# jerinphilip/whisper.tflite

Hardware: AMD Instinct MI355X
Metric: audio-sec/s (RTF) whisper-tiny 30s clips batch=32 at 1/2/4/8 MI355X (higher is better)
Workload: dtype f32 (operands as two fp16 planes, f16 MFMA, f32 accumulate); 1 GPU; whisper-tiny batch=32x30s synthetic mel U(-1,1.5), fp32, random-init weights (BASELINE.json configs[1]); mel resident in HBM -> token ids on host; clips_per_gpu=32, global_batch=32, decoder_positions=30, argmax_steps=27, parallelism=clip-parallel dp1, one RCCL all_gather of id records per 8 batches, pipelined=True, batches_in_flight=10, decoder=2 consecutive steps' batches share one decoder chain (dec_pair, dec_group), last_batches_announced=2, priming_batches=1

## Files before the change

### include/wt_debug.h

```cpp
#ifndef WT_DEBUG_H_
#define WT_DEBUG_H_
#include "wt_capi.h"
#ifdef __cplusplus
extern "C" {
#endif
int wt_dbg_gemm(wt_engine* h, int M, int N, int K, const float* A, const float* W, const float* bias,
                const float* R, const float* pos, int pos_period, int epi, float* C);
int wt_dbg_gemm_planes(wt_engine* h, int M, int N, int K, const float* A, const float* W, const float* bias,
                       const float* R, const float* pos, int pos_period, int epi, int planes_out, int iters, float* C,
                       float* avg_ms, int n_cu );
int wt_dbg_set_forced_ids(wt_engine* h, const int64_t* ids, int clips);
int wt_dbg_set_plane_gemm_mode(int mode);
int wt_dbg_gemm_planes_ln(wt_engine* h, int M, int K, const float* A, const float* W, const float* bias, const float* R,
                          const float* pos, int pos_period, int epi, const float* ln_g, const float* ln_b, int n_cu,
                          float* C, float* ln_out, float* ln_y32, int* fused);
int wt_dbg_encoder_attention_planes(wt_engine* h, int batch, int T, int heads, const float* qkv, int iters, float* out,
                                    float* avg_ms);
int wt_dbg_gemm_bench(wt_engine* h, int M, int N, int K, int epi, int variant, int iters, float* avg_ms);
int wt_dbg_interference(wt_engine* h, const float* d_mel, int batch, int n_enc, int chain_len, int blocks,
                        float* enc_ms, float* chain_ms);
int wt_dbg_concurrency(wt_engine* h, const float* d_mel, int batch, int n_dec, int n_enc, float* dec_ms,
                       float* enc_ms);
int wt_dbg_dec_gemm_bench(wt_engine* h, int kind, int B, int N, int K, int rows, int iters, float* avg_us);
int wt_dbg_dec_gemm(wt_engine* h, int mode, int B, int N, int K, const float* X, const float* W,
                    const float* bias, const float* R, float* Y, int64_t* argmax_out);
int wt_dbg_dec_ln_gemm(wt_engine* h, int B, int N, int K, const float* xin, const int64_t* ids, int pos,
                       const float* tok_emb, const float* pos_emb, int n_vocab, int n_pos,
                       const float* ln_g, const float* ln_b, const float* W, const float* bias,
                       int gelu, float* Y, float* xout);
int wt_dbg_layernorm(wt_engine* h, int M, int d, const float* x, const float* g, const float* b, float* y);
int wt_dbg_encoder_attention(wt_engine* h, int batch, int T, int heads, const float* qkv, float* out);
int wt_dbg_cross_attention(wt_engine* h, int batch, int heads, int T, int chunks, int nq, const float* x,
                           const float* ln_g, const float* ln_b, const float* wq, const float* bq, const float* kc,
                           const float* vc, float* out);
int wt_dbg_cross_absorbed(wt_engine* h, int batch, int heads, int T, int chunks, int nq, const float* qp, const float* E,
                          const float* wv, const float* bv, float* out, int iters, float* avg_us);
int wt_dbg_cross_absorbed_bf16(wt_engine* h, int batch, int heads, int T, int chunks, int nq, const float* qp, const float* E,
                               const float* wv, const float* bv, float* out, int iters, float* avg_us);
int wt_dbg_cross_absorbed_chain(wt_engine* h, int bf16, int batch, int heads, int T, int chunks, int nq, int split, int n_src,
                                const float* const* E_src, const float* qp, const float* wv, const float* bv, int mode,
                                int p0_only, int nq_only, float* out, float* ws);
int wt_dbg_absorbed_query_matrix(int heads, int d, const float* wq, const float* bq, const float* wk, float* A, float* av);
int wt_dbg_self_attention(wt_engine* h, int batch, int heads, int cap, int pos, int npos, const float* qkv,
                          float* kcache, float* vcache, float* out);
int wt_dbg_self_attention_long(wt_engine* h, int batch, int heads, int cap, int pos, const float* qkv, float* kcache,
                               float* vcache, float* out);
int wt_dbg_timestamp_select(wt_engine* h, int B, int V, const float* logits, const int64_t* ids, int ids_stride,
                            const int32_t* n_ids, int sample_begin, int eot, int beg, int max_initial_timestamp,
                            int64_t* token, double* L, float* M);
int wt_dbg_gemm_bf16(wt_engine* h, int M, int N, int K, const float* A, const float* W, const float* bias,
                     const float* R, const float* pos, int pos_period, int epi, int bf16_out, int iters, float* C,
                     float* avg_ms);
int wt_dbg_gemm_bf16_ln(wt_engine* h, int M, int N, int K, const float* A, const float* W, const float* bias, const float* R,
                        const float* ln_g, const float* ln_b, float* C, float* ln_out, float* ln_y32, int* fused);
int wt_dbg_encoder_attention_bf16(wt_engine* h, int batch, int T, int heads, const float* qkv, int iters, float* out,
                                  float* avg_ms);
int wt_dbg_dec_gemm_bf16(wt_engine* h, int mode, int B, int N, int K, const float* X, const float* W, const float* bias,
                         const float* R, float* Y, int64_t* argmax_out);
int wt_dbg_dec_ln_gemm_bf16(wt_engine* h, int B, int N, int K, const float* xin, const int64_t* ids, int pos,
                            const float* tok_emb, const float* pos_emb, int n_vocab, int n_pos, const float* ln_g,
                            const float* ln_b, const float* W, const float* bias, int gelu, float* Y, float* xout);
int wt_dbg_self_attention_bf16(wt_engine* h, int batch, int heads, int cap, int pos, int npos, const float* qkv,
                               float* kcache, float* vcache, float* out);
int wt_dbg_cross_attention_bf16(wt_engine* h, int batch, int heads, int T, int chunks, int nq, const float* x,
                                const float* ln_g, const float* ln_b, const float* wq, const float* bq, const float* kc,
                                const float* vc, float* out);
int wt_dbg_beam_topk(wt_engine* h, int rows, int V, int ldl, int kk, const float* logits, float* m, float* s,
                     uint64_t* keys);
int wt_dbg_beam_step(wt_engine* h, int K, int clips, int c0, int n_live, int pos, int n_prompt, int V, int64_t eot,
                     const float* logits, const int64_t* ids, float* live_sum, int32_t* fin_tok, float* fin_sum,
                     int32_t* fin_len, int32_t* n_fin, int32_t* done, int32_t* parent, int64_t* token, int64_t* ids_next);
int wt_dbg_beam_reorder(wt_engine* h, int src_rows, int dst_rows, int cap, int d, int slabs, int pos, int V,
                        const float* kv_src, float* kv_dst, const int64_t* ids_src, int64_t* ids_dst,
                        const int32_t* parent, const int64_t* token);
int wt_dbg_beam_finalize(wt_engine* h, int K, int clips, int c0, int pos, int n_prompt, const int64_t* ids,
                         const float* live_sum, int32_t* fin_tok, float* fin_sum, int32_t* fin_len, int32_t* n_fin,
                         const int32_t* done, int64_t* out_ids, int32_t* out_n, float* out_sum, int32_t* out_len);
int wt_dbg_dec_gemm_ksplit(wt_engine* h, int bf16, int M, int B, int N, int K, const float* X, const float* W,
                           const float* bias, float* R, float* Y, float* part);
int wt_dbg_dec_ln_gemm_rows(wt_engine* h, int bf16, int M, int B, int N, int K, const float* xin, const float* xpart,
                            const int64_t* ids, int ids_stride, int pos, const float* tok_emb, const float* pos_emb,
                            int n_vocab, int n_pos, const float* ln_g, const float* ln_b, const float* W, const float* bias,
                            int gelu, float* Y, float* xout);
int wt_dbg_dec_logits(wt_engine* h, int bf16, int M, int V, int K, const float* xin, const float* xpart, const float* ln_g,
                      const float* ln_b, const float* E, int blocks, float* logits, uint64_t* records);
int wt_dbg_select_token(wt_engine* h, int B, int n_tiles, const uint64_t* records, int64_t* ids, int stride, int pos,
                        int32_t* n_ids, int32_t* finished, int64_t eot, int stop_at_eot, int keep_ids);
int wt_dbg_language_head(wt_engine* h, int rows, int d, int n_vocab, int lang_lo, int n_lang, int forced_lang, const float* x,
                         const float* xpart, const float* ln_g, const float* ln_b, const float* tok_emb, float* probs,
                         int32_t* lang, float* lang_prob, int64_t* ids, int ids_stride);
#ifdef __cplusplus
}
#endif
#endif
```

### whisper.tflite_amd/__init__.py

```python
from __future__ import annotations

import ctypes
import enum
import os
from ctypes import (POINTER, byref, c_char_p, c_float, c_int, c_int32, c_int64, c_long, c_size_t,
                    c_uint64, c_void_p)

import numpy as np

_HERE = os.path.dirname(os.path.abspath(__file__))
LIB_PATH = os.environ.get("WT_LIB_PATH") or os.path.join(_HERE, "lib", "libwhisper-tflite.so")

WT_OK = 0
WT_MAX_IDS = 32
WT_PIPELINE_DEPTH = 24
WT_LANGUAGE_AUTO = -1
CHUNK_SAMPLES = 480000
STATUS_NAMES = {0: "WT_OK", 1: "WT_ERR_INVALID_ARG", 2: "WT_ERR_IO", 3: "WT_ERR_FORMAT",
                4: "WT_ERR_UNSUPPORTED", 5: "WT_ERR_DEVICE", 6: "WT_ERR_BUFFER"}

CAPI_SYMBOLS = [
    "wt_device_alloc", "wt_device_free", "wt_device_upload", "wt_device_download", "wt_device_synchronize",
    "wt_engine_create", "wt_engine_destroy", "wt_last_error", "wt_engine_dims",
    "wt_engine_set_option", "wt_engine_get_option", "wt_engine_set_prompt", "wt_transcribe_pcm", "wt_transcribe_long_pcm", "wt_transcribe_file",
    "wt_logmel_batch", "wt_logmel_batch_dev", "wt_encdec_tokens_batch",
    "wt_encdec_tokens_batch_dev", "wt_transcribe_tokens_batch_dev", "wt_pipeline_submit_dev", "wt_pipeline_submit_pcm_dev", "wt_pipeline_collect",
    "wt_encdec_debug_batch",
    "wt_encdec_tokens_full_batch", "wt_encdec_tokens_full_batch_dev", "wt_transcribe_tokens_full_batch_dev",
    "wt_last_segments", "wt_last_segment_text", "wt_vocab_segments",
    "wt_language_count", "wt_detect_language_batch", "wt_detect_language_batch_dev", "wt_detect_language_pcm", "wt_last_languages",
    "wt_last_timings", "wt_last_beam_scores", "wt_last_kernel_stats", "wt_decode_text", "wt_language_id", "wt_lang_code", "wt_wav_read_legacy",
    "wt_vocab_info", "wt_filters", "wt_write_synthetic_weights", "wt_write_synthetic_vocab",
    "wt_vocab_open", "wt_vocab_close", "wt_vocab_get_info", "wt_vocab_get_filters", "wt_vocab_size", "wt_vocab_token",
    "wt_vocab_decode", "wt_log_mel_spectrogram", "wt_convert_tflite", "wt_shutdown",
]
DEBUG_SYMBOLS = [
    "wt_dbg_cross_absorbed", "wt_dbg_cross_absorbed_bf16", "wt_dbg_gemm_planes_ln", "wt_dbg_gemm", "wt_dbg_gemm_bench", "wt_dbg_dec_gemm_bench", "wt_dbg_dec_gemm", "wt_dbg_dec_ln_gemm", "wt_dbg_layernorm", "wt_dbg_encoder_attention",
    "wt_dbg_cross_attention", "wt_dbg_self_attention", "wt_dbg_interference", "wt_dbg_concurrency",
    "wt_dbg_gemm_planes", "wt_dbg_set_plane_gemm_mode", "wt_dbg_set_forced_ids", "wt_dbg_dec_gemm_bf16", "wt_dbg_dec_ln_gemm_bf16",
    "wt_dbg_self_attention_bf16", "wt_dbg_cross_attention_bf16", "wt_dbg_encoder_attention_planes", "wt_dbg_gemm_bf16", "wt_dbg_gemm_bf16_ln", "wt_dbg_encoder_attention_bf16",
    "wt_dbg_beam_topk", "wt_dbg_beam_step", "wt_dbg_beam_reorder", "wt_dbg_beam_finalize",
    "wt_dbg_dec_gemm_ksplit", "wt_dbg_dec_ln_gemm_rows", "wt_dbg_dec_logits", "wt_dbg_select_token",
    "wt_dbg_cross_absorbed_chain", "wt_dbg_absorbed_query_matrix", "wt_dbg_language_head", "wt_dbg_self_attention_long",
    "wt_dbg_timestamp_select",
]


class WtError(RuntimeError):
    def __init__(self, code: int, message: str):
        super().__init__(f"{STATUS_NAMES.get(code, code)}: {message}")
        self.code = code


class EngineType(enum.IntEnum):
    Monolith = 0
    EncDec = 1


class Dims(ctypes.Structure):
    _fields_ = [(n, c_int32) for n in (
        "n_mels", "n_audio_ctx", "n_audio_state", "n_audio_head", "n_audio_layer",
        "n_vocab", "n_text_ctx", "n_text_state", "n_text_head", "n_text_layer")]


class Timings(ctypes.Structure):
    _fields_ = [("logmel_ms", c_float), ("encoder_ms", c_float), ("cross_kv_ms", c_float),
                ("decoder_ms", c_float), ("total_ms", c_float), ("batch", c_int32),
                ("decoder_steps", c_int32)]


class KernelStat(ctypes.Structure):
    _fields_ = [("name", ctypes.c_char * 48), ("launches", c_int32), ("reserved", c_int32),
                ("ms", ctypes.c_double), ("flops", ctypes.c_double), ("bytes", ctypes.c_double)]


_lib = None


def lib() -> ctypes.CDLL:
    global _lib
    if _lib is None:
        if not os.path.exists(LIB_PATH):
            raise ImportError(
                f"{LIB_PATH} is missing: build it with `make lib` (or __graft_entry__.build()); "
                "there is no Python/CPU fallback for the engine")
        L = ctypes.CDLL(LIB_PATH)
        fp, ip64, ip32 = POINTER(c_float), POINTER(c_int64), POINTER(c_int32)
        L.wt_engine_create.argtypes = [c_int, c_char_p, c_char_p, c_int, c_int, POINTER(c_void_p)]
        L.wt_engine_destroy.argtypes = [c_void_p]
        L.wt_engine_destroy.restype = None
        L.wt_last_error.argtypes = [c_void_p]
        L.wt_last_error.restype = c_char_p
        L.wt_engine_dims.argtypes = [c_void_p, POINTER(Dims)]
        L.wt_engine_set_option.argtypes = [c_void_p, c_char_p, c_long]
        L.wt_engine_get_option.argtypes = [c_void_p, c_char_p, POINTER(c_long)]
        L.wt_engine_set_prompt.argtypes = [c_void_p, ip64, c_int]
        L.wt_transcribe_pcm.argtypes = [c_void_p, fp, c_size_t, c_char_p, c_size_t, POINTER(c_size_t)]
        L.wt_transcribe_long_pcm.argtypes = [c_void_p, fp, c_size_t, c_char_p, c_size_t, POINTER(c_size_t)]
        L.wt_transcribe_file.argtypes = [c_void_p, c_char_p, c_char_p, c_size_t, POINTER(c_size_t)]
        L.wt_logmel_batch.argtypes = [c_void_p, fp, c_int, fp]
        L.wt_logmel_batch_dev.argtypes = [c_void_p, c_void_p, c_int, c_void_p]
        L.wt_encdec_tokens_batch.argtypes = [c_void_p, fp, c_int, ip64, ip32]
        L.wt_encdec_tokens_batch_dev.argtypes = [c_void_p, c_void_p, c_int, ip64, ip32]
        L.wt_transcribe_tokens_batch_dev.argtypes = [c_void_p, c_void_p, c_int, ip64, ip32]
        L.wt_pipeline_submit_dev.argtypes = [c_void_p, c_void_p, c_int]
        L.wt_pipeline_submit_pcm_dev.argtypes = [c_void_p, c_void_p, c_int]
        L.wt_pipeline_collect.argtypes = [c_void_p, ip64, ip32]
        L.wt_encdec_debug_batch.argtypes = [c_void_p, fp, c_int, ip64, ip32, fp, fp, c_int]
        L.wt_last_timings.argtypes = [c_void_p, POINTER(Timings)]
        L.wt_last_beam_scores.argtypes = [c_void_p, fp, ip32, c_int]
        L.wt_last_kernel_stats.argtypes = [c_void_p, POINTER(KernelStat), c_int]
        L.wt_decode_text.argtypes = [c_void_p, ip64, c_int, c_int, c_char_p, c_size_t, POINTER(c_size_t)]
        L.wt_language_id.argtypes = [c_char_p]
        L.wt_lang_code.argtypes = [c_int]
        L.wt_lang_code.restype = c_char_p
        L.wt_wav_read_legacy.argtypes = [c_char_p, fp, c_size_t, POINTER(c_size_t)]
        L.wt_vocab_info.argtypes = [c_void_p, ip32]
        L.wt_filters.argtypes = [c_void_p, fp, c_size_t, ip32, ip32]
        L.wt_write_synthetic_weights.argtypes = [c_char_p, c_char_p, c_uint64]
        L.wt_write_synthetic_vocab.argtypes = [c_char_p, c_int]
        L.wt_vocab_open.argtypes = [c_char_p, c_int, POINTER(c_void_p)]
        L.wt_vocab_close.argtypes = [c_void_p]
        L.wt_vocab_close.restype = None
        L.wt_vocab_get_info.argtypes = [c_void_p, ip32]
        L.wt_vocab_get_filters.argtypes = [c_void_p, fp, c_size_t, ip32, ip32]
        L.wt_vocab_size.argtypes = [c_void_p]
        L.wt_vocab_token.argtypes = [c_void_p, c_int, c_char_p, c_size_t, POINTER(c_size_t)]
        L.wt_vocab_decode.argtypes = [c_void_p, ip64, c_int, c_int, c_char_p, c_size_t, POINTER(c_size_t)]
        L.wt_log_mel_spectrogram.argtypes = [fp, c_int, fp, c_int, c_int, c_int, fp, c_size_t, POINTER(c_int)]
        L.wt_convert_tflite.argtypes = [c_char_p, c_char_p]
        L.wt_dbg_gemm.argtypes = [c_void_p, c_int, c_int, c_int, fp, fp, fp, fp, fp, c_int, c_int, fp]
        L.wt_dbg_gemm_planes.argtypes = [c_void_p, c_int, c_int, c_int, fp, fp, fp, fp, fp, c_int, c_int, c_int, c_int, fp,
                                         POINTER(c_float), c_int]
        L.wt_dbg_encoder_attention_planes.argtypes = [c_void_p, c_int, c_int, c_int, fp, c_int, fp, POINTER(c_float)]
        L.wt_dbg_cross_absorbed.argtypes = [c_void_p, c_int, c_int, c_int, c_int, c_int, fp, fp, fp, fp, fp, c_int, POINTER(c_float)]
        L.wt_dbg_cross_absorbed_bf16.argtypes = L.wt_dbg_cross_absorbed.argtypes
        L.wt_dbg_cross_absorbed_chain.argtypes = [c_void_p, c_int, c_int, c_int, c_int, c_int, c_int, c_int, c_int, POINTER(fp),
                                                  fp, fp, fp, c_int, c_int, c_int, fp, fp]
        L.wt_dbg_absorbed_query_matrix.argtypes = [c_int, c_int, fp, fp, fp, fp, fp]
        L.wt_dbg_gemm_planes_ln.argtypes = [c_void_p, c_int, c_int, fp, fp, fp, fp, fp, c_int, c_int, fp, fp, c_int, fp, fp, fp,
                                            POINTER(c_int)]
        L.wt_dbg_gemm_bf16.argtypes = [c_void_p, c_int, c_int, c_int, fp, fp, fp, fp, fp, c_int, c_int, c_int, c_int, fp,
                                       POINTER(c_float)]
        L.wt_dbg_encoder_attention_bf16.argtypes = [c_void_p, c_int, c_int, c_int, fp, c_int, fp, POINTER(c_float)]
        L.wt_dbg_gemm_bf16_ln.argtypes = [c_void_p, c_int, c_int, c_int, fp, fp, fp, fp, fp, fp, fp, fp, fp, POINTER(c_int)]
        L.wt_dbg_gemm_bench.argtypes = [c_void_p, c_int, c_int, c_int, c_int, c_int, c_int, POINTER(c_float)]
        L.wt_dbg_dec_gemm_bench.argtypes = [c_void_p, c_int, c_int, c_int, c_int, c_int, c_int, POINTER(c_float)]
        L.wt_dbg_dec_gemm.argtypes = [c_void_p, c_int, c_int, c_int, c_int, fp, fp, fp, fp, fp, ip64]
        L.wt_dbg_dec_ln_gemm.argtypes = [c_void_p, c_int, c_int, c_int, fp, ip64, c_int, fp, fp,
                                         c_int, c_int, fp, fp, fp, fp, c_int, fp, fp]
        L.wt_dbg_layernorm.argtypes = [c_void_p, c_int, c_int, fp, fp, fp, fp]
        L.wt_device_alloc.argtypes = [c_void_p, ctypes.c_size_t, POINTER(c_void_p)]
        L.wt_device_free.argtypes = [c_void_p, c_void_p]
        L.wt_device_upload.argtypes = [c_void_p, c_void_p, ctypes.c_size_t, c_void_p, ctypes.c_size_t]
        L.wt_device_download.argtypes = [c_void_p, c_void_p, c_void_p, ctypes.c_size_t, ctypes.c_size_t]
        L.wt_device_synchronize.argtypes = [c_void_p]
        L.wt_dbg_set_forced_ids.argtypes = [c_void_p, POINTER(c_int64), c_int]
        L.wt_dbg_dec_gemm_bf16.argtypes = L.wt_dbg_dec_gemm.argtypes
        L.wt_dbg_dec_ln_gemm_bf16.argtypes = L.wt_dbg_dec_ln_gemm.argtypes
        L.wt_dbg_encoder_attention.argtypes = [c_void_p, c_int, c_int, c_int, fp, fp]
        L.wt_dbg_cross_attention.argtypes = [c_void_p, c_int, c_int, c_int, c_int, c_int, fp, fp, fp, fp, fp, fp, fp, fp]
        L.wt_dbg_self_attention.argtypes = [c_void_p, c_int, c_int, c_int, c_int, c_int, fp, fp, fp, fp]
        L.wt_dbg_self_attention_bf16.argtypes = L.wt_dbg_self_attention.argtypes
        L.wt_dbg_cross_attention_bf16.argtypes = L.wt_dbg_cross_attention.argtypes
        u64p = POINTER(c_uint64)
        L.wt_dbg_beam_topk.argtypes = [c_void_p, c_int, c_int, c_int, c_int, fp, fp, fp, u64p]
        L.wt_dbg_beam_step.argtypes = [c_void_p, c_int, c_int, c_int, c_int, c_int, c_int, c_int, c_int64, fp, ip64, fp, ip32,
                                       fp, ip32, ip32, ip32, ip32, ip64, ip64]
        L.wt_dbg_beam_reorder.argtypes = [c_void_p, c_int, c_int, c_int, c_int, c_int, c_int, c_int, fp, fp, ip64, ip64, ip32,
                                          ip64]
        L.wt_dbg_beam_finalize.argtypes = [c_void_p, c_int, c_int, c_int, c_int, c_int, ip64, fp, ip32, fp, ip32, ip32, ip32,
                                           ip64, ip32, fp, ip32]
        L.wt_dbg_dec_gemm_ksplit.argtypes = [c_void_p, c_int, c_int, c_int, c_int, c_int, fp, fp, fp, fp, fp, fp]
        L.wt_dbg_dec_ln_gemm_rows.argtypes = [c_void_p, c_int, c_int, c_int, c_int, c_int, fp, fp, ip64, c_int, c_int, fp, fp,
                                              c_int, c_int, fp, fp, fp, fp, c_int, fp, fp]
        L.wt_dbg_dec_logits.argtypes = [c_void_p, c_int, c_int, c_int, c_int, fp, fp, fp, fp, fp, c_int, fp, u64p]
        L.wt_dbg_select_token.argtypes = [c_void_p, c_int, c_int, u64p, ip64, c_int, c_int, ip32, ip32, c_int64, c_int,
                                          c_int]
        L.wt_language_count.argtypes = [c_void_p]
        L.wt_detect_language_batch.argtypes = [c_void_p, fp, c_int, ip32, fp]
        L.wt_detect_language_batch_dev.argtypes = [c_void_p, c_void_p, c_int, ip32, fp]
        L.wt_detect_language_pcm.argtypes = [c_void_p, fp, c_size_t, ip32, fp]
        L.wt_last_languages.argtypes = [c_void_p, ip32, fp, c_int]
        L.wt_dbg_language_head.argtypes = [c_void_p, c_int, c_int, c_int, c_int, c_int, c_int, fp, fp, fp, fp, fp, fp, ip32, fp,
                                           ip64, c_int]
        L.wt_encdec_tokens_full_batch.argtypes = [c_void_p, fp, c_int, ip64, c_int, ip32]
        L.wt_encdec_tokens_full_batch_dev.argtypes = [c_void_p, c_void_p, c_int, ip64, c_int, ip32]
        L.wt_transcribe_tokens_full_batch_dev.argtypes = [c_void_p, c_void_p, c_int, ip64, c_int, ip32]
        L.wt_dbg_self_attention_long.argtypes = [c_void_p, c_int, c_int, c_int, c_int, fp, fp, fp, fp]
        L.wt_last_segments.argtypes = [c_void_p, c_void_p, c_int]
        L.wt_last_segment_text.argtypes = [c_void_p, c_int, c_char_p, c_size_t, POINTER(c_size_t)]
        L.wt_vocab_segments.argtypes = [c_void_p, ip64, c_int, c_int, c_void_p, c_int]
        L.wt_dbg_timestamp_select.argtypes = [c_void_p, c_int, c_int, fp, ip64, c_int, ip32, c_int, c_int, c_int, c_int,
                                              ip64, POINTER(ctypes.c_double), fp]
        _lib = L
    return _lib


def _f32(a) -> np.ndarray:
    return np.ascontiguousarray(a, dtype=np.float32)


def _fp(a: np.ndarray):
    return a.ctypes.data_as(POINTER(c_float)) if a is not None else None


def _ip32(a: np.ndarray):
    if a.dtype != np.int32 or not a.flags.c_contiguous:
        raise ValueError("expected a contiguous int32 array")
    return a.ctypes.data_as(POINTER(c_int32))


def _ip64(a: np.ndarray):
    if a.dtype != np.int64 or not a.flags.c_contiguous:
        raise ValueError("expected a contiguous int64 array")
    return a.ctypes.data_as(POINTER(c_int64))


def write_synthetic_weights(path: str, arch: str = "tiny", seed: int = 0) -> None:
    rc = lib().wt_write_synthetic_weights(path.encode(), arch.encode(), seed)
    if rc != WT_OK:
# ... 363 lines not shown
    def decode_text(self, ids, omit_special_tokens: bool = False) -> str:
        return self.decode_bytes(ids, omit_special_tokens).decode("utf-8", errors="replace")

    def vocab_info(self) -> dict:
        out = (c_int32 * 9)()
        self._check(lib().wt_vocab_info(self._h, out))
        keys = ("n_vocab", "eot", "sot", "translate", "transcribe", "prev", "solm", "not", "beg")
        return dict(zip(keys, list(out)))

    def filters(self) -> np.ndarray:
        nm, nf = c_int32(0), c_int32(0)
        total = lib().wt_filters(self._h, None, 0, byref(nm), byref(nf))
        out = np.zeros(total, np.float32)
        lib().wt_filters(self._h, _fp(out), out.size, byref(nm), byref(nf))
        return out.reshape(nm.value, nf.value)

    def dbg_gemm(self, A, W, bias=None, R=None, pos=None, epi=0):
        A, W = _f32(A), _f32(W)
        M, K = A.shape
        N = W.shape[0]
        C = np.zeros((M, N), np.float32)
        bias = _f32(bias) if bias is not None else None
        R = _f32(R) if R is not None else None
        pos = _f32(pos) if pos is not None else None
        self._check(lib().wt_dbg_gemm(self._h, M, N, K, _fp(A), _fp(W), _fp(bias), _fp(R), _fp(pos),
                                      pos.shape[0] if pos is not None else 0, epi, _fp(C)))
        return C

    def dbg_gemm_planes(self, A, W, bias=None, R=None, pos=None, epi=1, planes_out=False, iters=0, n_cu=0):
        A, W = _f32(A), _f32(W)
        M, K = A.shape
        N = W.shape[0]
        C = np.zeros((M, N), np.float32)
        bias = _f32(bias) if bias is not None else np.zeros(N, np.float32)
        R = _f32(R) if R is not None else None
        pos = _f32(pos) if pos is not None else None
        ms = c_float(0)
        self._check(lib().wt_dbg_gemm_planes(self._h, M, N, K, _fp(A), _fp(W), _fp(bias), _fp(R), _fp(pos),
                                             pos.shape[0] if pos is not None else 0, epi, int(planes_out), iters, _fp(C),
                                             byref(ms), int(n_cu)))
        return (C, ms.value) if iters > 0 else C

    def dbg_gemm_planes_ln(self, A, W, bias, ln_g, ln_b, R=None, pos=None, epi=5, n_cu=0, want_y32=True):
        A, W = _f32(A), _f32(W)
        M, K = A.shape
        assert W.shape[0] == 384
        C = np.zeros((M, 384), np.float32)
        ln = np.zeros((M, 384), np.float32)
        y32 = np.zeros((M, 384), np.float32) if want_y32 else None
        R = _f32(R) if R is not None else None
        pos = _f32(pos) if pos is not None else None
        fused = ctypes.c_int(0)
        self._check(lib().wt_dbg_gemm_planes_ln(self._h, M, K, _fp(A), _fp(W), _fp(_f32(bias)), _fp(R), _fp(pos),
                                                pos.shape[0] if pos is not None else 0, epi, _fp(_f32(ln_g)), _fp(_f32(ln_b)),
                                                int(n_cu), _fp(C), _fp(ln), _fp(y32) if y32 is not None else None, byref(fused)))
        return C, ln, y32, bool(fused.value)

    def dbg_cross_absorbed(self, qp, E, wv, bv, batch, heads, T, chunks, nq, iters=0, bf16=False):
        qp, E, wv, bv = _f32(qp), _f32(E), _f32(wv), _f32(bv)
        d = heads * 64
        out = np.zeros((nq * batch, d), np.float32)
        us = c_float(0)
        fn = lib().wt_dbg_cross_absorbed_bf16 if bf16 else lib().wt_dbg_cross_absorbed
        self._check(fn(self._h, batch, heads, T, chunks, nq, _fp(qp), _fp(E), _fp(wv), _fp(bv), _fp(out), iters, byref(us)))
        return (out, us.value) if iters > 0 else out

    def dbg_cross_absorbed_chain(self, qp, E_src, wv, bv, batch, heads, T, chunks, nq, split=None, bf16=False, only=None,
                                 combine_only=False, ws=None, out=None, ws_fill=-7.0, out_fill=-9.0):
        d, rows = heads * 64, nq * batch
        wv, bv = _f32(wv), _f32(bv)
        srcs = [_f32(e) for e in (E_src or [])]
        qp = _f32(qp) if qp is not None else None
        ws = np.array(ws, np.float32, order="C") if ws is not None else np.full((rows + 1, heads, chunks, d + 4), ws_fill, np.float32)
        out = np.array(out, np.float32, order="C") if out is not None else np.full((rows + 1, d), out_fill, np.float32)
        assert ws.shape == (rows + 1, heads, chunks, d + 4) and out.shape == (rows + 1, d)
        ptrs = (POINTER(c_float) * max(1, len(srcs)))(*[_fp(e) for e in srcs])
        mode = 2 if combine_only else (1 if only is not None else 0)
        p0, n1 = only if only is not None else (0, 0)
        self._check(lib().wt_dbg_cross_absorbed_chain(
            self._h, int(bf16), batch, heads, T, chunks, nq, batch if split is None else split, len(srcs), ptrs, _fp(qp),
            _fp(wv), _fp(bv), mode, p0, n1, _fp(out), _fp(ws)))
        return out, ws

    def dbg_encoder_attention_planes(self, qkv, batch, T, heads, iters=0):
        qkv = _f32(qkv)
        out = np.zeros((batch * T, heads * 64), np.float32)
        ms = c_float(0)
        self._check(lib().wt_dbg_encoder_attention_planes(self._h, batch, T, heads, _fp(qkv), iters, _fp(out), byref(ms)))
        return (out, ms.value) if iters > 0 else out

    def dbg_gemm_bf16(self, A, W, bias=None, R=None, pos=None, epi=1, bf16_out=False, iters=0):
        A, W = _f32(A), _f32(W)
        M, K = A.shape
        N = W.shape[0]
        C = np.zeros((M, N), np.float32)
        bias = _f32(bias) if bias is not None else np.zeros(N, np.float32)
        R = _f32(R) if R is not None else None
        pos = _f32(pos) if pos is not None else None
        ms = c_float(0)
        self._check(lib().wt_dbg_gemm_bf16(self._h, M, N, K, _fp(A), _fp(W), _fp(bias), _fp(R), _fp(pos),
                                           pos.shape[0] if pos is not None else 0, epi, int(bf16_out), iters, _fp(C),
                                           byref(ms)))
        return (C, ms.value) if iters > 0 else C

    def dbg_encoder_attention_bf16(self, qkv, batch, T, heads, iters=0):
        qkv = _f32(qkv)
        out = np.zeros((batch * T, heads * 64), np.float32)
        ms = c_float(0)
        self._check(lib().wt_dbg_encoder_attention_bf16(self._h, batch, T, heads, _fp(qkv), iters, _fp(out), byref(ms)))
        return (out, ms.value) if iters > 0 else out

    def dbg_gemm_bench(self, M, N, K, epi=1, variant=0, iters=10) -> float:
        ms = c_float(0)
        self._check(lib().wt_dbg_gemm_bench(self._h, M, N, K, epi, variant, iters, byref(ms)))
        return ms.value

    def device_array(self, a):
        return DeviceArray(self, a)

    def device_synchronize(self):
        self._check(lib().wt_device_synchronize(self._h))

    def set_forced_ids(self, ids=None):
        if ids is None:
            self._check(lib().wt_dbg_set_forced_ids(self._h, None, 0))
            return
        a = np.ascontiguousarray(ids, dtype=np.int64)
        assert a.ndim == 2 and a.shape[1] == 32
        self._check(lib().wt_dbg_set_forced_ids(self._h, a.ctypes.data_as(POINTER(c_int64)), a.shape[0]))

    def dbg_gemm_bf16_ln(self, A, W, bias, R, ln_g, ln_b):
        A, W, bias, R, ln_g, ln_b = (_f32(v) for v in (A, W, bias, R, ln_g, ln_b))
        M, K = A.shape
        N = W.shape[0]
        C = np.zeros((M, N), np.float32)
        ln = np.zeros((M, N), np.float32)
        y32 = np.zeros((M, N), np.float32)
        fused = c_int(0)
        self._check(lib().wt_dbg_gemm_bf16_ln(self._h, M, N, K, _fp(A), _fp(W), _fp(bias), _fp(R), _fp(ln_g), _fp(ln_b), _fp(C), _fp(ln),
                                              _fp(y32), byref(fused)))
        return C, ln, y32, bool(fused.value)

    def dbg_dec_gemm_bench(self, kind, B, N, K, rows=None, iters=200) -> float:
        us = c_float(0)
        self._check(lib().wt_dbg_dec_gemm_bench(self._h, kind, B, N, K, rows or B, iters, byref(us)))
        return us.value

    def dbg_dec_gemm(self, X, W, bias=None, mode=0, R=None, bf16=False):
        X, W = _f32(X), _f32(W)
        B, K = X.shape
        N = W.shape[0]
        bias = _f32(bias) if bias is not None else np.zeros(N, np.float32)
        R = _f32(R) if R is not None else None
        Y = np.zeros((B, N), np.float32)
        am = np.zeros(B, np.int64)
        fn = lib().wt_dbg_dec_gemm_bf16 if bf16 else lib().wt_dbg_dec_gemm
        self._check(fn(self._h, mode, B, N, K, _fp(X), _fp(W), _fp(bias), _fp(R), _fp(Y), am.ctypes.data_as(POINTER(c_int64))))
        return (Y, am) if mode == 3 else Y

    def dbg_dec_ln_gemm(self, W, bias, ln_g, ln_b, xin=None, ids=None, pos=0, tok_emb=None, pos_emb=None,
                        gelu=False, bf16=False):
        W, bias, ln_g, ln_b = _f32(W), _f32(bias), _f32(ln_g), _f32(ln_b)
        N, K = W.shape
        xin = _f32(xin) if xin is not None else None
        ids_a = np.ascontiguousarray(ids, dtype=np.int64) if ids is not None else None
        tok_emb = _f32(tok_emb) if tok_emb is not None else None
# ... 224 lines not shown
```

### whisper.tflite_amd/csrc/capi.cpp

```cpp
#include "wt_capi.h"

#include <hip/hip_runtime.h>

#include <functional>

#include <cstdio>
#include <cstdlib>
#include <sys/stat.h>
#include <unistd.h>
#include <cmath>
#include <cstring>
#include <memory>
#include <string>
#include <vector>

#include <mutex>

#include "engine.h"
#include "tflite_extract.h"
#include "weights_gen.h"
#include "wt_debug.h"
#include "kernels.h"

struct wt_engine {
// ... 127 lines not shown
    auto make = [&] {
      h->impl.reset(new wt::Engine(prefix, vocab_path, multilingual != 0, device_id, engine_type == WT_ENGINE_MONOLITH, wpath));
    };
    try {
      make();
    } catch (const wt::Error& e) {
      if (e.code != wt::kErrFormat || !have_pair || converted) throw;
      convert();
      make();
    }
  });
  if (rc != WT_OK) return rc;
  *out = h.release();
  return WT_OK;
}

void wt_engine_destroy(wt_engine* h) { delete h; }

const char* wt_last_error(const wt_engine* h) {
  return h ? h->last_error.c_str() : g_create_error.c_str();
}

int wt_engine_dims(const wt_engine* h, wt_dims* out) {
  if (!h || !out) return WT_ERR_INVALID_ARG;
  static_assert(sizeof(wt_dims) == sizeof(wtw::Dims), "wt_dims mirrors wtw::Dims");
  std::memcpy(out, &h->impl->dims(), sizeof(wt_dims));
  return WT_OK;
}

int wt_engine_set_option(wt_engine* h, const char* key, long value) {
  if (!h || !key) return WT_ERR_INVALID_ARG;
  wt::Engine& e = *h->impl;
  const std::string k(key);
  if (k == "language") {
    try {
      e.set_language(value);
    } catch (const wt::Error& err) {
      return fail(h, err.code, err.what());
    }
  } else if (k == "max_tokens") {
    if (value < 4 || value > 31) return fail(h, WT_ERR_INVALID_ARG, "max_tokens must be in [4, 31]");
    e.max_tokens = value;
  } else if (k == "max_positions") {
    if (value != 0 && (value < 32 || value > e.full_cap())) {
      return fail(h, WT_ERR_INVALID_ARG, "max_positions must be 0 (off) or in [32, n_text_ctx] (at most 448)");
    }
    e.max_positions = value;
  } else if (k == "timestamps") {
    if (value != 0 && value != 1) return fail(h, WT_ERR_INVALID_ARG, "timestamps must be 0 or 1");
    if (value == 1 && !e.has_timestamp_tokens()) {
      return fail(h, WT_ERR_UNSUPPORTED, "timestamps: the model's vocabulary has no timestamp ids (n_vocab <= token_beg + 1)");
    }
    e.timestamps = value;
  } else if (k == "max_initial_timestamp") {
    if (value < -1 || value > 1500) return fail(h, WT_ERR_INVALID_ARG, "max_initial_timestamp must be in [-1, 1500] (ticks of 20 ms, -1 = no limit)");
    e.max_initial_timestamp = value;
  } else if (k == "stop_at_eot") {
    e.stop_at_eot = value != 0;
  } else if (k == "verbose") {
    e.verbose = value;
  } else if (k == "cross_chunks") {
    if (value != 0 && value != 1 && value != 2 && value != 4 && value != 8) return fail(h, WT_ERR_INVALID_ARG, "cross_chunks must be 0 (by batch size), 1, 2, 4 or 8");
    e.cross_chunks = value;
  } else if (k == "attn_variant") {
    if (value != 0 && value != 1 && value != 4) return fail(h, WT_ERR_INVALID_ARG, "attn_variant must be 4 (default: two fp16 planes), 1 (three bf16 planes, full range) or 0 (fp32 MFMA)");
    e.attn_variant = value;
  } else if (k == "fc2_ksplit") {
    if (value != 1 && value != 2) return fail(h, WT_ERR_INVALID_ARG, "fc2_ksplit must be 1 or 2");
    e.fc2_ksplit = value;
  } else if (k == "use_graphs") {
    e.use_graphs = value != 0;
  } else if (k == "cross_absorb") {
    e.cross_absorb = value != 0;
  } else if (k == "last_batches") {
    if (value < 0 || value > WT_PIPELINE_DEPTH) return fail(h, WT_ERR_INVALID_ARG, "last_batches: 0..24");
    e.last_batches = value;
  } else if (k == "dec_pair") {
    if (h->impl->in_flight() > 0) return fail(h, WT_ERR_INVALID_ARG, "collect the submitted batches before changing dec_pair");
    e.dec_pair = value != 0;
  } else if (k == "dec_group") {
    if (h->impl->in_flight() > 0) return fail(h, WT_ERR_INVALID_ARG, "collect the submitted batches before changing dec_group");
    if (value < 2 || value > 4) return fail(h, WT_ERR_INVALID_ARG, "dec_group: 2, 3 or 4 batches per decoder chain (dec_pair = 0 turns grouping off)");
    e.dec_group = value;
  } else if (k == "abs_chunks") {
    if (value < 0 || value > 16) return fail(h, WT_ERR_INVALID_ARG, "abs_chunks must be 0 (automatic) or 1..16");
    e.abs_chunks = value;
  } else if (k == "gemm_variant") {
    if (value != -1 && !wt::gemm_variant_supported(int(value))) {
      return fail(h, WT_ERR_INVALID_ARG, "gemm_variant must be -1 (default: plane GEMM), 0 (fp32 MFMA), 13 or 16 (three bf16 planes)");
    }
    e.gemm_variant = value;
  } else if (k == "force_fallback") {
    try {
      e.set_force_fallback(value);
    } catch (const wt::Error& err) {
      return fail(h, err.code, err.what());
    }
  } else if (k == "kernel_timers") {
    if (value < 0 || value > 1024) return fail(h, WT_ERR_INVALID_ARG, "kernel_timers must be in [0, 1024]");
    e.kernel_timers = value;
  } else if (k == "beam_size") {
    if (value < 1 || value > wt::kBeamMax) return fail(h, WT_ERR_INVALID_ARG, "beam_size must be in [1, 8] (1 = greedy)");
    e.beam_size = value;
  } else if (k == "bf16") {
    try {
      e.bind_device();
      e.set_bf16(value != 0);
    } catch (const wt::Error& err) {
      return fail(h, err.code, err.what());
    } catch (const std::exception& err) {
      return fail(h, WT_ERR_DEVICE, err.what());
    }
  } else {
    return fail(h, WT_ERR_INVALID_ARG, "unknown option: " + k);
  }
  return WT_OK;
}

int wt_engine_set_prompt(wt_engine* h, const int64_t* ids, int n) {
  if (!h || n < 0 || n > 8 || (n && !ids)) return WT_ERR_INVALID_ARG;
  h->impl->prompt_override.assign(ids, ids + n);
  return WT_OK;
}

int wt_engine_get_option(const wt_engine* h, const char* key, long* value) {
  if (!h || !key || !value) return WT_ERR_INVALID_ARG;
  const wt::Engine& e = *h->impl;
  const std::string k(key);
  if (k == "language") *value = e.language;
  else if (k == "max_tokens") *value = e.max_tokens;
  else if (k == "max_positions") *value = e.max_positions;
  else if (k == "timestamps") *value = e.timestamps;
  else if (k == "max_initial_timestamp") *value = e.max_initial_timestamp;
  else if (k == "stop_at_eot") *value = e.stop_at_eot;
  else if (k == "verbose") *value = e.verbose;
  else if (k == "cross_chunks") *value = e.cross_chunks;
  else if (k == "gemm_variant") *value = e.gemm_variant;
  else if (k == "use_graphs") *value = e.use_graphs;
  else if (k == "cross_absorb") *value = e.cross_absorb;
  else if (k == "abs_chunks") *value = e.abs_chunks;
  else if (k == "dec_pair") *value = e.dec_pair;
  else if (k == "dec_group") *value = e.dec_group;
  else if (k == "last_batches") *value = e.last_batches;
  else if (k == "cross_absorb_active") *value = e.absorb_active() ? 1 : 0;
  else if (k == "bf16") *value = e.bf16;
  else if (k == "beam_size") *value = e.beam_size;
  else if (k == "kernel_timers") *value = e.kernel_timers;
  else if (k == "fc2_ksplit") *value = e.fc2_ksplit;
  else if (k == "attn_variant") *value = e.attn_variant;
  else if (k == "force_fallback") *value = e.force_fallback();
  else if (k == "f16_fallbacks") *value = e.f16_fallbacks();
  else if (k == "f16_contractions") *value = e.f16_contractions();
  else if (k == "f16_min_slack_millibits") *value = long(std::lround(1000.0 * e.f16_min_slack_bits()));
  else if (k == "in_flight") *value = e.in_flight();
  else if (k == "pipelined_encoder_cus") *value = e.pipelined_encoder_cus();
  else return WT_ERR_INVALID_ARG;
  return WT_OK;
}


int wt_device_alloc(wt_engine* h, size_t bytes, void** d_ptr) {
  if (!h || !d_ptr) return WT_ERR_INVALID_ARG;
  *d_ptr = nullptr;
  return guarded(h, [&] {
    h->impl->bind_device();
    hipchk(hipMalloc(d_ptr, bytes > 0 ? bytes : 4), "hipMalloc");
  });
}

int wt_device_free(wt_engine* h, void* d_ptr) {
  if (!h) return WT_ERR_INVALID_ARG;
  return guarded(h, [&] {
    h->impl->bind_device();
    if (d_ptr) hipchk(hipFree(d_ptr), "hipFree");
  });
}

int wt_device_upload(wt_engine* h, void* d_dst, size_t offset, const void* src, size_t bytes) {
  if (!h || !d_dst || (!src && bytes)) return WT_ERR_INVALID_ARG;
  return guarded(h, [&] {
    h->impl->bind_device();
    if (bytes) hipchk(hipMemcpy(static_cast<char*>(d_dst) + offset, src, bytes, hipMemcpyHostToDevice), "H2D");
  });
}

int wt_device_download(wt_engine* h, void* dst, const void* d_src, size_t offset, size_t bytes) {
  if (!h || !d_src || (!dst && bytes)) return WT_ERR_INVALID_ARG;
  return guarded(h, [&] {
    h->impl->bind_device();
    if (bytes) hipchk(hipMemcpy(dst, static_cast<const char*>(d_src) + offset, bytes, hipMemcpyDeviceToHost), "D2H");
  });
}

int wt_device_synchronize(wt_engine* h) {
  if (!h) return WT_ERR_INVALID_ARG;
  return guarded(h, [&] {
    h->impl->bind_device();
    hipchk(hipDeviceSynchronize(), "hipDeviceSynchronize");
  });
}

int wt_logmel_batch_dev(wt_engine* h, const float* d_pcm, int batch, float* d_mel) {
  if (!h || !d_pcm || !d_mel) return WT_ERR_INVALID_ARG;
  return guarded(h, [&] {
    h->impl->require_idle();
    h->impl->logmel(d_pcm, batch, d_mel);
    h->impl->sync();
  });
}

int wt_logmel_batch(wt_engine* h, const float* pcm, int batch, float* mel) {
  if (!h || !pcm || !mel) return WT_ERR_INVALID_ARG;
  return guarded(h, [&] {
    wt::Engine& e = *h->impl;
    e.require_idle();
    float* d_pcm = e.staging_pcm(batch);
    float* d_mel = e.staging_mel(batch);
    hipchk(hipMemcpyAsync(d_pcm, pcm, size_t(batch) * e.pcm_elems() * sizeof(float), hipMemcpyHostToDevice, e.stream()), "H2D pcm");
    e.logmel(d_pcm, batch, d_mel);
    hipchk(hipMemcpyAsync(mel, d_mel, size_t(batch) * e.mel_elems() * sizeof(float), hipMemcpyDeviceToHost, e.stream()), "D2H mel");
    e.sync();
  });
}
// ... 1537 lines not shown
    wt::launch_select_token(dRec.p, n_tiles, dids.p, stride, pos, dn.p, dfin.p, eot, stop_at_eot, B, h->impl->stream(),
                            keep_ids != 0);
    h->impl->sync();
    dids.to_host(reinterpret_cast<long long*>(ids));
    dn.to_host(n_ids);
    dfin.to_host(finished);
  });
}

int wt_dbg_timestamp_select(wt_engine* h, int B, int V, const float* logits, const int64_t* ids, int ids_stride,
                            const int32_t* n_ids, int sample_begin, int eot, int beg, int max_initial_timestamp,
                            int64_t* token, double* L, float* M) {
  if (!h || !logits || !ids || !n_ids || !token || B < 1 || B > 64 || V < 2 || ids_stride < 1 || sample_begin < 0) {
    return WT_ERR_INVALID_ARG;
  }
  return guarded(h, [&] {
    const int ldl = (V + 3) & ~3;
    for (int b = 0; b < B; ++b) {
      if (n_ids[b] < sample_begin || n_ids[b] > ids_stride) throw wt::Error(WT_ERR_INVALID_ARG, "wt_dbg_timestamp_select: n_ids outside [sample_begin, ids_stride]");
    }
    std::vector<float> padded(size_t(B) * ldl, 0.0f);
    for (int b = 0; b < B; ++b) std::memcpy(&padded[size_t(b) * ldl], logits + size_t(b) * V, size_t(V) * sizeof(float));
    const int stride = ids_stride + 1;
    std::vector<long long> rows(size_t(B) * stride, 0);
    for (int b = 0; b < B; ++b)
      for (int i = 0; i < n_ids[b]; ++i) rows[size_t(b) * stride + i] = ids[size_t(b) * ids_stride + i];
    DevArr<float> dlog(padded.size(), padded.data());
    DevArr<long long> dids(rows.size(), rows.data());
    DevArr<int> dn(B, n_ids), dfin(B);
    DevArr<wt::TsPart> dpart(size_t(B) * wt::ts_chunks(V));
    DevArr<wt::TsState> dstate(B);
    DevArr<double> dL(B);
    DevArr<float> dM(B);
    hipchk(hipMemsetAsync(dfin.p, 0, size_t(B) * sizeof(int), h->impl->stream()), "memset");
    wt::launch_ts_state_init(dids.p, stride, dn.p, 0, sample_begin, V, beg, dstate.p, B, h->impl->stream());
    for (int b0 = 0, b1 = 0; b0 < B; b0 = b1 + 1) {
      b1 = b0;
      while (b1 + 1 < B && n_ids[b1 + 1] == n_ids[b0]) ++b1;
      wt::TsSelectArgs t;
      t.logits = dlog.p + size_t(b0) * ldl; t.ldl = ldl; t.V = V; t.batch = b1 - b0 + 1;
      t.eot = eot; t.beg = beg; t.max_initial = max_initial_timestamp;
      t.n_gen = n_ids[b0] - sample_begin; t.part = dpart.p + size_t(b0) * wt::ts_chunks(V); t.state = dstate.p + b0;
      t.ids = dids.p + size_t(b0) * stride; t.ids_stride = stride; t.pos = n_ids[b0] - 1; t.stop_at_eot = 1;
      t.n_ids = dn.p + b0; t.finished = dfin.p + b0;
      t.dbg_L = dL.p + b0; t.dbg_M = dM.p + b0;
      wt::launch_ts_select(t, h->impl->stream());
    }
    h->impl->sync();
    dids.to_host(rows.data());
    for (int b = 0; b < B; ++b) token[b] = rows[size_t(b) * stride + n_ids[b]];
    if (L) dL.to_host(L);
    if (M) dM.to_host(M);
  });
}

int wt_dbg_language_head(wt_engine* h, int rows, int d, int n_vocab, int lang_lo, int n_lang, int forced_lang, const float* x,
                         const float* xpart, const float* ln_g, const float* ln_b, const float* tok_emb, float* probs,
                         int32_t* lang, float* lang_prob, int64_t* ids, int ids_stride) {
  if (!h || !x || !ln_g || !ln_b || !tok_emb || !probs || !lang || !lang_prob || rows < 1 || rows > 128 || d < 1 ||
      d > wt::kLangMaxD || n_vocab < 1 || n_vocab > 4096 || lang_lo < 0 || n_lang < 1 || n_lang > wt::kLangMax ||
      lang_lo + n_lang > n_vocab || forced_lang >= n_lang || (ids && ids_stride < 2)) {
    return WT_ERR_INVALID_ARG;
  }
  return guarded(h, [&] {
    const size_t rd = size_t(rows) * d;
    DevArr<float> dx(rd, x), dxp(xpart ? rd : 0, xpart), dg(d, ln_g), db(d, ln_b), demb(size_t(n_vocab) * d, tok_emb);
    DevArr<float> dprobs(size_t(rows) * n_lang), dprob(rows);
    DevArr<int> dlang(rows);
    DevArr<long long> dids(ids ? size_t(rows) * ids_stride : 0, reinterpret_cast<const long long*>(ids));
    wt::LanguageHeadArgs a;
    a.x = dx.p; a.xpart = xpart ? dxp.p : nullptr; a.ln_g = dg.p; a.ln_b = db.p; a.tok_emb = demb.p;
    a.rows = rows; a.d = d; a.n_vocab = n_vocab; a.lang_lo = lang_lo; a.n_lang = n_lang;
    a.probs = dprobs.p; a.lang = dlang.p; a.lang_prob = dprob.p; a.forced_lang = forced_lang;
    if (ids) a.ids = dids.p, a.ids_stride = ids_stride, a.id_pos = 1;
    wt::launch_language_head(a, h->impl->stream());
    h->impl->sync();
    dprobs.to_host(probs);
    dprob.to_host(lang_prob);
    dlang.to_host(lang);
    if (ids) dids.to_host(reinterpret_cast<long long*>(ids));
  });
}

int wt_dbg_cross_absorbed_chain(wt_engine* h, int bf16, int batch, int heads, int T, int chunks, int nq, int split, int n_src,
                                const float* const* E_src, const float* qp, const float* wv, const float* bv, int mode,
                                int p0_only, int nq_only, float* out, float* ws) {
  if (!h || !wv || !bv || !out || !ws || batch < 1 || heads < 1 || heads > 8 || T < 1 || nq < 1 || chunks < 1 || chunks > 16 ||
      size_t(nq) * batch > 128 || mode < 0 || mode > 2) {
    return WT_ERR_INVALID_ARG;
  }
  if (mode != 2) {
    if (!qp || !E_src || n_src < 1 || n_src > 4 || split < 1 || split > batch || (n_src == 1 && split != batch)) return WT_ERR_INVALID_ARG;
    for (int i = 0; i < n_src; ++i)
      if (!E_src[i]) return WT_ERR_INVALID_ARG;
    if (mode == 1 && (p0_only < 0 || nq_only < 1 || p0_only + nq_only > nq)) return WT_ERR_INVALID_ARG;
  }
  return guarded(h, [&] {
    const bool bf = bf16 != 0;
    const size_t d = size_t(heads) * 64, rows = size_t(nq) * batch, clip = size_t(T) * d;
    const std::vector<float> wvt = wt::cross_q_layout(wv, int(d));
    DevArr<float> dwv(wvt.size(), wvt.data()), dbv(d, bv), dq(mode != 2 ? rows * heads * d : 0, qp);
    DevArr<float> dws((rows + 1) * heads * chunks * (d + 4), ws), dout((rows + 1) * d, out);
    hipStream_t st = h->impl->stream();
    const size_t plane = size_t(batch) * clip + 64;
    std::vector<std::unique_ptr<DevArr<unsigned short>>> src;
    float se = 1.0f;
    if (mode != 2) {
      const auto clips_of = [&](int i) { return std::max(0, std::min(split, batch - i * split)); };
      float mx = 0.0f;
      for (int i = 0; i < n_src; ++i) mx = std::max(mx, max_abs(E_src[i], size_t(clips_of(i)) * clip));
      se = bf ? 1.0f : wt::f16_scale_for(mx);
      for (int i = 0; i < n_src; ++i) {
        const size_t n = size_t(clips_of(i)) * clip;
        std::vector<unsigned short> host((bf ? 1 : 2) * plane, bf ? 0x7FC0 : 0x7E00);
        for (size_t k = 0; k < n; ++k) {
          if (bf) {
            host[k] = DevBf16::rne(E_src[i][k]);
          } else {
            const float v = E_src[i][k] * se;
            const _Float16 hi = static_cast<_Float16>(v), lo = static_cast<_Float16>(v - static_cast<float>(hi));
            std::memcpy(&host[k], &hi, 2);
            std::memcpy(&host[plane + k], &lo, 2);
          }
        }
        src.push_back(std::make_unique<DevArr<unsigned short>>(host.size(), host.data()));
      }
      const int nq_max = wt::cross_absorbed_max_nq(heads);
      const auto launch = [&](int p0, int n) {
        wt::CrossAbsorbedArgs a;
        a.qp = dq.p; a.e = src[0]->p; a.e_plane = long(plane); a.e_scale = se; a.ws = dws.p; a.bf16 = bf;
        if (n_src > 1) {
          a.split = split;
          a.e2 = src[1]->p;
          if (n_src > 2) a.e3 = src[2]->p;
          if (n_src > 3) a.e4 = src[3]->p;
        }
        a.batch = batch; a.heads = heads; a.d_model = int(d); a.T = T; a.chunks = chunks; a.nq = n; a.p0 = p0;
        wt::launch_cross_absorbed(a, st);
      };
      if (mode == 1) {
        launch(p0_only, nq_only);
      } else {
        for (int p0 = 0; p0 < nq; p0 += nq_max) launch(p0, std::min(nq_max, nq - p0));
      }
    }
    wt::launch_cross_absorbed_combine(dws.p, dwv.p, dbv.p, dout.p, int(rows), heads, chunks, int(d), st);
    h->impl->sync();
    dout.to_host(out);
    dws.to_host(ws);
  });
}

int wt_dbg_absorbed_query_matrix(int heads, int d, const float* wq, const float* bq, const float* wk, float* A, float* av) {
  if (heads < 1 || d != heads * 64 || !wq || !bq || !wk || !A || !av) return WT_ERR_INVALID_ARG;
  return guarded(nullptr, [&] {
    std::vector<float> Am, am;
    wt::absorbed_query_matrix(wq, bq, wk, heads, d, &Am, &am);
    std::memcpy(A, Am.data(), Am.size() * sizeof(float));
    std::memcpy(av, am.data(), am.size() * sizeof(float));
  });
}

}
```

### whisper.tflite_amd/csrc/engine.cpp

```cpp
#include "engine.h"

#include <fcntl.h>
#include <sys/mman.h>
#include <sys/stat.h>
#include <unistd.h>

#include <chrono>
#include <cmath>
#include <complex>
#include <cstdio>
#include <cstdlib>
#include <cstring>
#include <stdexcept>

#include "kernels.h"

namespace wt {

namespace {
void hip_check(hipError_t e, const char* what) {
  if (e != hipSuccess) {
    throw Error(5, std::string("HIP failure in ") + what + ": " + hipGetErrorString(e));
  }
}
// ... 828 lines not shown
  if (target == stream_) return;
  HIPCHK(hipEventRecord(ev_switch_, stream_));
  HIPCHK(hipStreamWaitEvent(target, ev_switch_, 0));
  stream_ = target;
}

void Engine::bind_device() { HIPCHK(hipSetDevice(device_)); }

void Engine::sync() {
  HIPCHK(hipStreamSynchronize(stream_full_));
  if (stream_masked_) HIPCHK(hipStreamSynchronize(stream_masked_));
  for (auto& ds : dstream_) HIPCHK(hipStreamSynchronize(ds));
}

void Engine::need_cross_kv(Slot& slot) {
  if (slot.cross_kv) return;
  const wtw::Dims& c = dims_;
  void* p = nullptr;
  HIPCHK(hipMalloc(&p, size_t(c.n_text_layer) * 2 * size_t(ws_.batch) * c.n_audio_ctx * c.n_audio_state * sizeof(float)));
  ws_.owned.push_back(p);
  slot.cross_kv = static_cast<float*>(p);
}

void Engine::ensure_batch(int batch) {
  if (batch <= 0 || batch > 4096) throw Error(1, "batch must be in [1, 4096]");
  HIPCHK(hipSetDevice(device_));
  if (batch <= ws_.batch) return;
  if (!inflight_.empty()) throw Error(1, "cannot grow the workspace while batches are in flight");
  HIPCHK(hipStreamSynchronize(stream_));
  for (auto& ds : dstream_) HIPCHK(hipStreamSynchronize(ds));
  for (auto& g : graphs_) (void)hipGraphExecDestroy(g.second.exec);
  graphs_.clear();
  for (void* p : ws_.owned) (void)hipFree(p);
  ws_ = Workspace();
  const wtw::Dims& c = dims_;
  const size_t B = batch, T0 = mel_frames(), T = c.n_audio_ctx, d = c.n_audio_state;
  auto alloc = [&](size_t n_floats, bool zero) -> float* {
    void* p = nullptr;
    HIPCHK(hipMalloc(&p, n_floats * sizeof(float)));
    ws_.owned.push_back(p);
    if (zero) HIPCHK(hipMemsetAsync(p, 0, n_floats * sizeof(float), stream_));
    return static_cast<float*>(p);
  };
  if (d == 0) {
    ws_.mel_stage = alloc(B * mel_elems(), false);
    ws_.batch = batch;
    HIPCHK(hipStreamSynchronize(stream_));
    return;
  }
  ws_.melT = alloc(B * (T0 + 2) * c.n_mels + 256, true);
  ws_.h1p = alloc(B * (T0 + 2) * d + 256, true);
  ws_.melTp = reinterpret_cast<unsigned short*>(alloc(B * (T0 + 2) * c.n_mels + 256, true));
  ws_.h1pp = reinterpret_cast<unsigned short*>(alloc(B * (T0 + 2) * d + 256, true));
  ws_.x = alloc(B * T * d, false);
  ws_.ln = alloc(B * T * d, false);
  ws_.qkv = alloc(B * T * 3 * d, false);
  ws_.att = alloc(B * T * d, false);
  ws_.hid = alloc(B * T * 4 * d, false);
  ws_.enc_out = alloc(B * T * d, false);
  ws_.cvt = reinterpret_cast<unsigned short*>(alloc(B * T * 4 * d, false));
  for (Slot& sl : slots_) {
    sl.cross_kv = nullptr;
    sl.e_planes = reinterpret_cast<unsigned short*>(alloc(B * T * d, false));
    sl.used = false;
  }
  const size_t R = std::max<size_t>(B, kDecRowsMax);
  for (DecWorkspace& dw : dws_) {
    dw.xd = alloc(R * d, false);
    dw.xb = alloc(R * d, false);
    dw.xpart = alloc(R * d, false);
    dw.qkvd = alloc(R * 3 * d, false);
    dw.attd = alloc(R * d, false);
    dw.hd = alloc(R * 4 * d, false);
    dw.cross_ws = alloc(R * c.n_text_head * 8 * 68, false);
    dw.qp = alloc(R * c.n_text_head * d, false);
    dw.abs_ws = alloc(R * c.n_text_head * 16 * (d + 4), false);
    dw.cabs = alloc(R * c.n_text_head * d, false);
    dw.self_kv = alloc(size_t(c.n_text_layer) * 2 * B * self_cap_ * d, true);
    dw.logits = alloc(B * c.n_vocab, false);
    dw.best = reinterpret_cast<unsigned long long*>(alloc(B * 2 * size_t((c.n_vocab + 31) / 32), true));
    dw.ids = reinterpret_cast<long long*>(alloc(B * 32 * 2, true));
    dw.n_ids = reinterpret_cast<int*>(alloc(B, true));
    dw.finished = reinterpret_cast<int*>(alloc(B, true));
  }
  ws_.mel_stage = alloc(B * mel_elems(), false);
  ws_.batch = batch;
  HIPCHK(hipStreamSynchronize(stream_));
}

float* Engine::staging_mel(int batch) {
  ensure_batch(batch);
  return ws_.mel_stage;
}

float* Engine::staging_pcm(int batch) {
  ensure_batch(batch);
  if (!ws_.pcm_stage) {
    void* p = nullptr;
    HIPCHK(hipMalloc(&p, size_t(ws_.batch) * pcm_elems() * sizeof(float)));
    ws_.owned.push_back(p);
    ws_.pcm_stage = static_cast<float*>(p);
  }
  return ws_.pcm_stage;
}


void Engine::logmel(const float* d_pcm, int batch, float* d_mel, int valid_frames) {
  if (!have_logmel_) throw Error(3, "vocab file carries no 80x201 mel filter bank");
  ensure_batch(batch);
  const size_t T0 = mel_frames(), n_samples = pcm_elems(), pad = n_samples + 512;
  if (!ws_.pcm_planes) {
    const size_t Bc = ws_.batch;
    auto alloc = [&](size_t n_floats) -> float* {
      void* p = nullptr;
      HIPCHK(hipMalloc(&p, n_floats * sizeof(float)));
      ws_.owned.push_back(p);
      HIPCHK(hipMemsetAsync(p, 0, n_floats * sizeof(float), stream_));
      return static_cast<float*>(p);
    };
    pcm_plane_ = long(Bc * pad + 1024);
    ws_.pcm_planes = reinterpret_cast<unsigned short*>(alloc((size_t(pcm_plane_) * 2 * sizeof(unsigned short) + 3) / 4 + 64));
    ws_.pw = alloc(Bc * T0 * size_t(pw_ld_));
    ws_.melacc = alloc(Bc * T0 * mel_n);
    ws_.clip_max = reinterpret_cast<unsigned*>(alloc(Bc * kClipMaxStride * kClipMaxWays));
  }
  HIPCHK(hipEventRecord(ev_[0], stream_));
  const long M = long(batch) * long(T0);
  launch_pcm_to_planes(d_pcm, ws_.pcm_planes, pcm_plane_, f16_scale_for(kPcmBound), kPcmBound, batch, long(n_samples), long(pad),
                       stream_);
  PlaneGemmArgs g;
  g.A = ws_.pcm_planes;
  g.a_plane = pcm_plane_;
  g.a_rpb = int(T0);
  g.a_bs = long(pad);
  g.lda = 160;
  g.W = dft_basis_p_.w;
  g.bias = dft_zero_bias_;
  g.C = ws_.pw;
  g.M = int(M);
  g.N = dft_n;
  g.K = dft_k;
  g.ldc = pw_ld_;
  g.a_scale = f16_scale_for(kPcmBound);
  g.w_scale = dft_w_scale_;
  g.n_cu = stream_ == stream_masked_ && enc_cus_masked_ > 0 ? enc_cus_masked_ : n_cu_;
  launch_gemm_planes(g, kEpiBias | kEpiPower, stream_);
  GemmArgs m;
  m.A = ws_.pw;
  m.lda = pw_ld_;
  m.W = mel_w;
  m.C = ws_.melacc;
  m.M = int(M);
  m.N = mel_n;
  m.K = mel_k;
  m.ldc = mel_n;
  m.variant = gemm_variant >= 0 ? int(gemm_variant) : 13;
  launch_gemm(m, 0, stream_);
  HIPCHK(hipMemsetAsync(ws_.clip_max, 0, sizeof(unsigned) * batch * kClipMaxStride * kClipMaxWays, stream_));
  launch_log_clipmax(ws_.melacc, mel_n, d_mel, ws_.clip_max, batch, dims_.n_mels, int(T0), stream_, valid_frames);
  launch_mel_normalize(d_mel, ws_.clip_max, batch, dims_.n_mels, int(T0), stream_);
  HIPCHK(hipEventRecord(ev_[1], stream_));
  timings_.logmel_ms = -1.0f;
}


thread_local LaunchTimer g_launch_timer;
// ... 616 lines not shown
  float* d_mel = staging_mel(batch);
  logmel(d_pcm, batch, d_mel);
  encode_enqueue(d_mel, batch);
  submit_decoder(batch, last_enc_slot_);
}

void Engine::collect(int64_t* ids, int32_t* n_ids) {
  if (inflight_.empty()) throw Error(1, "collect() without a submitted batch");
  const int slot = inflight_.front();
  if (std::find(pending_.begin(), pending_.end(), slot) != pending_.end()) flush_pending();
  inflight_.erase(inflight_.begin());
  decode_collect(slot, ids, n_ids);
}

std::vector<long long> Engine::prompt() const {
  if (!prompt_override.empty()) return prompt_override;
  if (monolith_ && !multilingual_) {
    if (timestamps) return {vocab_.token_sot};
    return {vocab_.token_sot, vocab_.token_not};
  }
  if (timestamps) return {vocab_.token_sot, kLangLo + std::max<long>(language, 0), vocab_.token_transcribe};
  return {vocab_.token_sot, kLangLo + std::max<long>(language, 0), vocab_.token_transcribe, vocab_.token_not};
}

void Engine::decode_enqueue(int batch, int slot_idx, float* logits_host, int logits_steps_cap, int group, bool pipelined,
                            int stream_override) {
  const bool paired = group > 1;
  const int per = batch;
  if (group < 1 || group > 4) throw Error(kErrInvalidArg, "decoder chains take one to four batches");
  batch = group * per;
  if (batch > (paired ? kDecRowsMax : 64)) throw Error(1, "decoder batches are limited to 64 clips per call");
  for (int j = 0; paired && j < group; ++j) {
    if (!slots_[(slot_idx + j) % kSlots].absorbed || logits_host) throw Error(kErrInvalidArg, "decoder groups: the absorbed form only");
  }
  ensure_batch(batch);
  Slot& slot = slots_[slot_idx];
  auto dec_of = [&](int si) { return stream_override >= 0 ? stream_override : (si / group) % n_dec_streams_; };
  slot.dec = dec_of(slot_idx);
  slot.pair_leader = -1;
  DecWorkspace& dw = dws_[slot.dec];
  hipStream_t const stream_ = dec_stream_at(slot.dec);
  HIPCHK(hipStreamWaitEvent(stream_, slot.enc_done, 0));
  for (int j = 1; j < group; ++j) HIPCHK(hipStreamWaitEvent(stream_, slots_[(slot_idx + j) % kSlots].enc_done, 0));
  HIPCHK(hipEventRecord(slot.dec_begin, stream_));
  long long* const h_ids_ = slot.h_ids;
  int* const h_n_ = slot.h_n;
  const wtw::Dims& c = dims_;
  const int d = c.n_text_state, T = c.n_audio_ctx, H = c.n_text_head, V = c.n_vocab;
  const int lang_mode = detect_only_ ? 2 : (language < 0 ? 1 : 0);
  const int n_lang = lang_mode ? lang_tokens() : 0;
  if (lang_mode) {
    if (n_lang < 1) throw Error(kErrUnsupported, "language detection: this engine's vocabulary has no language tokens");
    ensure_lang_workspace();
  }
  const std::vector<long long> prompt = lang_mode == 2 ? std::vector<long long>{vocab_.token_sot} : this->prompt();
  const int n_prompt = int(prompt.size()), stride = 32;
  for (long long id : prompt) {
    if (id < 0 || id >= V) throw Error(1, "prompt token id outside the model's vocabulary");
  }
  const int max_pos = lang_mode == 2 ? 1 : int(std::min<long>(std::max<long>(max_tokens, n_prompt), 31));
  const bool forced = !forced_ids.empty() && lang_mode != 2;
  if (forced && forced_ids.size() != size_t(batch) * stride) {
    throw Error(kErrInvalidArg, "forced ids are set for another number of clips than this decode has");
  }
  for (long long id : forced_ids) {
    if (!forced) break;
    if (id < 0 || id >= V) throw Error(kErrInvalidArg, "forced token id outside the model's vocabulary");
  }
  for (int b = 0; b < batch; ++b) {
    for (int i = 0; i < stride; ++i) {
      h_ids_[size_t(b) * stride + i] = forced ? forced_ids[size_t(b) * stride + i] : (i < n_prompt ? prompt[i] : 0);
    }
    h_n_[b] = n_prompt;
  }
  int chunks = int(cross_chunks);
  if (chunks == 0) {
    chunks = 1;
    while (chunks < 8 && batch * H * chunks < 192) chunks *= 2;
  }
  const bool absorbed = slot.absorbed;
  const int abs_blocks = pipelined ? (bf16 ? 64 : 128) : 256;
  int n_abs = abs_chunks > 0 ? int(abs_chunks) : std::min(16, std::max(1, (abs_blocks + batch - 1) / batch));
  n_abs = std::min(n_abs, (T + 31) / 32);
  int steps = 0;
  static const bool dec_timers = getenv("WT_DEC_KERNEL_TIMERS") != nullptr;
  std::vector<hipEvent_t>& dt_ev = slot.dt_events;
  std::vector<int>& dt_cls = slot.dt_cls;
  size_t dt_used = 0;
  bool dt_on = false;
#define DT(CLS, CALL)                                                         \
  do {                                                                        \
    if (dt_on) {                                                              \
      while (dt_ev.size() < dt_used + 2) {                                    \
        hipEvent_t e_;                                                        \
        HIPCHK(hipEventCreate(&e_));                                          \
        dt_ev.push_back(e_);                                                  \
      }                                                                       \
      HIPCHK(hipEventRecord(dt_ev[dt_used], stream_));                        \
      CALL;                                                                   \
      HIPCHK(hipEventRecord(dt_ev[dt_used + 1], stream_));                    \
      dt_cls.push_back(CLS);                                                  \
      dt_used += 2;                                                           \
    } else {                                                                  \
      CALL;                                                                   \
    }                                                                         \
  } while (0)
  (void)dw;
  auto enqueue_all = [&](int si) {
    Slot& slot = slots_[si];
    const Slot* const member[4] = {&slot, &slots_[(si + 1) % kSlots], &slots_[(si + 2) % kSlots], &slots_[(si + 3) % kSlots]};
    DecWorkspace& dw = dws_[dec_of(si)];
    hipStream_t const stream_ = dec_stream_at(dec_of(si));
    long long* const h_ids_ = slot.h_ids;
    int* const h_n_ = slot.h_n;
    steps = 0;
    HIPCHK(hipMemcpyAsync(dw.ids, h_ids_, size_t(batch) * stride * sizeof(long long),
                          hipMemcpyHostToDevice, stream_));
    HIPCHK(hipMemcpyAsync(dw.n_ids, h_n_, size_t(batch) * sizeof(int), hipMemcpyHostToDevice, stream_));
    HIPCHK(hipMemsetAsync(dw.finished, 0, size_t(batch) * sizeof(int), stream_));

    const bool bf = bf16 != 0;
    const size_t kv_slab = size_t(batch) * T * d;
    const size_t self_slab = size_t(batch) * self_cap_ * d;
    auto cache_at = [&](float* base, size_t elems) -> void* {
      return bf ? static_cast<void*>(reinterpret_cast<unsigned short*>(base) + elems) : static_cast<void*>(base + elems);
    };
    float* const x = dw.xd;
    const bool split = fc2_ksplit == 2 && (4 * d) % 256 == 0;
    const int np_max = std::max(1, std::min(4, kDecRowsMax / batch));
    const int prompt_end = std::min(n_prompt, max_pos);
    for (int pos0 = 0, np = 1; pos0 < max_pos; pos0 += np) {
      np = pos0 < prompt_end ? std::min(np_max, prompt_end - pos0) : 1;
      if (lang_mode && pos0 == 0) np = 1;
      const int M = np * batch, last = pos0 + np - 1;
      for (int l = 0; l < c.n_text_layer; ++l) {
        const DecBlockWeights& w = bf ? dec_blocks_bf_[l] : dec_blocks_[l];
        DecGemmArgs q;
        q.bf16 = bf;
        q.Wt = w.wqkv.w; q.w_scale = w.wqkv.scale; q.N = 3 * d; q.K = d; q.B = batch; q.M = M;
        q.xin = x; q.ln_g = w.attn_ln_g; q.ln_b = w.attn_ln_b;
        if (l > 0 && split) {
          q.xin = dw.xb; q.xpart = dw.xpart; q.xout = x;
        }
        if (l == 0) {
          q.ids = dw.ids; q.ids_stride = stride; q.pos = pos0; q.tok_emb = tok_emb; q.pos_emb = dec_pos;
          q.n_vocab = V; q.xout = x;
        }
        q.bias = w.bqkv; q.Y = dw.qkvd; q.ldy = 3 * d;
        DT(0, launch_dec_gemm(q, kProLn, kDecBias, stream_));
        DT(1, launch_self_attention(dw.qkvd, cache_at(dw.self_kv, (size_t(l) * 2 + 0) * self_slab),
                                    cache_at(dw.self_kv, (size_t(l) * 2 + 1) * self_slab), self_cap_, pos0, np, dw.attd,
                                    batch, H, stream_, bf));
        DecGemmArgs o;
        o.bf16 = bf;
        o.Wt = w.wo.w; o.w_scale = w.wo.scale; o.N = d; o.K = d; o.B = batch; o.M = M; o.X = dw.attd; o.ldx = d;
        o.bias = w.bo; o.R = x; o.Y = x; o.ldy = d;
        DT(2, launch_dec_gemm(o, kProNone, kDecResid, stream_));

        if (absorbed) {
          DecGemmArgs qa;
          qa.Wt = w.wq_abs.w; qa.w_scale = w.wq_abs.scale; qa.N = H * d; qa.K = d; qa.B = batch; qa.M = M;
          qa.bf16 = bf;
          qa.xin = x; qa.ln_g = w.cross_ln_g; qa.ln_b = w.cross_ln_b; qa.bias = w.bq_abs; qa.Y = dw.qp; qa.ldy = H * d;
          DT(3, launch_dec_gemm(qa, kProLn, kDecBias, stream_));
          const int nq_max = cross_absorbed_max_nq(H);
          for (int p0 = 0; p0 < np; p0 += nq_max) {
            CrossAbsorbedArgs ca;
            ca.qp = dw.qp; ca.e = slot.e_planes; ca.e_plane = long(ws_.batch) * T * d; ca.e_scale = sc_cross_kv_.a;
            ca.bf16 = bf;
            if (paired) {
              ca.split = per;
              ca.e2 = member[1]->e_planes;
              if (group > 2) ca.e3 = member[2]->e_planes;
              if (group > 3) ca.e4 = member[3]->e_planes;
            }
            ca.ws = dw.abs_ws; ca.batch = batch; ca.heads = H; ca.d_model = d; ca.T = T; ca.chunks = n_abs;
            ca.nq = std::min(nq_max, np - p0); ca.p0 = p0;
            DT(4, launch_cross_absorbed(ca, stream_));
          }
          DT(8, launch_cross_absorbed_combine(dw.abs_ws, w.cross_wv_t, w.cross_bv, dw.cabs, M, H, n_abs, d, stream_));
          DecGemmArgs co;
          co.bf16 = bf;
          co.Wt = w.cross_wo.w; co.w_scale = w.cross_wo.scale; co.N = d; co.K = d; co.B = batch; co.M = M;
          co.X = dw.cabs; co.ldx = d; co.bias = w.cross_bo; co.R = x; co.Y = x; co.ldy = d;
          DT(5, launch_dec_gemm(co, kProNone, kDecResid, stream_));
        } else {
        CrossAttnArgs ca;
        ca.x = x; ca.ln_g = w.cross_ln_g; ca.ln_b = w.cross_ln_b; ca.wq_t = w.cross_wq_t; ca.bq = w.cross_bq;
        ca.kc = cache_at(slot.cross_kv, (size_t(l) * 2 + 0) * kv_slab); ca.vc = cache_at(slot.cross_kv, (size_t(l) * 2 + 1) * kv_slab);
        ca.bf16 = bf;
        ca.ws = dw.cross_ws; ca.batch = batch; ca.heads = H; ca.T = T; ca.chunks = chunks; ca.nq = np;
        DT(4, launch_cross_attention(ca, stream_));
        DecGemmArgs co;
        co.bf16 = bf;
        co.Wt = w.cross_wo.w; co.w_scale = w.cross_wo.scale; co.N = d; co.K = d; co.B = batch; co.M = M;
        co.cross_ws = dw.cross_ws; co.heads = H; co.chunks = chunks;
        co.bias = w.cross_bo; co.R = x; co.Y = x; co.ldy = d;
        DT(5, launch_dec_gemm(co, kProCombine, kDecResid, stream_));
        }

        DecGemmArgs f1;
        f1.bf16 = bf;
        f1.Wt = w.w1.w; f1.w_scale = w.w1.scale; f1.N = 4 * d; f1.K = d; f1.B = batch; f1.M = M;
        f1.xin = x; f1.ln_g = w.mlp_ln_g; f1.ln_b = w.mlp_ln_b;
        f1.bias = w.b1; f1.Y = dw.hd; f1.ldy = 4 * d;
        DT(6, launch_dec_gemm(f1, kProLn, kDecBiasGelu, stream_));
        DecGemmArgs f2;
        f2.bf16 = bf;
        f2.Wt = w.w2.w; f2.w_scale = w.w2.scale; f2.N = d; f2.K = 4 * d; f2.B = batch; f2.M = M; f2.X = dw.hd; f2.ldx = 4 * d;
        f2.bias = w.b2; f2.R = x; f2.Y = x; f2.ldy = d;
        if (split) {
          f2.Y = dw.xb; f2.ksplit = 2; f2.part = dw.xpart;
        }
        DT(7, launch_dec_gemm(f2, kProNone, kDecResid, stream_));
      }
      if (lang_mode && pos0 == 0) {
        LangWorkspace& lw = lw_[dec_of(si)];
        LanguageHeadArgs la;
        la.x = split ? dw.xb : x; la.xpart = split ? dw.xpart : nullptr; la.ln_g = dec_ln_g; la.ln_b = dec_ln_b;
        la.tok_emb = tok_emb; la.rows = batch; la.d = d; la.n_vocab = V; la.lang_lo = int(kLangLo); la.n_lang = n_lang;
        la.probs = lw.probs; la.lang = lw.lang; la.lang_prob = lw.prob;
        if (lang_mode == 1) la.ids = dw.ids, la.ids_stride = stride, la.id_pos = 1;
        DT(10, launch_language_head(la, stream_));
        if (!pipelined) {
          HIPCHK(hipMemcpyAsync(h_lang_, lw.lang, size_t(batch) * sizeof(int), hipMemcpyDeviceToHost, stream_));
          HIPCHK(hipMemcpyAsync(h_lang_prob_, lw.prob, size_t(batch) * sizeof(float), hipMemcpyDeviceToHost, stream_));
          if (lang_mode == 2) {
            HIPCHK(hipMemcpyAsync(h_lang_probs_, lw.probs, size_t(batch) * n_lang * sizeof(float), hipMemcpyDeviceToHost, stream_));
          }
        }
      }
      if (last >= n_prompt - 1 && lang_mode != 2) {
        const size_t off = size_t(np - 1) * batch * d;
        DecGemmArgs lg;
        lg.bf16 = bf;
        lg.logits_blocks = pipelined ? 256 : 0;
        lg.Wt = (bf ? tok_emb_tiled_bf_ : tok_emb_tiled).w; lg.w_scale = (bf ? tok_emb_tiled_bf_ : tok_emb_tiled).scale; lg.N = V; lg.K = d; lg.B = batch;
        lg.xin = (split ? dw.xb : x) + off; lg.xpart = split ? dw.xpart + off : nullptr; lg.ln_g = dec_ln_g; lg.ln_b = dec_ln_b;
        lg.Y = logits_host ? dw.logits : nullptr; lg.ldy = V; lg.best = dw.best;
        DT(9, launch_dec_gemm(lg, kProLn, kDecLogits, stream_));
        if (logits_host && steps < logits_steps_cap) {
          HIPCHK(hipMemcpy2DAsync(logits_host + size_t(steps) * V, size_t(logits_steps_cap) * V * sizeof(float),
                                  dw.logits, size_t(V) * sizeof(float), size_t(V) * sizeof(float), batch,
                                  hipMemcpyDeviceToHost, stream_));
        }
        DT(10, launch_select_token(dw.best, (V + 31) / 32, dw.ids, stride, last, dw.n_ids, dw.finished,
                            vocab_.token_eot, int(stop_at_eot), batch, stream_, forced));
        ++steps;
      }
    }
    for (int j = 0; j < group; ++j) {
      HIPCHK(hipMemcpyAsync(member[j]->h_ids, dw.ids + size_t(j) * per * stride, size_t(per) * stride * sizeof(long long),
                            hipMemcpyDeviceToHost, stream_));
      HIPCHK(hipMemcpyAsync(member[j]->h_n, dw.n_ids + size_t(j) * per, size_t(per) * sizeof(int), hipMemcpyDeviceToHost, stream_));
    }
  };
  auto key_of = [&](int si) {
    return std::vector<long long>{si, batch, max_pos, n_prompt, chunks, long(stop_at_eot), fc2_ksplit, bf16, absorbed ? 1 : 0, n_abs, group, stream_override, forced ? 1 : 0, pipelined ? 1 : 0, lang_mode};
  };
  if (!absorbed && use_graphs && !logits_host) {
    for (Slot& s : slots_) need_cross_kv(s);
  }
  hipGraphExec_t exec = nullptr;
  if (use_graphs && !logits_host) {
    auto it = graphs_.find(key_of(slot_idx));
    if (it != graphs_.end()) {
      exec = it->second.exec;
      steps = it->second.steps;
    }
  }
  if (exec) {
    HIPCHK(hipGraphLaunch(exec, stream_));
  } else {
    dt_on = dec_timers && !logits_host;
    dt_cls.clear();
    enqueue_all(slot_idx);
    dt_on = false;
    const int eager_steps = steps;
    HIPCHK(hipEventRecord(slot.dec_done, stream_));
    slot.steps = eager_steps;
    for (int j = 1; j < group; ++j) {
      Slot& sb = slots_[(slot_idx + j) % kSlots];
      HIPCHK(hipEventRecord(sb.dec_done, stream_));
      sb.pair_leader = slot_idx, sb.steps = eager_steps, sb.dec = slot.dec;
    }
    if (use_graphs && !logits_host) {
      std::map<std::vector<long long>, GraphEntry> fresh;
      try {
        for (int si = 0; si < kSlots; ++si) {
          hipStream_t cs = dec_stream_at(dec_of(si));
          hipGraph_t graph = nullptr;
          hipGraphExec_t ge = nullptr;
          HIPCHK(hipStreamBeginCapture(cs, hipStreamCaptureModeThreadLocal));
          try {
            enqueue_all(si);
          } catch (...) {
            (void)hipStreamEndCapture(cs, &graph);
            if (graph) (void)hipGraphDestroy(graph);
            throw;
          }
          HIPCHK(hipStreamEndCapture(cs, &graph));
          const hipError_t ie = hipGraphInstantiate(&ge, graph, nullptr, nullptr, 0);
          (void)hipGraphDestroy(graph);
          if (ie != hipSuccess) throw Error(kErrDevice, std::string("hipGraphInstantiate: ") + hipGetErrorString(ie));
          fresh[key_of(si)] = GraphEntry{ge, steps};
        }
        for (auto& g : fresh) graphs_[g.first] = g.second;
      } catch (const std::exception& e) {
        for (auto& g : fresh) (void)hipGraphExecDestroy(g.second.exec);
        (void)hipGetLastError();
        use_graphs = 0;
        std::fprintf(stderr, "[wt] decoder hipGraph capture failed (%s): continuing with eager launches\n", e.what());
      }
    }
    steps = eager_steps;
    return;
  }
  HIPCHK(hipEventRecord(slot.dec_done, stream_));
  slot.steps = steps;
  for (int j = 1; j < group; ++j) {
    Slot& sb = slots_[(slot_idx + j) % kSlots];
    HIPCHK(hipEventRecord(sb.dec_done, stream_));
    sb.pair_leader = slot_idx, sb.steps = steps, sb.dec = slot.dec;
  }
}

#undef DT

void Engine::debug_concurrency(const float* d_mel, int batch, int n_dec, int n_enc, float* dec_ms,
                               float* enc_ms) {
  if (!inflight_.empty()) throw Error(1, "collect the submitted batches first");
  if (n_dec < 0 || n_dec > 4 || n_enc < 0 || n_enc > 4) throw Error(1, "debug_concurrency: 0..4 decodes, 0..4 encoder passes");
  ensure_batch(batch);
  sync();
  for (int i = 0; i < n_dec; ++i)
    if (!slots_[i].used) throw Error(1, "debug_concurrency: run a batch per slot first so every slot holds a cross-KV cache");
  select_stream(true);
  hipEvent_t e0, e1;
  HIPCHK(hipEventCreate(&e0));
  HIPCHK(hipEventCreate(&e1));
  for (int i = 0; i < n_dec; ++i) decode_enqueue(batch, i, nullptr, 0);
// ... 620 lines not shown
```

### whisper.tflite_amd/csrc/engine.h

```cpp
#pragma once
#include <hip/hip_runtime.h>

#include <algorithm>
#include <cstdint>
#include <map>
#include <stdexcept>
#include <string>
#include <vector>

#include "error.h"
#include "host_util.h"
#include "wtw_format.h"

namespace wt {

struct TsPart;
struct TsState;

struct BeamPart;

struct Timings {
  float logmel_ms = 0, encoder_ms = 0, cross_kv_ms = 0, decoder_ms = 0, total_ms = 0;
  int batch = 0, decoder_steps = 0;
};

struct KernelStat {
  const char* name;
  int launches;
  double ms;
  double flops;
  double bytes;
};
enum KernelClass { kKcGemm = 0, kKcEncAttn, kKcLayerNorm, kKcTranspose, kKcGemmAlt, kKcEncAttnAlt, kKcConvert, kKcCount };

struct AttnWeights {
  const float *wqkv = nullptr, *bqkv = nullptr;
  const float *wo = nullptr, *bo = nullptr;
};
struct BlockWeights {
  const float *attn_ln_g, *attn_ln_b;
  AttnWeights attn;
  const float *mlp_ln_g, *mlp_ln_b, *w1, *b1, *w2, *b2;
};
struct TiledW {
  const unsigned short* w = nullptr;
  float scale = 1.0f;
};
struct DecBlockWeights {
  const float *attn_ln_g, *attn_ln_b, *bqkv, *bo;
  TiledW wqkv, wo;
  const float *cross_ln_g, *cross_ln_b, *cross_wq_t, *cross_bq, *cross_bo;
  TiledW cross_wo;
  TiledW wq_abs;
  const float *bq_abs = nullptr, *cross_wv_t = nullptr, *cross_bv = nullptr;
  const float *mlp_ln_g, *mlp_ln_b, *b1, *b2;
  TiledW w1, w2;
};

void check_wtw_file(const std::string& path);

class Engine {
 public:
  Engine(const std::string& model_prefix, const std::string& vocab_path, bool multilingual,
         int device_id, bool monolith = false, const std::string& weights_path = "");
  Engine(const FilterBank& filters, int device_id);
  ~Engine();
  Engine(const Engine&) = delete;
  Engine& operator=(const Engine&) = delete;

  const wtw::Dims& dims() const { return dims_; }
  const VocabData& vocab() const { return vocab_; }
  const FilterBank& filters() const { return filters_; }
  const Timings& timings() const { return timings_; }
  hipStream_t stream() const { return stream_; }
  hipStream_t decoder_stream(int i) const { return dstream_[i % n_dec_streams_]; }

  long language = 2;
  long max_tokens = 30;
  long stop_at_eot = 1;
  long verbose = 0;
  long cross_chunks = 0;
  long attn_variant = 4;
  long fc2_ksplit = 2;
  long use_graphs = 1;
  long cross_absorb = 1;
  long abs_chunks = 0;
  long dec_pair = 1;
  long dec_group = 2;
  long last_batches = 0;
  bool absorb_active() const { return cross_absorb != 0 && (bf16 != 0 || (gemm_variant < 0 && sc_cross_kv_.f16_ok)); }
  bool absorb_for(int batch) const { return absorb_active() && (pipelined_call_ || batch >= 32 || beam_size > 1); }
  long beam_size = 1;
  void check_beam_call(bool logits_tap) const;
  std::vector<float> beam_sum;
  std::vector<int> beam_len;
  bool beam_scores_valid = false;
  static constexpr long kLangLo = 50259;
  int lang_tokens() const;
  void set_language(long value);
  void check_language_call() const;
  void detect_language(int batch, int32_t* lang, float* probs, float* prob);
  std::vector<int> last_lang;
  std::vector<float> last_lang_prob;
  bool last_lang_valid = false;
  long max_positions = 0;
  int full_cap() const { return std::min(dims_.n_text_ctx, 448); }
  void check_full_args(int batch, int ids_stride) const;
  void check_full_call() const;
  void decode_full(int batch, int64_t* ids, int ids_stride, int32_t* n_ids);
  void encode_full(const float* d_mel, int batch);
  long timestamps = 0;
  long max_initial_timestamp = 50;
  bool has_timestamp_tokens() const { return dims_.n_vocab > vocab_.token_beg + 1 && vocab_.token_eot >= 0 && vocab_.token_eot < vocab_.token_beg; }
  void check_timestamp_call() const;
  std::vector<Segment> last_segments;
  std::vector<std::string> last_segment_text;
  bool last_segments_valid = false;
  long gemm_variant = -1;
  long bf16 = 0;
  void set_bf16(bool on);
  long kernel_timers = 1;
  std::vector<long long> prompt_override;
  std::vector<long long> forced_ids;
  std::vector<long long> prompt() const;

  int mel_frames() const { return 2 * dims_.n_audio_ctx; }
  size_t mel_elems() const { return size_t(dims_.n_mels) * mel_frames(); }
  size_t pcm_elems() const { return size_t(mel_frames()) * 160; }

  void logmel(const float* d_pcm, int batch, float* d_mel, int valid_frames = -1);
  void encode(const float* d_mel, int batch);
  void decode(int batch, int64_t* ids, int32_t* n_ids, float* logits_host, int logits_steps_cap);
  void submit(const float* d_mel, int batch);
  void submit_pcm(const float* d_pcm, int batch);
  void collect(int64_t* ids, int32_t* n_ids);
  int in_flight() const { return int(inflight_.size()); }
  int f16_fallbacks() const { return n_f16_fallbacks_; }
  float f16_min_slack_bits() const { return f16_min_slack_bits_; }
  int f16_contractions() const { return int(load_ok_.size()); }
  void set_force_fallback(long mask);
  long force_fallback() const { return force_fallback_; }
  void require_idle() const;
  void sync();
  void bind_device();

  const float* enc_out() const { return ws_.enc_out; }
  void ensure_batch(int batch);
  float* staging_mel(int batch);
  float* staging_pcm(int batch);

  void debug_concurrency(const float* d_mel, int batch, int n_dec, int n_enc, float* dec_ms, float* enc_ms);
  float* dalloc(size_t n_floats);

  const KernelStat* kernel_stats() const { return kstats_; }

 private:
  void open_device();
  void create_streams();
  void release() noexcept;
  void upload_weights(const std::string& path);
  void ensure_bf16_weights();
  std::string weights_path_;
  bool bf16_ready_ = false;
  struct Bf16Encoder {
    const unsigned short *conv1 = nullptr, *conv2 = nullptr, *cross_kv = nullptr;
    int conv1_kpad = 0;
    struct Layer {
      const unsigned short *qkv = nullptr, *out = nullptr, *fc1 = nullptr, *fc2 = nullptr;
    };
// ... 82 lines not shown
    std::vector<int> kt_cls;
    std::vector<double> kt_flops, kt_bytes;
  } slots_[kSlots];
  struct GraphEntry {
    hipGraphExec_t exec;
    int steps;
  };
  void need_cross_kv(Slot& slot);
  std::map<std::vector<long long>, GraphEntry> graphs_;
  hipEvent_t trace_base_ = nullptr;
  int enc_slot_ = 0;
  int last_enc_slot_ = 0;
  std::vector<int> inflight_;
  wtw::Dims dims_{};
  VocabData vocab_;
  FilterBank filters_;
  Timings timings_;
  bool have_logmel_ = false;

  std::vector<void*> allocations_;
  std::map<std::string, const float*> tensors_;

  const float *conv1_w = nullptr, *conv1_b = nullptr, *conv2_w = nullptr, *conv2_b = nullptr;
  int conv1_kpad = 0;
  struct PlaneW {
    const unsigned short* w = nullptr;
  };
  PlaneW conv1_p_, conv2_p_, cross_kv_p_;
  struct EncLayerPlanes {
    PlaneW qkv, out, fc1, fc2;
  };
  std::vector<EncLayerPlanes> enc_planes_;
  PlaneW upload_planes(const float* W, int N, int K, int Kpad, float scale);
  int conv1_kpad_p_ = 0;
  const float* enc_pos = nullptr;
  std::vector<BlockWeights> enc_blocks_;
  std::vector<DecBlockWeights> dec_blocks_;
  std::vector<DecBlockWeights> dec_blocks_bf_;
  TiledW tok_emb_tiled_bf_;
  struct GemmScale {
    float a = 1.0f, w = 64.0f;
    bool f16_ok = true;
  };
  bool gemm_on_planes(const GemmScale& sc) const { return gemm_variant < 0 && sc.f16_ok; }
  struct EncLayerScales {
    GemmScale qkv, out, fc1, fc2;
    float q = 1.0f, k = 1.0f, v = 1.0f;
    bool attn_f16_ok = true;
  };
  static constexpr float kMelBound = 8.0f;
  static constexpr float kF16Slack = 4096.0f;
  int n_f16_fallbacks_ = 0;
  float f16_min_slack_bits_ = 0.0f;
  long force_fallback_ = 0;
  std::vector<bool> load_ok_;
  std::vector<bool*> ok_flags();
  int alt_gemm_variant() const {
    if (gemm_variant >= 0) return int(gemm_variant);
    return (stream_ == stream_masked_ && stream_masked_) ? 16 : 13;
  }
  GemmScale sc_conv1_, sc_conv2_, sc_cross_kv_;
  std::vector<EncLayerScales> sc_layers_;
  const float *enc_ln_post_g = nullptr, *enc_ln_post_b = nullptr;
  const float *cross_kv_w = nullptr, *cross_kv_b = nullptr;
  const float *tok_emb = nullptr, *dec_pos = nullptr, *dec_ln_g = nullptr, *dec_ln_b = nullptr;
  TiledW tok_emb_tiled;
  PlaneW dft_basis_p_;
  const float* dft_zero_bias_ = nullptr;
  float dft_w_scale_ = 1.0f;
  int pw_ld_ = 0;
  long pcm_plane_ = 0;
  static constexpr float kPcmBound = 32.0f;
  const float* mel_w = nullptr;
  int dft_n = 0, dft_k = 0, mel_n = 0, mel_k = 0;

  struct DecWorkspace {
    float *xb = nullptr, *xpart = nullptr;
    float *xd = nullptr, *qkvd = nullptr, *attd = nullptr,
          *hd = nullptr, *cross_ws = nullptr, *self_kv = nullptr, *logits = nullptr;
    float *qp = nullptr, *abs_ws = nullptr, *cabs = nullptr;
    unsigned long long* best = nullptr;
    long long* ids = nullptr;
    int *n_ids = nullptr, *finished = nullptr;
  } dws_[kDecStreams + 1];
  struct LangWorkspace {
    float *probs = nullptr, *prob = nullptr;
    int* lang = nullptr;
  } lw_[kDecStreams + 1];
  float *h_lang_probs_ = nullptr, *h_lang_prob_ = nullptr;
  int* h_lang_ = nullptr;
  void ensure_lang_workspace();
  bool detect_only_ = false;
  struct Workspace {
    int batch = 0;
    float *melT = nullptr, *h1p = nullptr, *x = nullptr, *ln = nullptr, *qkv = nullptr,
          *att = nullptr, *hid = nullptr, *enc_out = nullptr;
    unsigned short *melTp = nullptr, *h1pp = nullptr;
    unsigned short* cvt = nullptr;
    unsigned short* pcm_planes = nullptr;
    float *pw = nullptr, *melacc = nullptr;
    unsigned* clip_max = nullptr;
    float *mel_stage = nullptr, *pcm_stage = nullptr;
    std::vector<void*> owned;
  } ws_;
  bool kt_on_ = true;
  long enc_count_ = 0;
  void kt_begin(int cls, double flops, double bytes);
  void kt_end();
  void resolve_kernel_stats(int slot);
  KernelStat kstats_[kKcCount] = {{"gemm_planes_tile", 0, 0, 0, 0},     {"encoder_attention_planes", 0, 0, 0, 0},
                                  {"layernorm_rows", 0, 0, 0, 0},       {"mel_transpose", 0, 0, 0, 0},
                                  {"gemm_split16_tile", 0, 0, 0, 0},    {"encoder_attention_split", 0, 0, 0, 0},
                                  {"f32_to_planes", 0, 0, 0, 0}};
  int self_cap_ = 32;
  static constexpr int kDecRowsMax = 128;
};

}
```

### whisper.tflite_amd/csrc/k_cross_absorbed.hip

```cpp
#include <hip/hip_runtime.h>

#include <algorithm>

#include "bf16_split.h"
#include "kernels.h"

namespace wt {
namespace {

using f32x4 = __attribute__((ext_vector_type(4))) float;
using half8 = __attribute__((ext_vector_type(8))) _Float16;
using u32x4 = __attribute__((ext_vector_type(4))) unsigned;
using u32x2 = __attribute__((ext_vector_type(2))) unsigned;

struct CrossAbsDev {
  const float* qp;
  const _Float16* e;
  const _Float16* eg[4];
  int split;
  long e_plane;
  float e_scale;
  float* ws;
  int B, H, T, chunks, nq, p0, tiles_per_chunk;
};

constexpr float kDeferA = 3.0f, kPShiftA = 12.0f;

__device__ __forceinline__ unsigned lds_addr(const void* p) {
  return (unsigned)(size_t)(const __attribute__((address_space(3))) unsigned char*)p;
}
struct TrFrag {
  u32x2 h0, h1, g0, g1;
};
__device__ __forceinline__ void ds_read_tr16_x2(unsigned a0, unsigned a1, unsigned b0, unsigned b1, unsigned plane, TrFrag& x,
                                                TrFrag& y) {
  asm volatile(
      "ds_read_b64_tr_b16 %0, %8\n\t"
      "ds_read_b64_tr_b16 %1, %9\n\t"
      "ds_read_b64_tr_b16 %2, %12\n\t"
      "ds_read_b64_tr_b16 %3, %13\n\t"
      "ds_read_b64_tr_b16 %4, %10\n\t"
      "ds_read_b64_tr_b16 %5, %11\n\t"
      "ds_read_b64_tr_b16 %6, %14\n\t"
      "ds_read_b64_tr_b16 %7, %15\n\t"
      "s_waitcnt lgkmcnt(0)"
      : "=&v"(x.h0), "=&v"(x.h1), "=&v"(x.g0), "=&v"(x.g1), "=&v"(y.h0), "=&v"(y.h1), "=&v"(y.g0), "=&v"(y.g1)
      : "v"(a0), "v"(a1), "v"(b0), "v"(b1), "v"(a0 + plane), "v"(a1 + plane), "v"(b0 + plane), "v"(b1 + plane)
      : "memory");
}

__device__ __forceinline__ void ds_read_tr16_x2_one_plane(unsigned a0, unsigned a1, unsigned b0, unsigned b1, TrFrag& x, TrFrag& y) {
  asm volatile(
      "ds_read_b64_tr_b16 %0, %4\n\t"
      "ds_read_b64_tr_b16 %1, %5\n\t"
      "ds_read_b64_tr_b16 %2, %6\n\t"
      "ds_read_b64_tr_b16 %3, %7\n\t"
      "s_waitcnt lgkmcnt(0)"
      : "=&v"(x.h0), "=&v"(x.h1), "=&v"(y.h0), "=&v"(y.h1)
      : "v"(a0), "v"(a1), "v"(b0), "v"(b1)
      : "memory");
}

#ifdef WT_ABS_STAMPS
__device__ long long g_abs_stamps[4096 * 16];
#define ABS_ACC(i)                                    \
  do {                                                \
    const long long t__ = __builtin_readcyclecounter(); \
    ph_[i] += t__ - tl_;                              \
    tl_ = t__;                                        \
  } while (0)
#define ABS_STAMP(i) st_[i] = __builtin_readcyclecounter()
#else
#define ABS_STAMP(i) \
  do {               \
  } while (0)
#define ABS_ACC(i) \
  do {             \
  } while (0)
#endif

template <int DM, int NST, bool BF>
__global__ __launch_bounds__(320) void cross_absorbed_attention(CrossAbsDev a) {
  using bf16x8 = __attribute__((ext_vector_type(8))) __bf16;
  constexpr int P = DM / 128;
  constexpr int kPlane = P * 8192;
  constexpr int NP = BF ? 1 : 2;
  constexpr int kStage = NP * kPlane;
  constexpr int KS = DM / 64;
  constexpr int DT = DM / 64;
  constexpr int IPT = 8 * NP * P;
  extern __shared__ __attribute__((aligned(16))) unsigned char lds[];
  float* const xch = reinterpret_cast<float*>(lds + NST * kStage);
#ifdef WT_ABS_STAMPS
  long long st_[8] = {0, 0, 0, 0, 0, 0, 0, 0};
  long long ph_[6] = {0, 0, 0, 0, 0, 0}, tl_ = 0;
  const long long rt0_ = (long long)__builtin_amdgcn_s_memrealtime();
  ABS_STAMP(0);
#endif

  const int b = blockIdx.x / a.chunks, ck = blockIdx.x % a.chunks;
  const int tid = threadIdx.x, lane = tid & 63, wid = __builtin_amdgcn_readfirstlane(tid >> 6);
  const int qc = lane & 15, lq = lane >> 4;
  const int sub = wid & 1, khalf = wid >> 1;
  const int n_qc = a.nq * a.H;
  const bool q_ok = qc < n_qc;
  const int qpos = q_ok ? qc / a.H : 0, qh_i = q_ok ? qc % a.H : 0;
  const long row = (long)(a.p0 + qpos) * a.B + b;

  const int key_lo = ck * a.tiles_per_chunk * 32;
  int key_hi = key_lo + a.tiles_per_chunk * 32;
  key_hi = key_hi < a.T ? key_hi : a.T;
  const int n_tiles = key_hi > key_lo ? (key_hi - key_lo + 31) / 32 : 0;

  const int eb = b / a.split;
  const _Float16* const ebase = (eb == 0 ? a.e : eb == 1 ? a.eg[1] : eb == 2 ? a.eg[2] : a.eg[3]) + (long)(b - eb * a.split) * a.T * DM;
  const unsigned long long ebytes = reinterpret_cast<unsigned long long>(ebase);
  const unsigned lds_ring = lds_addr(lds);
  const unsigned voff_even = (unsigned)(lq * DM * 2 + (((lane & 15) ^ ((lq & 7) << 1)) << 4));
  const unsigned voff_odd = (unsigned)(lq * DM * 2 + (((lane & 15) ^ (((4 + lq) & 7) << 1)) << 4));
  auto dma_part = [&](int t, int i0, int i1) {
    if (t >= n_tiles) return;
    const int stage = t % NST;
    if (key_lo + t * 32 + 32 <= a.T) {
      const unsigned long long tb = ebytes + (unsigned long long)(key_lo + t * 32) * (DM * 2);
#pragma unroll
      for (int i = i0; i < i1; ++i) {
        const int plane = i / (8 * P), rem = i % (8 * P), panel = rem / 8, kg = rem % 8;
        const unsigned long long sb = tb + (unsigned long long)plane * (unsigned long long)a.e_plane * 2 + (unsigned)((4 * kg * DM + panel * 128) * 2);
        lds_dma16_sgpr((kg & 1) ? voff_odd : voff_even, sb, lds_ring + (unsigned)(stage * kStage + plane * kPlane + panel * 8192 + kg * 1024));
      }
    } else {
      unsigned char* const sbase = lds + stage * kStage;
#pragma unroll
      for (int i = i0; i < i1; ++i) {
        const int plane = i / (8 * P), rem = i % (8 * P), panel = rem / 8, kg = rem % 8;
        const int key = 4 * kg + lq;
        int gk = key_lo + t * 32 + key;
        gk = gk < a.T ? gk : a.T - 1;
        const int chunk = (lane & 15) ^ ((key & 7) << 1);
        __builtin_amdgcn_global_load_lds(
            (const __attribute__((address_space(1))) void*)(ebase + plane * a.e_plane + (long)gk * DM + panel * 128 + chunk * 8),
            (__attribute__((address_space(3))) void*)(sbase + plane * kPlane + panel * 8192 + kg * 1024), 16, 0, 0);
      }
    }
  };

  if (wid == 4) {
    constexpr int kHead = IPT / 3;
    static_assert(NST <= 2 || IPT <= 63, "the counted wait leaves one whole tile in flight: it must fit the 6-bit counter");
#pragma unroll
    for (int st0 = 0; st0 < NST - 1; ++st0) dma_part(st0, 0, IPT);
    for (int t = 0; t < n_tiles; ++t) {
      if (NST > 2 && t + 1 < n_tiles) {
        asm volatile("s_waitcnt vmcnt(%0)" ::"n"(IPT < 63 ? IPT : 63) : "memory");
      } else {
        asm volatile("s_waitcnt vmcnt(0)" ::: "memory");
      }
      __builtin_amdgcn_s_barrier();
      dma_part(t + NST - 1, 0, kHead);
      __builtin_amdgcn_s_barrier();
      dma_part(t + NST - 1, kHead, IPT);
    }
    asm volatile("s_waitcnt vmcnt(0)" ::: "memory");
    return;
// ... 107 lines not shown
    float tmax = fmaxf(fmaxf(fmaxf(s0[0], s0[1]), fmaxf(s0[2], s0[3])), fmaxf(fmaxf(s1[0], s1[1]), fmaxf(s1[2], s1[3])));
    tmax = xor32_max(xor16_max(tmax));
    tmax *= s_inv;
    if (__any(tmax > m_run + kDeferA)) {
      const float m_new = fmaxf(m_run, tmax);
      const float alpha = __builtin_amdgcn_exp2f(m_run - m_new);
      l_run *= alpha;
#pragma unroll
      for (int d = 0; d < DT; ++d) cacc[d] *= alpha;
      m_run = m_new;
    }
    const float shift = kPShiftA - m_run;
    float psum = 0.0f;
#pragma unroll
    for (int r = 0; r < 4; ++r) {
      s0[r] = __builtin_amdgcn_exp2f(fmaf(s0[r], s_inv, shift));
      s1[r] = __builtin_amdgcn_exp2f(fmaf(s1[r], s_inv, shift));
      psum += s0[r] + s1[r];
    }
    psum = xor32_sum(xor16_sum(psum));
    l_run += psum;
    unsigned ph[4], pl[4] = {0, 0, 0, 0};
    if constexpr (BF) {
      ph[0] = pack_bf16x2(s0[0], s0[1]);
      ph[1] = pack_bf16x2(s0[2], s0[3]);
      ph[2] = pack_bf16x2(s1[0], s1[1]);
      ph[3] = pack_bf16x2(s1[2], s1[3]);
    } else {
      split_f16x2(s0[0], s0[1], &ph[0], &pl[0]);
      split_f16x2(s0[2], s0[3], &ph[1], &pl[1]);
      split_f16x2(s1[0], s1[1], &ph[2], &pl[2]);
      split_f16x2(s1[2], s1[3], &ph[3], &pl[3]);
    }
    const half8 pH = __builtin_bit_cast(half8, u32x4{ph[0], ph[1], ph[2], ph[3]});
    const half8 pL = __builtin_bit_cast(half8, u32x4{pl[0], pl[1], pl[2], pl[3]});
    ABS_ACC(4);
    const unsigned sa = lds0 + (unsigned)((t % NST) * kStage);
    const int k0 = 4 * lq + tq, k1 = 16 + 4 * lq + tq;
    static_assert(DT % 2 == 0, "d tiles are read in pairs");
#pragma unroll
    for (int d = 0; d < DT; d += 2) {
      unsigned ad[2][2];
#pragma unroll
      for (int u = 0; u < 2; ++u) {
        const int dtg = wid * DT + d + u;
        const unsigned col = (unsigned)((dtg >> 3) * 8192 + tp * 8);
        ad[u][0] = sa + col + (unsigned)(k0 * 256 + (((dtg & 7) ^ (k0 & 7)) << 5));
        ad[u][1] = sa + col + (unsigned)(k1 * 256 + (((dtg & 7) ^ (k1 & 7)) << 5));
      }
      TrFrag f[2];
      if constexpr (BF) {
        ds_read_tr16_x2_one_plane(ad[0][0], ad[0][1], ad[1][0], ad[1][1], f[0], f[1]);
      } else {
        ds_read_tr16_x2(ad[0][0], ad[0][1], ad[1][0], ad[1][1], (unsigned)kPlane, f[0], f[1]);
      }
#pragma unroll
      for (int u = 0; u < 2; ++u) {
        const half8 eh = __builtin_bit_cast(half8, u32x4{f[u].h0[0], f[u].h0[1], f[u].h1[0], f[u].h1[1]});
        if constexpr (BF) {
          cacc[d + u] = __builtin_amdgcn_mfma_f32_16x16x32_bf16(__builtin_bit_cast(bf16x8, eh), __builtin_bit_cast(bf16x8, pH),
                                                                cacc[d + u], 0, 0, 0);
        } else {
          const half8 el = __builtin_bit_cast(half8, u32x4{f[u].g0[0], f[u].g0[1], f[u].g1[0], f[u].g1[1]});
          cacc[d + u] = __builtin_amdgcn_mfma_f32_16x16x32_f16(eh, pL, cacc[d + u], 0, 0, 0);
          cacc[d + u] = __builtin_amdgcn_mfma_f32_16x16x32_f16(el, pH, cacc[d + u], 0, 0, 0);
          cacc[d + u] = __builtin_amdgcn_mfma_f32_16x16x32_f16(eh, pH, cacc[d + u], 0, 0, 0);
        }
      }
    }
    ABS_ACC(5);
  }

  ABS_STAMP(3);
  if (q_ok) {
    const float cs = 1.0f / (a.e_scale * 4096.0f);
    float* rec = a.ws + ((row * a.H + qh_i) * a.chunks + ck) * (long)(DM + 4);
#pragma unroll
    for (int d = 0; d < DT; ++d) *reinterpret_cast<f32x4*>(rec + 16 * (wid * DT + d) + 4 * lq) = cacc[d] * cs;
    if (wid == 0 && lq == 0) {
      rec[DM] = m_run * 0.69314718055994530942f;
      rec[DM + 1] = l_run * (1.0f / 4096.0f);
    }
  }
#ifdef WT_ABS_STAMPS
  ABS_STAMP(4);
  if (tid == 0 && blockIdx.x < 4096) {
    long long* o = g_abs_stamps + blockIdx.x * 16;
    o[0] = st_[1] - st_[0], o[1] = st_[2] - st_[1], o[2] = st_[3] - st_[2], o[3] = st_[4] - st_[3], o[4] = st_[4] - st_[0];
    o[5] = (long long)__builtin_amdgcn_s_memrealtime() - rt0_;
    o[6] = n_tiles;
    for (int i = 0; i < 6; ++i) o[8 + i] = ph_[i];
  }
#endif
}

__global__ __launch_bounds__(256) void cross_absorbed_combine(const float* __restrict__ ws, const float* __restrict__ wv_t,
                                                              const float* __restrict__ bv, float* __restrict__ out, int H,
                                                              int chunks, int DM) {
  __shared__ __attribute__((aligned(16))) float cs[512];
  __shared__ float part[4][64];
  const long rh = blockIdx.x;
  const int h = (int)(rh % H);
  const float* rec = ws + rh * chunks * (long)(DM + 4);
  const int tid = threadIdx.x;
  float mx = -3.0e38f;
  for (int k = 0; k < chunks; ++k) mx = fmaxf(mx, rec[k * (DM + 4) + DM]);
  if (4 * tid < DM) {
    f32x4 acc = {0, 0, 0, 0};
    float l = 0.0f;
    for (int k = 0; k < chunks; ++k) {
      const float* r = rec + k * (long)(DM + 4);
      const float w = __expf(r[DM] - mx);
      acc += w * *reinterpret_cast<const f32x4*>(r + 4 * tid);
      l += w * r[DM + 1];
    }
    *reinterpret_cast<f32x4*>(&cs[4 * tid]) = acc * (1.0f / l);
  }
  __syncthreads();
  const int j = tid & 63, cq = tid >> 6, c4n = DM / 16;
  const float* w = wv_t + ((long)h * (DM / 4) + cq * c4n) * 256 + j * 4;
  float acc = 0.0f;
  for (int c = 0; c < c4n; ++c) {
    const f32x4 wv = *reinterpret_cast<const f32x4*>(w + (long)c * 256);
    const f32x4 x = *reinterpret_cast<const f32x4*>(&cs[(cq * c4n + c) * 4]);
    acc += (wv[0] * x[0] + wv[1] * x[1]) + (wv[2] * x[2] + wv[3] * x[3]);
  }
  part[cq][j] = acc;
  __syncthreads();
  if (tid < 64) out[(rh / H) * (long)(H * 64) + h * 64 + tid] = ((part[0][tid] + part[1][tid]) + (part[2][tid] + part[3][tid])) + bv[h * 64 + tid];
}

template <int DM, int NST, bool BF = false>
void launch_abs(const CrossAbsDev& g, hipStream_t s) {
  constexpr size_t smem = (size_t)NST * (BF ? 1 : 2) * (DM / 128) * 8192 + 8192;
  static_assert(smem <= 160 * 1024, "ring + exchange buffer fit the CU's LDS");
  static const bool raised = [] {
    (void)hipFuncSetAttribute(reinterpret_cast<const void*>(&cross_absorbed_attention<DM, NST, BF>),
                              hipFuncAttributeMaxDynamicSharedMemorySize, 160 * 1024);
    return true;
  }();
  (void)raised;
  hipLaunchKernelGGL((cross_absorbed_attention<DM, NST, BF>), dim3(g.B * g.chunks), dim3(320), smem, s, g);
}

}

int cross_absorbed_max_nq(int heads) { return heads > 0 ? 16 / heads : 0; }

void launch_cross_absorbed(const CrossAbsorbedArgs& a, hipStream_t s) {
  const int dm = a.d_model;
  if (!a.qp || !a.e || !a.ws || a.batch < 1 || a.heads < 1 || a.heads * 64 != dm || a.T < 1 || a.chunks < 1 || a.chunks > 16 ||
      a.nq < 1 || a.nq * a.heads > 16 || a.p0 < 0 || !(a.e_scale > 0.0f) ||
      (!a.bf16 && a.e_plane < (long)(a.e2 ? std::min(a.split, a.batch) : a.batch) * a.T * dm)) {
    throw Error(kErrInvalidArg, "absorbed cross-attention: shape outside the kernel contract");
  }
  const int tiles = (a.T + 31) / 32;
  const int split = a.e2 ? a.split : a.batch;
  if (split < 1 || split > a.batch) throw Error(kErrInvalidArg, "absorbed cross-attention: bad batch split");
  const int groups = (a.batch + split - 1) / split;
  const unsigned short* src[4] = {a.e, a.e2, a.e3, a.e4};
  if (groups > 4) throw Error(kErrInvalidArg, "absorbed cross-attention: at most four encoder batches per chain");
  for (int i = 0; i < groups; ++i)
    if (!src[i]) throw Error(kErrInvalidArg, "absorbed cross-attention: an encoder batch of the chain has no planes");
  CrossAbsDev g{a.qp, reinterpret_cast<const _Float16*>(a.e),
                {reinterpret_cast<const _Float16*>(a.e), reinterpret_cast<const _Float16*>(src[1] ? src[1] : a.e),
                 reinterpret_cast<const _Float16*>(src[2] ? src[2] : a.e), reinterpret_cast<const _Float16*>(src[3] ? src[3] : a.e)},
                split, a.e_plane, a.bf16 ? 1.0f : a.e_scale, a.ws, a.batch, a.heads, a.T, a.chunks, a.nq, a.p0,
                (tiles + a.chunks - 1) / a.chunks};
  switch (dm) {
    case 128: a.bf16 ? launch_abs<128, 3, true>(g, s) : launch_abs<128, 3>(g, s); break;
    case 384: a.bf16 ? launch_abs<384, 3, true>(g, s) : launch_abs<384, 3>(g, s); break;
    case 512: a.bf16 ? launch_abs<512, 3, true>(g, s) : launch_abs<512, 2>(g, s); break;
    default: throw Error(kErrFormat, "absorbed cross-attention supports d_model 128, 384 or 512");
  }
}

void launch_cross_absorbed_combine(const float* ws, const float* wv_t, const float* bv, float* out, int rows, int heads,
                                   int chunks, int d_model, hipStream_t s) {
  if (!ws || !wv_t || !bv || !out || rows < 1 || heads < 1 || chunks < 1 || d_model != heads * 64 || d_model > 512) {
    throw Error(kErrInvalidArg, "absorbed cross-attention combine: bad shape");
  }
  hipLaunchKernelGGL(cross_absorbed_combine, dim3(rows * heads), dim3(256), 0, s, ws, wv_t, bv, out, heads, chunks, d_model);
}

}
```

### whisper.tflite_amd/csrc/k_decoder.hip

```cpp
#include <hip/hip_runtime.h>

#include <cstdlib>

#include "bf16_split.h"
#include "kernels.h"

namespace wt {
namespace {

using f32x16 = __attribute__((ext_vector_type(16))) float;
using f32x4 = __attribute__((ext_vector_type(4))) float;
using half8 = __attribute__((ext_vector_type(8))) _Float16;

__device__ __forceinline__ float gelu_erf(float x) {
  return 0.5f * x * (1.0f + erff(x * 0.70710678118654752440f));
}
__device__ __forceinline__ unsigned ordered_bits(float v) {
  v = v + 0.0f;
  const unsigned u = __float_as_uint(v);
  return (u & 0x80000000u) ? ~u : (u | 0x80000000u);
}
__device__ __forceinline__ int crow(int r, int h) { return (r & 3) + 8 * (r >> 2) + 4 * h; }

struct DecGemmDev {
  const unsigned short* Wt;
  float w_descale;
  int N, K, M, B;
  const float* X;
  int ldx;
  const float* xin;
  float* xout;
  const float* ln_g;
  const float* ln_b;
  const long long* ids;
  int ids_stride, pos;
  const float* tok_emb;
  const float* pos_emb;
  int n_vocab;
  const float* cross_ws;
  int heads, chunks;
  const float* bias;
  int gelu;
  const float* R;
  float* Y;
  int ldy;
  unsigned long long* best;
  int best_stride;
  int ksplit;
  float* part;
  const float* xpart;
  int lnp_off;
};

struct RowSrc {
  const float* xin;
  const float* xpart;
  const long long* ids;
  int ids_stride, pos, B;
  const float* tok_emb;
  const float* pos_emb;
  int n_vocab;
};

template <int NF4, int LNMODE>
__device__ __forceinline__ void load_row(f32x4 (&v)[NF4], const RowSrc& r, int row, int sub, int K) {
  const float* src = r.xin + (long)row * K;
  int p = 0;
  if (LNMODE == 2) {
    p = row / r.B;
    const int b = row - p * r.B;
    long long id = r.ids[(long)b * r.ids_stride + r.pos + p];
    id = id < 0 ? 0 : (id >= r.n_vocab ? r.n_vocab - 1 : id);
    src = r.tok_emb + id * K;
  }
#pragma unroll
  for (int j = 0; j < NF4; ++j) v[j] = *reinterpret_cast<const f32x4*>(src + (sub + 8 * j) * 4);
  if (LNMODE == 2) {
    const float* pe = r.pos_emb + (long)(r.pos + p) * K;
#pragma unroll
    for (int j = 0; j < NF4; ++j) v[j] += *reinterpret_cast<const f32x4*>(pe + (sub + 8 * j) * 4);
  }
  if (LNMODE == 3) {
    const float* pp = r.xpart + (long)row * K;
#pragma unroll
    for (int j = 0; j < NF4; ++j) v[j] += *reinterpret_cast<const f32x4*>(pp + (sub + 8 * j) * 4);
  }
}

template <int NF4>
__device__ __forceinline__ void row_stats(const f32x4 (&v)[NF4], int K, float* mean, float* rstd) {
  float s = 0.0f;
#pragma unroll
  for (int j = 0; j < NF4; ++j) s += (v[j][0] + v[j][1]) + (v[j][2] + v[j][3]);
  s += __shfl_xor(s, 1, 64);
  s += __shfl_xor(s, 2, 64);
  s += __shfl_xor(s, 4, 64);
  const float m = s / (float)K;
  float q = 0.0f;
#pragma unroll
  for (int j = 0; j < NF4; ++j)
#pragma unroll
    for (int e = 0; e < 4; ++e) {
      const float t = v[j][e] - m;
      q += t * t;
    }
  q += __shfl_xor(q, 1, 64);
  q += __shfl_xor(q, 2, 64);
  q += __shfl_xor(q, 4, 64);
  *mean = m;
  *rstd = rsqrtf(q / (float)K + 1e-5f);
}

template <int PRO, int EPI, int NF4, int LNMODE, int WAVES, int CH, int GT, int SMAX, bool BF>
__global__ __launch_bounds__(WAVES * 64) void dec_gemm(DecGemmDev g) {
  extern __shared__ __attribute__((aligned(16))) float smem[];
  float* const xs = smem;
  float* const red = smem;
  float* const lnp = smem + g.lnp_off;
  const int tid = threadIdx.x, lane = tid & 63, wid = tid >> 6;
  const int l31 = lane & 31, lh = lane >> 5;
  const int n_tiles = (g.N + 31) / 32;
  const int tile = blockIdx.x % n_tiles, khalf = blockIdx.x / n_tiles;
  const int K = g.K, M = g.M, xld = K + 4;
  const int m_tiles = (M + 31) >> 5;

  const int kwave = (K / g.ksplit) / WAVES;
  const int k0 = khalf * (K / g.ksplit) + wid * kwave;
  const int nsteps = kwave >> 4;
  constexpr int WSTEP = BF ? 512 : 1024;
  const unsigned short* wp = g.Wt + ((long)tile * (K >> 4) + (k0 >> 4)) * WSTEP + lane * 8;
  u32x4_t wh[SMAX], wl[BF ? 1 : SMAX];
#pragma unroll
  for (int s = 0; s < SMAX; ++s) {
    const int ss = s < nsteps ? s : nsteps - 1;
// ... 295 lines not shown
#pragma unroll
        for (int e = 0; e < 8; ++e) mx = fmaxf(mx, fabsf(xa[s][e]));
      mx = fmaxf(mx, __shfl_xor(mx, 32, 64));
      const unsigned ex = (__float_as_uint(mx) >> 23) & 0xFFu;
      const float sc = ex < 32u ? 1.0f : __uint_as_float((268u - ex) << 23);
      inv = ex < 32u ? 1.0f : __uint_as_float((ex - 14u) << 23);
#pragma unroll
      for (int s = 0; s < KS; ++s) {
        u32x4_t pl[3];
        split8_f16x2(xa[s], sc, pl);
        ah[s] = pl[0];
        al[s] = pl[1];
      }
    }
  }
  if (LNMODE >= 0) __syncthreads();
  float rscale[16];
#pragma unroll
  for (int r = 0; r < 16; ++r) rscale[r] = BF ? 1.0f : __shfl(inv, crow(r, lh), 64) * g.w_descale;

  for (int par = 0; tile < n_tiles; tile += gridDim.x, par ^= 1) {
    const int nt = tile + (int)gridDim.x < n_tiles ? tile + (int)gridDim.x : tile;
    const unsigned short* np = wbase + (long)nt * tile_stride;
    u32x4_t nwh[KS], nwl[BF ? 1 : KS];
#pragma unroll
    for (int s = 0; s < KS; ++s) {
      nwh[s] = *reinterpret_cast<const u32x4_t*>(np + (long)s * WSTEP);
      if (!BF) nwl[s] = *reinterpret_cast<const u32x4_t*>(np + (long)s * WSTEP + 512);
    }
    f32x16 part;
#pragma unroll
    for (int r = 0; r < 16; ++r) part[r] = 0.0f;
#pragma unroll
    for (int s = 0; s < KS; ++s) {
      if (BF) {
        using bf16x8 = __attribute__((ext_vector_type(8))) __bf16;
        part = __builtin_amdgcn_mfma_f32_32x32x16_bf16(__builtin_bit_cast(bf16x8, ah[s]), __builtin_bit_cast(bf16x8, wh[s]), part, 0, 0, 0);
      } else {
        const half8 a_h = __builtin_bit_cast(half8, ah[s]), a_l = __builtin_bit_cast(half8, al[BF ? 0 : s]);
        const half8 b_h = __builtin_bit_cast(half8, wh[s]), b_l = __builtin_bit_cast(half8, wl[BF ? 0 : s]);
        part = __builtin_amdgcn_mfma_f32_32x32x16_f16(a_h, b_l, part, 0, 0, 0);
        part = __builtin_amdgcn_mfma_f32_32x32x16_f16(a_l, b_h, part, 0, 0, 0);
        part = __builtin_amdgcn_mfma_f32_32x32x16_f16(a_h, b_h, part, 0, 0, 0);
      }
    }
#pragma unroll
    for (int r = 0; r < 16; ++r) red[par][wid][r][lane] = BF ? part[r] : 0.0f + part[r] * rscale[r];
    __syncthreads();
    {
      const int n_epi = tile * 32 + l31;
      const bool n_ok = n_epi < g.N;
#pragma unroll
      for (int rr = 0; rr < 4; ++rr) {
        const int r = wid * 4 + rr;
        float v = red[par][0][r][lane];
        v += red[par][1][r][lane];
        v += red[par][2][r][lane];
        v += red[par][3][r][lane];
        v += 0.0f;
        const int m = m0 + crow(r, lh);
        const bool ok = n_ok && m < M;
        if (ok && g.Y) g.Y[(long)m * g.ldy + n_epi] = v;
        const unsigned key = ok ? ordered_bits(v) : 0u;
        unsigned kmax = key;
#pragma unroll
        for (int off = 16; off >= 1; off >>= 1) {
          const unsigned o2 = __shfl_xor(kmax, off, 64);
          kmax = o2 > kmax ? o2 : kmax;
        }
        const unsigned long long hit = __ballot(ok && key == kmax);
        const unsigned half_hits = (unsigned)(hit >> (32 * lh));
        if (l31 == 0 && m < M) {
          const unsigned col = half_hits ? (unsigned)(tile * 32 + 31 - __clz(half_hits)) : 0u;
          g.best[(long)m * g.best_stride + tile] = half_hits ? (((unsigned long long)kmax << 32) | col) : 0ull;
        }
      }
    }
#pragma unroll
    for (int s = 0; s < KS; ++s) {
      wh[s] = nwh[s];
      if (!BF) wl[s] = nwl[s];
    }
  }
}

template <bool BF, int LNMODE>
bool launch_logits_persistent(const DecGemmDev& g, hipStream_t s, int blocks = 0) {
  if (g.K % 64 != 0 || g.ksplit != 1) return false;
  const int n_tiles = (g.N + 31) / 32, m_tiles = (g.M + 31) / 32;
  static const int forced = [] {
    const char* v = getenv("WT_LOGITS_BLOCKS");
    const int n = v ? atoi(v) : 0;
    return n >= 32 && n <= 1024 ? n : 0;
  }();
  const int total = forced ? forced : (blocks >= 32 && blocks <= 1024 ? blocks : 512);
  const int per = total / m_tiles;
  const dim3 grid(n_tiles < per ? n_tiles : per, m_tiles);
  switch (g.K / 64) {
    case 2: hipLaunchKernelGGL((dec_logits_persistent<2, BF, LNMODE>), grid, dim3(256), 0, s, g); return true;
    case 6: hipLaunchKernelGGL((dec_logits_persistent<6, BF, LNMODE>), grid, dim3(256), 0, s, g); return true;
    case 8: hipLaunchKernelGGL((dec_logits_persistent<8, BF, LNMODE>), grid, dim3(256), 0, s, g); return true;
    default: return false;
  }
}

template <int NF4, int LNMODE>
__global__ __launch_bounds__(256) void dec_finalize_ln(RowSrc src, const float* __restrict__ g,
                                                       const float* __restrict__ b,
                                                       float* __restrict__ y, int B, int K) {
  const int lane = threadIdx.x & 63, wid = threadIdx.x >> 6;
  const int r8 = lane >> 3, sub = lane & 7;
  const int row = blockIdx.x * 32 + wid * 8 + r8;
  if (row >= B) return;
  f32x4 v[NF4], gg[NF4], bb[NF4];
#pragma unroll
  for (int j = 0; j < NF4; ++j) {
    gg[j] = *reinterpret_cast<const f32x4*>(g + (sub + 8 * j) * 4);
    bb[j] = *reinterpret_cast<const f32x4*>(b + (sub + 8 * j) * 4);
  }
  load_row<NF4, LNMODE>(v, src, row, sub, K);
  float mean, rstd;
  row_stats<NF4>(v, K, &mean, &rstd);
#pragma unroll
  for (int j = 0; j < NF4; ++j) {
    const int c = (sub + 8 * j) * 4;
    f32x4 o;
#pragma unroll
    for (int e = 0; e < 4; ++e) o[e] = (v[j][e] - mean) * rstd * gg[j][e] + bb[j][e];
    *reinterpret_cast<f32x4*>(y + (long)row * K + c) = o;
  }
}

template <int PRO, int EPI, int NF4, int LNMODE, int WAVES, int CH, int GT, int SMAX, bool BF>
void launch_one(const DecGemmDev& g, size_t smem, dim3 grid, hipStream_t s) {
  static const bool raised = [] {
    (void)hipFuncSetAttribute(reinterpret_cast<const void*>(&dec_gemm<PRO, EPI, NF4, LNMODE, WAVES, CH, GT, SMAX, BF>),
                              hipFuncAttributeMaxDynamicSharedMemorySize, 160 * 1024);
    return true;
  }();
  (void)raised;
  hipLaunchKernelGGL((dec_gemm<PRO, EPI, NF4, LNMODE, WAVES, CH, GT, SMAX, BF>), grid, dim3(WAVES * 64), smem, s, g);
}

template <int PRO, int EPI, int NF4, int LNMODE, int WAVES, int CH, int GT, bool BF>
void launch_steps(DecGemmDev g, hipStream_t s) {
  const int n_tiles = (g.N + 31) / 32;
  const dim3 grid(n_tiles * (PRO == kProNone && EPI == kDecResid ? g.ksplit : 1));
  const size_t red_bytes = (size_t)WAVES * GT * 16 * 64 * sizeof(float);
  const size_t xs_bytes = PRO == kProLn ? (size_t)GT * 32 * (g.K + 4) * sizeof(float) : 0;
  const size_t body = red_bytes > xs_bytes ? red_bytes : xs_bytes;
  g.lnp_off = (int)(body / sizeof(float));
  const size_t smem = body + (PRO == kProLn ? (size_t)2 * g.K * sizeof(float) : 0);
  const int nsteps = (g.K / g.ksplit) / WAVES / 16;
  if (nsteps <= 2) launch_one<PRO, EPI, NF4, LNMODE, WAVES, CH, GT, 2, BF>(g, smem, grid, s);
  else if (nsteps == 3) launch_one<PRO, EPI, NF4, LNMODE, WAVES, CH, GT, 3, BF>(g, smem, grid, s);
  else if (nsteps == 4) launch_one<PRO, EPI, NF4, LNMODE, WAVES, CH, GT, 4, BF>(g, smem, grid, s);
  else if (nsteps <= 6) launch_one<PRO, EPI, NF4, LNMODE, WAVES, CH, GT, 6, BF>(g, smem, grid, s);
  else launch_one<PRO, EPI, NF4, LNMODE, WAVES, CH, GT, 8, BF>(g, smem, grid, s);
}

template <int PRO, int EPI, int NF4, int LNMODE, int WAVES, int CH, bool BF>
void launch_gt(const DecGemmDev& g, hipStream_t s) {
  const bool two = g.M > 32 && !(PRO == kProLn && g.K > 512);
  if (two) {
    launch_steps<PRO, EPI, NF4, LNMODE, WAVES, CH, 2, BF>(g, s);
  } else {
    launch_steps<PRO, EPI, NF4, LNMODE, WAVES, CH, 1, BF>(g, s);
  }
}

template <int LNMODE, bool BF>
void launch_ln(const DecGemmDev& g, hipStream_t s) {
  switch (g.K) {
    case 128: launch_gt<kProLn, kDecBias, 4, LNMODE, 4, 1, BF>(g, s); break;
    case 384: launch_gt<kProLn, kDecBias, 12, LNMODE, 4, 1, BF>(g, s); break;
    case 512: launch_gt<kProLn, kDecBias, 16, LNMODE, 4, 1, BF>(g, s); break;
    default: throw Error(kErrFormat, "decoder kernels support d_model 128, 384 or 512");
  }
}

}

template <bool BF>
static void dispatch_dec_gemm(const DecGemmArgs& a, const DecGemmDev& g, int pro, int epi, hipStream_t s) {
  if (pro == kProLn && epi == kDecLogits) {
    if (a.ids || !a.xin || !a.ln_g || !a.ln_b) throw Error(kErrInvalidArg, "logits GEMM: LayerNorm rows come from xin (+ xpart)");
    const bool ok = a.xpart ? launch_logits_persistent<BF, 3>(g, s, a.logits_blocks) : launch_logits_persistent<BF, 0>(g, s, a.logits_blocks);
    if (!ok) throw Error(kErrInvalidArg, "logits GEMM with the LayerNorm prologue: K must be a multiple of 64");
    return;
  }
  if (pro == kProLn) {
    if (epi != kDecBias) throw Error(kErrInvalidArg, "decoder GEMM: the LayerNorm prologue pairs with the bias epilogue");
    if (a.ids) {
      if (a.xpart) throw Error(kErrInvalidArg, "decoder GEMM: embedding rows have no pending partial");
      launch_ln<2, BF>(g, s);
    } else if (a.xpart) {
      launch_ln<3, BF>(g, s);
    } else {
      launch_ln<0, BF>(g, s);
    }
    return;
  }
  const int key = pro * 8 + epi;
  switch (key) {
    case kProNone * 8 + kDecResid: launch_gt<kProNone, kDecResid, 0, 0, 8, 1, BF>(g, s); break;
    case kProNone * 8 + kDecBias: launch_gt<kProNone, kDecBias, 0, 0, 4, 1, BF>(g, s); break;
    case kProNone * 8 + kDecLogits:
      if (!launch_logits_persistent<BF, -1>(g, s, a.logits_blocks)) launch_gt<kProNone, kDecLogits, 0, 0, 4, 1, BF>(g, s);
      break;
    case kProCombine * 8 + kDecResid:
      switch (a.chunks) {
        case 1: launch_gt<kProCombine, kDecResid, 0, 0, 8, 1, BF>(g, s); break;
        case 2: launch_gt<kProCombine, kDecResid, 0, 0, 8, 2, BF>(g, s); break;
        case 4: launch_gt<kProCombine, kDecResid, 0, 0, 8, 4, BF>(g, s); break;
        case 8: launch_gt<kProCombine, kDecResid, 0, 0, 8, 8, BF>(g, s); break;
        default: throw Error(kErrInvalidArg, "cross_chunks must be 1, 2, 4 or 8");
      }
      break;
    default: throw Error(kErrInvalidArg, "unsupported decoder GEMM prologue / epilogue pair");
  }
}

void launch_dec_gemm(const DecGemmArgs& a, int pro, int epi, hipStream_t s) {
  const int gelu = epi == kDecBiasGelu ? 1 : 0;
  if (epi == kDecBiasGelu) epi = kDecBias;
  const int M = a.M > 0 ? a.M : a.B;
  const int ksplit = a.ksplit > 0 ? a.ksplit : 1;
  DecGemmDev g{a.Wt,      1.0f / a.w_scale, a.N,  a.K,       M,         a.B,     a.X,     a.ldx,   a.xin,  a.xout,
               a.ln_g,    a.ln_b,    a.ids,      a.ids_stride, a.pos,   a.tok_emb, a.pos_emb, a.n_vocab,
               a.cross_ws, a.heads,  a.chunks,   a.bias,    gelu,      a.R,     a.Y,     a.ldy,   a.best,
               a.best_stride > 0 ? a.best_stride : (a.N + 31) / 32, ksplit, a.part,  a.xpart, 0};
  const bool resid = epi == kDecResid;
  const int waves = resid ? 8 : 4;
  const int kblock = a.K / ksplit;
  if (!a.Wt || a.B < 1 || M < a.B || M > 128 || M % a.B != 0 || a.K > 4096 || a.K % 16 != 0 || !(a.w_scale > 0.0f) ||
      ksplit > 2 || kblock % (16 * waves) != 0 ||
      (pro == kProCombine && a.K != a.heads * 64) || (resid && (!a.R || !a.Y))) {
    throw Error(kErrInvalidArg, "decoder GEMM shape outside the kernel contract");
  }
  if (ksplit != 1 && !(pro == kProNone && epi == kDecResid && a.part && a.R != a.Y)) {
    throw Error(kErrInvalidArg, "decoder GEMM: K split needs the out-of-place residual form");
  }
  if (a.bf16) {
    dispatch_dec_gemm<true>(a, g, pro, epi, s);
  } else {
    dispatch_dec_gemm<false>(a, g, pro, epi, s);
  }
}

template <int LNMODE>
static void launch_finalize_mode(const RowSrc& src, const float* g, const float* b, float* y, int B, int K,
                                 hipStream_t s) {
  const dim3 grid((B + 31) / 32);
  switch (K) {
    case 128: hipLaunchKernelGGL((dec_finalize_ln<4, LNMODE>), grid, dim3(256), 0, s, src, g, b, y, B, K); break;
    case 384: hipLaunchKernelGGL((dec_finalize_ln<12, LNMODE>), grid, dim3(256), 0, s, src, g, b, y, B, K); break;
    case 512: hipLaunchKernelGGL((dec_finalize_ln<16, LNMODE>), grid, dim3(256), 0, s, src, g, b, y, B, K); break;
    default: throw Error(kErrFormat, "decoder kernels support d_model 128, 384 or 512");
  }
}

void launch_dec_finalize_ln(const float* xin, const float* g, const float* b, float* y, int B, int K,
                            hipStream_t s, const float* xpart) {
  const RowSrc src{xin, xpart, nullptr, 0, 0, B, nullptr, nullptr, 0};
  if (xpart) {
    launch_finalize_mode<3>(src, g, b, y, B, K, s);
  } else {
    launch_finalize_mode<0>(src, g, b, y, B, K, s);
  }
}

}
```

### whisper.tflite_amd/csrc/k_misc.hip

```cpp
#include <hip/hip_runtime.h>

#include <algorithm>

#include "bf16_split.h"
#include "kernels.h"

namespace wt {
namespace {

__device__ __forceinline__ float wave_sum(float v) {
#pragma unroll
  for (int off = 32; off >= 1; off >>= 1) v += __shfl_xor(v, off, 64);
  return v;
}

template <int PER>
__global__ __launch_bounds__(256) void layernorm_rows(const float* __restrict__ x,
                                                      float* __restrict__ y,
                                                      const float* __restrict__ g,
                                                      const float* __restrict__ b, int M, int d,
                                                      int* __restrict__ nonfinite) {
  const int lane = threadIdx.x & 63;
  const long row = (long)blockIdx.x * 4 + (threadIdx.x >> 6);
  if (row >= M) return;
  const float* xr = x + row * d;
  float v[PER];
  float s = 0.0f;
#pragma unroll
  for (int i = 0; i < PER; ++i) {
    const int c = lane + 64 * i;
    v[i] = c < d ? xr[c] : 0.0f;
    s += v[i];
  }
  const float mean = wave_sum(s) / (float)d;
  float q = 0.0f;
#pragma unroll
  for (int i = 0; i < PER; ++i) {
    const int c = lane + 64 * i;
    const float t = c < d ? v[i] - mean : 0.0f;
    q += t * t;
  }
  const float var = wave_sum(q) / (float)d;
  if (nonfinite != nullptr && lane == 0 && !(fabsf(mean) <= 3.0e38f && var <= 3.0e38f)) atomicOr(nonfinite, 1);
  const float rstd = rsqrtf(var + 1e-5f);
  float* yr = y + row * d;
#pragma unroll
  for (int i = 0; i < PER; ++i) {
    const int c = lane + 64 * i;
    if (c < d) yr[c] = (v[i] - mean) * rstd * g[c] + b[c];
  }
}

template <int PER, bool BF>
__global__ __launch_bounds__(256) void layernorm_rows_planes(const float* __restrict__ x, _Float16* __restrict__ yp,
                                                             long plane, float scale, float* __restrict__ y32,
                                                             const float* __restrict__ g, const float* __restrict__ b,
                                                             int M, int d, int* __restrict__ nonfinite) {
  using f32x4 = __attribute__((ext_vector_type(4))) float;
  using half4 = __attribute__((ext_vector_type(4))) _Float16;
  const int l32 = threadIdx.x & 31;
  const long row = (long)blockIdx.x * 8 + (threadIdx.x >> 5);
  if (row >= M) return;
  const float* xr = x + row * d;
  f32x4 v[PER], gg[PER], bb[PER];
  float s = 0.0f;
#pragma unroll
  for (int i = 0; i < PER; ++i) {
    const int c = (l32 + 32 * i) * 4;
    v[i] = *reinterpret_cast<const f32x4*>(xr + c);
    gg[i] = *reinterpret_cast<const f32x4*>(g + c);
    bb[i] = *reinterpret_cast<const f32x4*>(b + c);
    s += (v[i][0] + v[i][1]) + (v[i][2] + v[i][3]);
  }
#pragma unroll
  for (int off = 16; off >= 1; off >>= 1) s += __shfl_xor(s, off, 64);
  const float mean = s / (float)d;
  float q = 0.0f;
#pragma unroll
  for (int i = 0; i < PER; ++i)
#pragma unroll
    for (int e = 0; e < 4; ++e) {
      const float t = v[i][e] - mean;
      q += t * t;
    }
#pragma unroll
  for (int off = 16; off >= 1; off >>= 1) q += __shfl_xor(q, off, 64);
  const float var = q / (float)d;
// ... 130 lines not shown
                                                   int T, int t_valid) {
  __shared__ float tile[32][33];
  __shared__ unsigned smax;
  const int b = blockIdx.z, t0 = blockIdx.x * 32, c0 = blockIdx.y * 32;
  const int tx = threadIdx.x & 31, ty = threadIdx.x >> 5;
  if (threadIdx.x == 0) smax = 0u;
  __syncthreads();
  unsigned lmax = 0u;
  float e4[4];
#pragma unroll
  for (int i = 0; i < 4; ++i) {
    const int t = t0 + ty + 8 * i, c = c0 + tx;
    e4[i] = melacc[((long)b * T + (t < T ? t : T - 1)) * ld + (c < ld ? c : ld - 1)];
  }
#pragma unroll
  for (int i = 0; i < 4; ++i) {
    const int t = t0 + ty + 8 * i, c = c0 + tx;
    float v = 0.0f;
    if (t < T && c < n_mel) {
      float e = e4[i];
      e = e < 1e-10f ? 1e-10f : e;
      const float l2 = __builtin_amdgcn_logf(e);
      v = fmaf(l2, 0.30102999566f, l2 * -1.4320989e-8f);
      if (e <= 1e-10f) v = -10.0f;
      const unsigned o = ordered_bits(v);
      if (t < t_valid) lmax = o > lmax ? o : lmax;
    }
    tile[ty + 8 * i][tx] = v;
  }
#pragma unroll
  for (int off = 32; off >= 1; off >>= 1) {
    const unsigned o = __shfl_xor(lmax, off, 64);
    lmax = o > lmax ? o : lmax;
  }
  if ((threadIdx.x & 63) != 0) lmax = 0u;
  atomicMax(&smax, lmax);
  __syncthreads();
#pragma unroll
  for (int i = 0; i < 4; ++i) {
    const int c = c0 + ty + 8 * i, t = t0 + tx;
    if (c < n_mel && t < T) logmel[((long)b * n_mel + c) * T + t] = tile[tx][ty + 8 * i];
  }
  if (threadIdx.x == 0 && smax != 0u) atomicMax(&clip_max[((long)b * kClipMaxWays + (blockIdx.x % kClipMaxWays)) * kClipMaxStride], smax);
}

__global__ __launch_bounds__(256) void mel_normalize(float* __restrict__ logmel,
                                                     const unsigned* __restrict__ clip_max,
                                                     long per_clip) {
  const int b = blockIdx.y;
  unsigned mx = 0u;
  for (int w = 0; w < kClipMaxWays; ++w) {
    const unsigned o = clip_max[((long)b * kClipMaxWays + w) * kClipMaxStride];
    mx = o > mx ? o : mx;
  }
  const double floor_v = (double)from_ordered(mx) - 8.0;
  float* p = logmel + (long)b * per_clip;
  for (long i = (long)blockIdx.x * 256 + threadIdx.x; i < per_clip; i += (long)gridDim.x * 256) {
    float v = p[i];
    if ((double)v < floor_v) v = (float)floor_v;
    p[i] = (float)(((double)v + 4.0) / 4.0);
  }
}

__global__ __launch_bounds__(256) void select_token(const unsigned long long* __restrict__ best,
                                                    int n_tiles, long long* ids, int ids_stride,
                                                    int pos, int* n_ids, int* finished, long long eot,
                                                    int stop_at_eot, int keep_ids) {
  __shared__ unsigned long long wmax[4];
  const int b = blockIdx.x;
  unsigned long long p = 0ull;
  for (int t = threadIdx.x; t < n_tiles; t += 256) {
    const unsigned long long v = best[(long)b * n_tiles + t];
    p = v > p ? v : p;
  }
#pragma unroll
  for (int off = 32; off >= 1; off >>= 1) {
    const unsigned long long o = __shfl_xor(p, off, 64);
    p = o > p ? o : p;
  }
  if ((threadIdx.x & 63) == 0) wmax[threadIdx.x >> 6] = p;
  __syncthreads();
  if (threadIdx.x != 0) return;
  for (int w = 1; w < 4; ++w) p = wmax[w] > p ? wmax[w] : p;
  const long long tok = (long long)(unsigned)(p & 0xffffffffull);
  if (!keep_ids) ids[(long)b * ids_stride + pos + 1] = tok;
  if (!finished[b]) {
    n_ids[b] = pos + 2;
    if (stop_at_eot && tok == eot) finished[b] = 1;
  }
}

__device__ __forceinline__ float block_sum_256(float v, float* red) {
#pragma unroll
  for (int off = 32; off >= 1; off >>= 1) v += __shfl_xor(v, off, 64);
  __syncthreads();
  if ((threadIdx.x & 63) == 0) red[threadIdx.x >> 6] = v;
  __syncthreads();
  return ((red[0] + red[1]) + red[2]) + red[3];
}

__global__ __launch_bounds__(256) void language_head(const float* __restrict__ x, const float* __restrict__ xpart,
                                                     const float* __restrict__ g, const float* __restrict__ bta,
                                                     const float* __restrict__ tok_emb, int d, int lang_lo, int n_lang,
                                                     float* __restrict__ probs, int* __restrict__ lang,
                                                     float* __restrict__ lang_prob, long long* ids, int ids_stride,
                                                     int id_pos, int forced_lang) {
  __shared__ float ys[kLangMaxD];
  __shared__ float zs[kLangMax];
  __shared__ float red[4];
  const int b = blockIdx.x, tid = threadIdx.x, lane = tid & 63, wave = tid >> 6;
  const float* row = x + (long)b * d;
  const float* prow = xpart ? xpart + (long)b * d : nullptr;
  float s = 0.0f;
  for (int i = tid; i < d; i += 256) {
    const float v = prow ? row[i] + prow[i] : row[i];
    ys[i] = v;
    s += v;
  }
  const float mean = block_sum_256(s, red) / (float)d;
  float q = 0.0f;
  for (int i = tid; i < d; i += 256) {
    const float t = ys[i] - mean;
    q += t * t;
  }
  const float rstd = rsqrtf(block_sum_256(q, red) / (float)d + 1e-5f);
  for (int i = tid; i < d; i += 256) ys[i] = (ys[i] - mean) * rstd * g[i] + bta[i];
  __syncthreads();
  for (int r = wave; r < n_lang; r += 4) {
    const float* e = tok_emb + (long)(lang_lo + r) * d;
    float acc = 0.0f;
    for (int i = lane; i < d; i += 64) acc = fmaf(ys[i], e[i], acc);
#pragma unroll
    for (int off = 32; off >= 1; off >>= 1) acc += __shfl_xor(acc, off, 64);
    if (lane == 0) zs[r] = acc;
  }
  __syncthreads();
  if (wave != 0) return;
  float bz = -INFINITY;
  int bi = -1;
  for (int r = lane; r < n_lang; r += 64) {
    if (zs[r] >= bz) bz = zs[r], bi = r;
  }
#pragma unroll
  for (int off = 32; off >= 1; off >>= 1) {
    const float oz = __shfl_xor(bz, off, 64);
    const int oi = __shfl_xor(bi, off, 64);
    if (oz > bz || (oz == bz && oi > bi)) bz = oz, bi = oi;
  }
  float sum = 0.0f;
  for (int r = lane; r < n_lang; r += 64) sum += expf(zs[r] - bz);
#pragma unroll
  for (int off = 32; off >= 1; off >>= 1) sum += __shfl_xor(sum, off, 64);
  const float inv = 1.0f / sum;
  for (int r = lane; r < n_lang; r += 64) probs[(long)b * n_lang + r] = expf(zs[r] - bz) * inv;
  if (lane != 0) return;
  if (forced_lang >= 0) bi = forced_lang < n_lang ? forced_lang : n_lang - 1;
  bi = bi < 0 ? 0 : bi;
  lang[b] = bi;
  lang_prob[b] = expf(zs[bi] - bz) * inv;
  if (ids) ids[(long)b * ids_stride + id_pos] = (long long)lang_lo + bi;
}

}

void launch_language_head(const LanguageHeadArgs& a, hipStream_t s) {
  if (a.rows < 1 || a.d < 1 || a.d > kLangMaxD || a.n_lang < 1 || a.n_lang > kLangMax || a.lang_lo < 0 ||
      long(a.lang_lo) + a.n_lang > long(a.n_vocab) || !a.x || !a.ln_g || !a.ln_b || !a.tok_emb || !a.probs || !a.lang ||
      !a.lang_prob || a.forced_lang >= a.n_lang || (a.ids && (a.id_pos < 0 || a.id_pos >= a.ids_stride))) {
    throw Error(kErrInvalidArg, "language_head: bad shape or language range");
  }
  hipLaunchKernelGGL(language_head, dim3(a.rows), dim3(256), 0, s, a.x, a.xpart, a.ln_g, a.ln_b, a.tok_emb, a.d, a.lang_lo,
                     a.n_lang, a.probs, a.lang, a.lang_prob, a.ids, a.ids_stride, a.id_pos, a.forced_lang < 0 ? -1 : a.forced_lang);
// ... 122 lines not shown
```

### whisper.tflite_amd/csrc/kernels.h

```cpp
#pragma once
#include <hip/hip_runtime.h>
#include <hip/hip_ext.h>

#include <cstdint>
#include <vector>

#include "error.h"

namespace wt {

struct LaunchTimer {
  hipEvent_t start = nullptr, stop = nullptr;
};
extern thread_local LaunchTimer g_launch_timer;

#define WT_LAUNCH_TIMED(kernel, grid, block, smem, stream, ...)                                                      \
  do {                                                                                                                \
    if (::wt::g_launch_timer.start) {                                                                                 \
      hipExtLaunchKernelGGL(kernel, grid, block, smem, stream, ::wt::g_launch_timer.start, ::wt::g_launch_timer.stop, \
                            0, __VA_ARGS__);                                                                          \
    } else {                                                                                                          \
      hipLaunchKernelGGL(kernel, grid, block, smem, stream, __VA_ARGS__);                                             \
    }                                                                                                                 \
  } while (0)
// ... 28 lines not shown
};
void launch_gemm(const GemmArgs& a, int epi, hipStream_t s);
float f16_scale_for(float bound);
int gemm_occupancy(int variant);
bool gemm_variant_supported(int variant);

struct PlaneGemmArgs {
  const unsigned short* A = nullptr;
  long a_plane = 0;
  const unsigned short* W = nullptr;
  float* C = nullptr;
  unsigned short* P = nullptr;
  long p_plane = 0;
  const float* bias = nullptr;
  const float* R = nullptr;
  const float* pos = nullptr;
  int M = 0, N = 0, K = 0;
  int a_rpb = 1 << 30;
  long a_bs = 0;
  int lda = 0;
  int c_rpb = 1 << 30;
  long c_bs = 0;
  int ldc = 0;
  int pos_period = 1;
  int kv_batch = 0, kv_heads = 0, kv_dmodel = 0;
  float a_scale = 1.0f, w_scale = 1.0f;
  float out_scale[3] = {1.0f, 1.0f, 1.0f};
  int seg = 0;
  int n_cu = 256;
  const float *ln_g = nullptr, *ln_b = nullptr;
  unsigned short* ln_P = nullptr;
  long ln_plane = 0;
  float ln_scale = 1.0f;
  float* ln_y32 = nullptr;
  int* nonfinite = nullptr;
};
bool launch_gemm_planes(const PlaneGemmArgs& a, int epi, hipStream_t s);
int plane_gemm_mode();
void set_plane_gemm_mode(int m);
bool launch_gemm_bf16_planes(const PlaneGemmArgs& a, int epi, hipStream_t s);
std::vector<unsigned short> round_weights_bf16(const float* W, int N, int K, int Kpad);
std::vector<unsigned short> split_weight_planes(const float* W, int N, int K, int Kpad, float scale);

enum DecPro : int {
  kProNone = 0,
  kProLn = 1,
  kProCombine = 2
};
enum DecEpi : int {
  kDecResid = 0,
  kDecBias = 1,
  kDecBiasGelu = 2,
  kDecLogits = 3
};
struct DecGemmArgs {
  int logits_blocks = 0;
  const unsigned short* Wt = nullptr;
  float w_scale = 1.0f;
  int N = 0, K = 0, B = 0;
  int M = 0;
  const float* X = nullptr;
  int ldx = 0;
  const float* xin = nullptr;
  float* xout = nullptr;
  const float* ln_g = nullptr;
  const float* ln_b = nullptr;
  const long long* ids = nullptr;
  int ids_stride = 0, pos = 0;
  const float* tok_emb = nullptr;
  const float* pos_emb = nullptr;
  int n_vocab = 0;
  const float* cross_ws = nullptr;
  int heads = 0, chunks = 0;
  const float* bias = nullptr;
  const float* R = nullptr;
  float* Y = nullptr;
  int ldy = 0;
  unsigned long long* best = nullptr;
  int best_stride = 0;
  int ksplit = 1;
  float* part = nullptr;
  const float* xpart = nullptr;
  bool bf16 = false;
};
void launch_dec_gemm(const DecGemmArgs& a, int pro, int epi, hipStream_t s);
void launch_dec_finalize_ln(const float* xin, const float* g, const float* b, float* y, int B, int K,
                            hipStream_t s, const float* xpart = nullptr);

void launch_layernorm(const float* x, float* y, const float* g, const float* b, int M, int d,
                      hipStream_t s, int* nonfinite = nullptr);
void launch_layernorm_planes(const float* x, unsigned short* yp, long plane, float scale, float* y32, const float* g,
                             const float* b, int M, int d, hipStream_t s, int* nonfinite = nullptr, bool bf16 = false);

void launch_spin(int microseconds, hipStream_t s);

void launch_f32_to_planes(const float* x, unsigned short* yp, long plane, long M, int ld, const float* scales, int seg,
                          hipStream_t s);
void launch_pcm_to_planes(const float* pcm, unsigned short* yp, long plane, float scale, float limit, int batch, long n,
                          long out_stride, hipStream_t s);

void launch_encoder_attention(const float* qkv, float* out, int batch, int T, int heads, int variant,
                              hipStream_t stream, float q_scale = 1.0f, float k_scale = 1.0f, float v_scale = 1.0f);
void launch_encoder_attention_planes(const unsigned short* qkv, long plane, unsigned short* out, long out_plane,
                                     int batch, int T, int heads, float q_scale, float k_scale, float v_scale,
                                     float out_scale, hipStream_t stream);
void launch_encoder_attention_bf16(const unsigned short* qkv, unsigned short* out, int batch, int T, int heads,
                                   hipStream_t stream);

void launch_chain_probe(float* p, int blocks, hipStream_t stream);
void launch_mel_transpose(const float* mel, float* melT, int batch, int n_mels, int T,
                          hipStream_t s);
void launch_mel_transpose_planes(const float* mel, unsigned short* out, long plane, float scale, int batch, int n_mels,
                                 int T, int ld, hipStream_t s, bool bf16 = false);
constexpr int kClipMaxStride = 32, kClipMaxWays = 4;
void launch_log_clipmax(const float* melacc, int ld, float* logmel, unsigned* clip_max, int batch,
                        int n_mel, int T, hipStream_t s, int t_valid = -1);
void launch_mel_normalize(float* logmel, const unsigned* clip_max, int batch, int n_mel, int T,
                          hipStream_t s);

void launch_self_attention(const float* qkv, void* kcache, void* vcache, int cap, int pos0, int npos, float* out,
                           int batch, int heads, hipStream_t s, bool bf16 = false);
constexpr int kSelfLongCap = 448;
void check_self_attention_long(int cap, int pos, int batch, int heads);
void launch_self_attention_long(const float* qkv, float* kcache, float* vcache, int cap, int pos, float* out, int batch,
                                int heads, hipStream_t s);
struct CrossAttnArgs {
  const float* x = nullptr;
  const float *ln_g = nullptr, *ln_b = nullptr, *wq_t = nullptr, *bq = nullptr;
  const void *kc = nullptr, *vc = nullptr;
  float* ws = nullptr;
  int batch = 0, heads = 0, T = 0, chunks = 1, nq = 1;
  bool bf16 = false;
};
void launch_cross_attention(const CrossAttnArgs& a, hipStream_t s);
struct CrossAbsorbedArgs {
  const float* qp = nullptr;
  const unsigned short* e = nullptr;
  const unsigned short* e2 = nullptr;
  const unsigned short* e3 = nullptr;
  const unsigned short* e4 = nullptr;
  int split = 0;
  long e_plane = 0;
  float e_scale = 1.0f;
  float* ws = nullptr;
  int batch = 0, heads = 0, d_model = 0, T = 0, chunks = 1, nq = 1, p0 = 0;
  bool bf16 = false;
};
void launch_cross_absorbed(const CrossAbsorbedArgs& a, hipStream_t s);
int cross_absorbed_max_nq(int heads);
void launch_cross_absorbed_combine(const float* ws, const float* wv_t, const float* bv, float* out, int rows, int heads,
                                   int chunks, int d_model, hipStream_t s);
void launch_select_token(const unsigned long long* best, int n_tiles, long long* ids, int ids_stride,
                         int pos, int* n_ids, int* finished, long long eot, int stop_at_eot, int batch,
                         hipStream_t s, bool keep_ids = false);

constexpr int kLangMax = 128;
constexpr int kLangMaxD = 1280;
struct LanguageHeadArgs {
  const float *x = nullptr, *xpart = nullptr, *ln_g = nullptr, *ln_b = nullptr;
  const float* tok_emb = nullptr;
  int rows = 0, d = 0, n_vocab = 0, lang_lo = 0, n_lang = 0;
  float* probs = nullptr;
  int* lang = nullptr;
  float* lang_prob = nullptr;
  long long* ids = nullptr;
  int ids_stride = 0, id_pos = 1, forced_lang = -1;
};
void launch_language_head(const LanguageHeadArgs& a, hipStream_t s);

constexpr int kBeamMax = 8;
constexpr int kBeamChunk = 4096;
constexpr int kBeamMaxChunks = 16;
constexpr int kBeamClipsMax = 64;
struct BeamPart {
  float m, s;
  unsigned long long key[kBeamMax + 1];
};
int beam_chunks(int n_vocab);
void launch_beam_topk(const float* logits, int ldl, int V, int rows, int kk, BeamPart* part, hipStream_t s);
struct BeamStepArgs {
  const BeamPart* part = nullptr;
  int n_chunks = 0;
  const long long* ids = nullptr;
  int clips = 0, K = 0, n_live = 0, pos = 0, n_prompt = 0, V = 0, c0 = 0;
  long long eot = 0;
  float* live_sum = nullptr;
  int* fin_tok = nullptr;
  float* fin_sum = nullptr;
  int *fin_len = nullptr, *n_fin = nullptr, *done = nullptr;
  int* parent = nullptr;
  long long* token = nullptr;
};
void launch_beam_select(const BeamStepArgs& a, hipStream_t s);
struct BeamReorderArgs {
  const float* kv_src = nullptr;
  float* kv_dst = nullptr;
  int src_rows = 0, dst_rows = 0, cap = 0, d = 0, slabs = 0, pos = 0, V = 0;
  const long long* ids_src = nullptr;
  long long* ids_dst = nullptr;
  const int* parent = nullptr;
  const long long* token = nullptr;
};
void launch_beam_reorder(const BeamReorderArgs& a, hipStream_t s);
struct BeamFinalArgs {
  const long long* ids = nullptr;
  int clips = 0, K = 0, c0 = 0, pos = 0, n_prompt = 0;
  const float* live_sum = nullptr;
  int* fin_tok = nullptr;
  float* fin_sum = nullptr;
  int *fin_len = nullptr, *n_fin = nullptr;
  const int* done = nullptr;
  long long* out_ids = nullptr;
  int* out_n = nullptr;
  float* out_sum = nullptr;
  int* out_len = nullptr;
};
void launch_beam_finalize(const BeamFinalArgs& a, hipStream_t s);

constexpr int kTsChunk = 4096;
constexpr int kTsMaxChunks = 64;
struct TsState {
  int tick;
  int last_is_ts, prev_is_ts;
};
struct TsPart {
  unsigned long long key_text, key_ts;
  float m, s;
};
int ts_chunks(int n_vocab);
// ... 25 lines not shown
```

Before: 150,200 audio-sec/s.

## Fuse absorbed cross-attention combine and token select into producer kernels via tickets

Adds a last-block-done ticket tail to the absorbed cross-attention kernel, so the final chunk block for each clip performs the wv combine itself and the separate combine kernel is skipped. Adds a similar tail to the logits GEMM, where the last block reduces the per-tile argmax records and runs the greedy token step, replacing the separate select_token launch. The aim is to cut two kernel launches and their serialization gaps per decoder step. In exchange it adds atomics and fences, a serial tail in a single block, and a ticket buffer that the kernel must reset itself. The path is gated by a dec_fuse engine option and only applies to the non-bf16 path.

After: 147,500 audio-sec/s. 0.982x the previous value.

```diff
diff --git a/include/wt_debug.h b/include/wt_debug.h
--- a/include/wt_debug.h
+++ b/include/wt_debug.h
@@ -40,6 +40,12 @@
 int wt_dbg_cross_absorbed_chain(wt_engine* h, int bf16, int batch, int heads, int T, int chunks, int nq, int split, int n_src,
                                 const float* const* E_src, const float* qp, const float* wv, const float* bv, int mode,
                                 int p0_only, int nq_only, float* out, float* ws);
+int wt_dbg_cross_absorbed_chain_fused(wt_engine* h, int batch, int heads, int T, int chunks, int nq, int split, int n_src,
+                                      const float* const* E_src, const float* qp, const float* wv, const float* bv, int repeat,
+                                      float* out, float* ws, uint32_t* tickets);
+int wt_dbg_dec_logits_select(wt_engine* h, int fused, int M, int V, int K, const float* xin, const float* ln_g, const float* ln_b,
+                             const float* E, int blocks, int repeat, uint64_t* records, int64_t* ids, int stride, int pos,
+                             int32_t* n_ids, int32_t* finished, int64_t eot, int stop_at_eot, int keep_ids, uint32_t* ticket);
 int wt_dbg_absorbed_query_matrix(int heads, int d, const float* wq, const float* bq, const float* wk, float* A, float* av);
 int wt_dbg_self_attention(wt_engine* h, int batch, int heads, int cap, int pos, int npos, const float* qkv,
                           float* kcache, float* vcache, float* out);
diff --git a/whisper.tflite_amd/__init__.py b/whisper.tflite_amd/__init__.py
--- a/whisper.tflite_amd/__init__.py
+++ b/whisper.tflite_amd/__init__.py
@@ -4,7 +4,7 @@
 import enum
 import os
 from ctypes import (POINTER, byref, c_char_p, c_float, c_int, c_int32, c_int64, c_long, c_size_t,
-                    c_uint64, c_void_p)
+                    c_uint32, c_uint64, c_void_p)
 
 import numpy as np
 
@@ -41,7 +41,7 @@
     "wt_dbg_self_attention_bf16", "wt_dbg_cross_attention_bf16", "wt_dbg_encoder_attention_planes", "wt_dbg_gemm_bf16", "wt_dbg_gemm_bf16_ln", "wt_dbg_encoder_attention_bf16",
     "wt_dbg_beam_topk", "wt_dbg_beam_step", "wt_dbg_beam_reorder", "wt_dbg_beam_finalize",
     "wt_dbg_dec_gemm_ksplit", "wt_dbg_dec_ln_gemm_rows", "wt_dbg_dec_logits", "wt_dbg_select_token",
-    "wt_dbg_cross_absorbed_chain", "wt_dbg_absorbed_query_matrix", "wt_dbg_language_head", "wt_dbg_self_attention_long",
+    "wt_dbg_cross_absorbed_chain", "wt_dbg_cross_absorbed_chain_fused", "wt_dbg_dec_logits_select", "wt_dbg_absorbed_query_matrix", "wt_dbg_language_head", "wt_dbg_self_attention_long",
     "wt_dbg_timestamp_select",
 ]
 
@@ -137,6 +137,10 @@
         L.wt_dbg_cross_absorbed_bf16.argtypes = L.wt_dbg_cross_absorbed.argtypes
         L.wt_dbg_cross_absorbed_chain.argtypes = [c_void_p, c_int, c_int, c_int, c_int, c_int, c_int, c_int, c_int, POINTER(fp),
                                                   fp, fp, fp, c_int, c_int, c_int, fp, fp]
+        L.wt_dbg_cross_absorbed_chain_fused.argtypes = [c_void_p, c_int, c_int, c_int, c_int, c_int, c_int, c_int, POINTER(fp),
+                                                        fp, fp, fp, c_int, fp, fp, POINTER(c_uint32)]
+        L.wt_dbg_dec_logits_select.argtypes = [c_void_p, c_int, c_int, c_int, c_int, fp, fp, fp, fp, c_int, c_int, POINTER(c_uint64), ip64,
+                                               c_int, c_int, ip32, ip32, c_int64, c_int, c_int, POINTER(c_uint32)]
         L.wt_dbg_absorbed_query_matrix.argtypes = [c_int, c_int, fp, fp, fp, fp, fp]
         L.wt_dbg_gemm_planes_ln.argtypes = [c_void_p, c_int, c_int, fp, fp, fp, fp, fp, c_int, c_int, fp, fp, c_int, fp, fp, fp,
                                             POINTER(c_int)]
@@ -666,6 +670,37 @@
             _fp(wv), _fp(bv), mode, p0, n1, _fp(out), _fp(ws)))
         return out, ws
 
+    def dbg_cross_absorbed_chain_fused(self, qp, E_src, wv, bv, batch, heads, T, chunks, nq, split=None, repeat=1,
+                                       ws_fill=-7.0, out_fill=-9.0):
+        d, rows = heads * 64, nq * batch
+        wv, bv, qp = _f32(wv), _f32(bv), _f32(qp)
+        srcs = [_f32(e) for e in E_src]
+        ws = np.full((rows + 1, heads, chunks, d + 4), ws_fill, np.float32)
+        out = np.full((rows + 1, d), out_fill, np.float32)
+        tickets = np.full(batch + 1, 0xFFFFFFFF, np.uint32)
+        ptrs = (POINTER(c_float) * len(srcs))(*[_fp(e) for e in srcs])
+        self._check(lib().wt_dbg_cross_absorbed_chain_fused(
+            self._h, batch, heads, T, chunks, nq, batch if split is None else split, len(srcs), ptrs, _fp(qp), _fp(wv), _fp(bv),
+            repeat, _fp(out), _fp(ws), tickets.ctypes.data_as(POINTER(c_uint32))))
+        return out, ws, tickets
+
+    def dbg_dec_logits_select(self, fused, xin, ln_g, ln_b, E, ids, pos, n_ids, finished, eot, stop_at_eot=True,
+                              keep_ids=False, blocks=0, repeat=1):
+        xin, E, ln_g, ln_b = _f32(xin), _f32(E), _f32(ln_g), _f32(ln_b)
+        M, K = xin.shape
+        V = E.shape[0]
+        ids = np.array(ids, np.int64)
+        g_ids = np.concatenate([ids, np.full((1, ids.shape[1]), -77, np.int64)])
+        g_n = np.concatenate([np.array(n_ids, np.int32), np.array([-77], np.int32)])
+        g_fin = np.concatenate([np.array(finished, np.int32), np.array([-77], np.int32)])
+        records = np.full((M + 1, (V + 31) // 32), 0x7777777777777777, np.uint64)
+        ticket = np.full(2, 0xFFFFFFFF, np.uint32)
+        self._check(lib().wt_dbg_dec_logits_select(
+            self._h, int(fused), M, V, K, _fp(xin), _fp(ln_g), _fp(ln_b), _fp(E), blocks, repeat,
+            records.ctypes.data_as(POINTER(c_uint64)), _ip64(g_ids), ids.shape[1], pos, _ip32(g_n), _ip32(g_fin), int(eot),
+            int(stop_at_eot), int(keep_ids), ticket.ctypes.data_as(POINTER(c_uint32))))
+        return records, g_ids, g_n, g_fin, ticket
+
     def dbg_encoder_attention_planes(self, qkv, batch, T, heads, iters=0):
         qkv = _f32(qkv)
         out = np.zeros((batch * T, heads * 64), np.float32)
diff --git a/whisper.tflite_amd/csrc/capi.cpp b/whisper.tflite_amd/csrc/capi.cpp
--- a/whisper.tflite_amd/csrc/capi.cpp
+++ b/whisper.tflite_amd/csrc/capi.cpp
@@ -233,6 +233,9 @@
     if (h->impl->in_flight() > 0) return fail(h, WT_ERR_INVALID_ARG, "collect the submitted batches before changing dec_group");
     if (value < 2 || value > 4) return fail(h, WT_ERR_INVALID_ARG, "dec_group: 2, 3 or 4 batches per decoder chain (dec_pair = 0 turns grouping off)");
     e.dec_group = value;
+  } else if (k == "dec_fuse") {
+    if (value != 0 && value != 1) return fail(h, WT_ERR_INVALID_ARG, "dec_fuse must be 0 or 1");
+    e.dec_fuse = value;
   } else if (k == "abs_chunks") {
     if (value < 0 || value > 16) return fail(h, WT_ERR_INVALID_ARG, "abs_chunks must be 0 (automatic) or 1..16");
     e.abs_chunks = value;
@@ -290,6 +293,8 @@
   else if (k == "use_graphs") *value = e.use_graphs;
   else if (k == "cross_absorb") *value = e.cross_absorb;
   else if (k == "abs_chunks") *value = e.abs_chunks;
+  else if (k == "dec_fuse") *value = e.dec_fuse;
+  else if (k == "dec_fuse_active") *value = e.dec_fuse_active_;
   else if (k == "dec_pair") *value = e.dec_pair;
   else if (k == "dec_group") *value = e.dec_group;
   else if (k == "last_batches") *value = e.last_batches;
@@ -1993,9 +1998,9 @@
   });
 }
 
-int wt_dbg_cross_absorbed_chain(wt_engine* h, int bf16, int batch, int heads, int T, int chunks, int nq, int split, int n_src,
-                                const float* const* E_src, const float* qp, const float* wv, const float* bv, int mode,
-                                int p0_only, int nq_only, float* out, float* ws) {
+static int abs_chain_impl(wt_engine* h, int bf16, int batch, int heads, int T, int chunks, int nq, int split, int n_src,
+                          const float* const* E_src, const float* qp, const float* wv, const float* bv, int mode,
+                          int p0_only, int nq_only, float* out, float* ws, int fused, int repeat, uint32_t* tickets) {
   if (!h || !wv || !bv || !out || !ws || batch < 1 || heads < 1 || heads > 8 || T < 1 || nq < 1 || chunks < 1 || chunks > 16 ||
       size_t(nq) * batch > 128 || mode < 0 || mode > 2) {
     return WT_ERR_INVALID_ARG;
@@ -2012,6 +2017,9 @@
     const std::vector<float> wvt = wt::cross_q_layout(wv, int(d));
     DevArr<float> dwv(wvt.size(), wvt.data()), dbv(d, bv), dq(mode != 2 ? rows * heads * d : 0, qp);
     DevArr<float> dws((rows + 1) * heads * chunks * (d + 4), ws), dout((rows + 1) * d, out);
+    std::vector<unsigned> zeros(size_t(batch) + 1, 0u);
+    zeros.back() = 0xFFFFFFFFu;
+    DevArr<unsigned> dtick(zeros.size(), zeros.data());
     hipStream_t st = h->impl->stream();
     const size_t plane = size_t(batch) * clip + 64;
     std::vector<std::unique_ptr<DevArr<unsigned short>>> src;
@@ -2047,18 +2055,75 @@
           if (n_src > 3) a.e4 = src[3]->p;
         }
         a.batch = batch; a.heads = heads; a.d_model = int(d); a.T = T; a.chunks = chunks; a.nq = n; a.p0 = p0;
+        if (fused) a.wv_t = dwv.p, a.bv = dbv.p, a.out = dout.p, a.tickets = dtick.p;
         wt::launch_cross_absorbed(a, st);
       };
-      if (mode == 1) {
-        launch(p0_only, nq_only);
-      } else {
-        for (int p0 = 0; p0 < nq; p0 += nq_max) launch(p0, std::min(nq_max, nq - p0));
+      for (int rep = 0; rep < repeat; ++rep) {
+        if (rep > 0) hipchk(hipMemsetAsync(dout.p, 0xFF, rows * d * sizeof(float), st), "memset");
+        if (mode == 1) {
+          launch(p0_only, nq_only);
+        } else {
+          for (int p0 = 0; p0 < nq; p0 += nq_max) launch(p0, std::min(nq_max, nq - p0));
+        }
       }
     }
-    wt::launch_cross_absorbed_combine(dws.p, dwv.p, dbv.p, dout.p, int(rows), heads, chunks, int(d), st);
+    if (!fused) wt::launch_cross_absorbed_combine(dws.p, dwv.p, dbv.p, dout.p, int(rows), heads, chunks, int(d), st);
     h->impl->sync();
     dout.to_host(out);
     dws.to_host(ws);
+    if (tickets) dtick.to_host(tickets);
+  });
+}
+
+int wt_dbg_cross_absorbed_chain(wt_engine* h, int bf16, int batch, int heads, int T, int chunks, int nq, int split, int n_src,
+                                const float* const* E_src, const float* qp, const float* wv, const float* bv, int mode,
+                                int p0_only, int nq_only, float* out, float* ws) {
+  return abs_chain_impl(h, bf16, batch, heads, T, chunks, nq, split, n_src, E_src, qp, wv, bv, mode, p0_only, nq_only, out, ws, 0, 1,
+                        nullptr);
+}
+
+int wt_dbg_cross_absorbed_chain_fused(wt_engine* h, int batch, int heads, int T, int chunks, int nq, int split, int n_src,
+                                      const float* const* E_src, const float* qp, const float* wv, const float* bv, int repeat,
+                                      float* out, float* ws, uint32_t* tickets) {
+  if (repeat < 1 || repeat > 4 || !tickets) return WT_ERR_INVALID_ARG;
+  return abs_chain_impl(h, 0, batch, heads, T, chunks, nq, split, n_src, E_src, qp, wv, bv, 0, 0, 0, out, ws, 1, repeat, tickets);
+}
+
+int wt_dbg_dec_logits_select(wt_engine* h, int fused, int M, int V, int K, const float* xin, const float* ln_g, const float* ln_b,
+                             const float* E, int blocks, int repeat, uint64_t* records, int64_t* ids, int stride, int pos,
+                             int32_t* n_ids, int32_t* finished, int64_t eot, int stop_at_eot, int keep_ids, uint32_t* ticket) {
+  if (!h || !xin || !ln_g || !ln_b || !E || !records || !ids || !n_ids || !finished || !ticket || M < 1 || M > 128 || V < 1 ||
+      blocks < 0 || (K != 128 && K != 384 && K != 512) || pos < 0 || pos + 1 >= stride || repeat < 1 || repeat > 4) {
+    return WT_ERR_INVALID_ARG;
+  }
+  return guarded(h, [&] {
+    const int n_tiles = (V + 31) / 32;
+    const DevTiled dE(E, V, K, false);
+    DevArr<float> dxin(size_t(M) * K, xin), dg(K, ln_g), db(K, ln_b);
+    DevArr<unsigned long long> dBest((size_t(M) + 1) * n_tiles, reinterpret_cast<const unsigned long long*>(records));
+    DevArr<long long> dids((size_t(M) + 1) * stride, reinterpret_cast<const long long*>(ids));
+    DevArr<int> dn(size_t(M) + 1, n_ids), dfin(size_t(M) + 1, finished);
+    const unsigned zero[2] = {0u, 0xFFFFFFFFu};
+    DevArr<unsigned> dtick(2, zero);
+    hipStream_t st = h->impl->stream();
+    wt::DecGemmArgs g;
+    g.logits_blocks = blocks;
+    g.Wt = dE.w(); g.w_scale = dE.scale; g.N = V; g.K = K; g.B = M; g.M = M;
+    g.xin = dxin.p; g.ln_g = dg.p; g.ln_b = db.p; g.ldy = V; g.best = dBest.p;
+    if (fused) {
+      g.sel_ticket = dtick.p; g.sel_ids = dids.p; g.sel_stride = stride; g.sel_pos = pos; g.sel_n_ids = dn.p;
+      g.sel_finished = dfin.p; g.sel_eot = eot; g.sel_stop = stop_at_eot; g.sel_keep = keep_ids != 0;
+    }
+    for (int rep = 0; rep < repeat; ++rep) {
+      wt::launch_dec_gemm(g, wt::kProLn, wt::kDecLogits, st);
+      if (!fused) wt::launch_select_token(dBest.p, n_tiles, dids.p, stride, pos, dn.p, dfin.p, eot, stop_at_eot, M, st, keep_ids != 0);
+    }
+    h->impl->sync();
+    dBest.to_host(reinterpret_cast<unsigned long long*>(records));
+    dids.to_host(reinterpret_cast<long long*>(ids));
+    dn.to_host(n_ids);
+    dfin.to_host(finished);
+    dtick.to_host(ticket);
   });
 }
 
diff --git a/whisper.tflite_amd/csrc/dec_select.h b/whisper.tflite_amd/csrc/dec_select.h
--- /dev/null
+++ b/whisper.tflite_amd/csrc/dec_select.h
@@ -0,0 +1,16 @@
+#pragma once
+#include <hip/hip_runtime.h>
+
+namespace wt {
+
+__device__ __forceinline__ void greedy_step(unsigned long long p, int b, long long* ids, int ids_stride, int pos, int* n_ids,
+                                            int* finished, long long eot, int stop_at_eot, int keep_ids) {
+  const long long tok = (long long)(unsigned)(p & 0xffffffffull);
+  if (!keep_ids) ids[(long)b * ids_stride + pos + 1] = tok;
+  if (!finished[b]) {
+    n_ids[b] = pos + 2;
+    if (stop_at_eot && tok == eot) finished[b] = 1;
+  }
+}
+
+}
diff --git a/whisper.tflite_amd/csrc/engine.cpp b/whisper.tflite_amd/csrc/engine.cpp
--- a/whisper.tflite_amd/csrc/engine.cpp
+++ b/whisper.tflite_amd/csrc/engine.cpp
@@ -934,6 +934,7 @@
     dw.ids = reinterpret_cast<long long*>(alloc(B * 32 * 2, true));
     dw.n_ids = reinterpret_cast<int*>(alloc(B, true));
     dw.finished = reinterpret_cast<int*>(alloc(B, true));
+    dw.tickets = reinterpret_cast<unsigned*>(alloc(R + 32, true));
   }
   ws_.mel_stage = alloc(B * mel_elems(), false);
   ws_.batch = batch;
@@ -1716,6 +1717,8 @@
   const int abs_blocks = pipelined ? (bf16 ? 64 : 128) : 256;
   int n_abs = abs_chunks > 0 ? int(abs_chunks) : std::min(16, std::max(1, (abs_blocks + batch - 1) / batch));
   n_abs = std::min(n_abs, (T + 31) / 32);
+  const bool fuse = dec_fuse != 0 && bf16 == 0;
+  dec_fuse_active_ = fuse ? (absorbed ? 3 : 2) : 0;
   int steps = 0;
   static const bool dec_timers = getenv("WT_DEC_KERNEL_TIMERS") != nullptr;
   std::vector<hipEvent_t>& dt_ev = slot.dt_events;
@@ -1754,6 +1757,9 @@
     HIPCHK(hipMemsetAsync(dw.finished, 0, size_t(batch) * sizeof(int), stream_));
 
     const bool bf = bf16 != 0;
+    const bool fuse_abs = fuse && absorbed, fuse_sel = fuse;
+    unsigned* const clip_tickets = dw.tickets;
+    unsigned* const sel_ticket = dw.tickets + std::max<size_t>(size_t(ws_.batch), kDecRowsMax);
     const size_t kv_slab = size_t(batch) * T * d;
     const size_t self_slab = size_t(batch) * self_cap_ * d;
     auto cache_at = [&](float* base, size_t elems) -> void* {
@@ -1810,9 +1816,10 @@
             }
             ca.ws = dw.abs_ws; ca.batch = batch; ca.heads = H; ca.d_model = d; ca.T = T; ca.chunks = n_abs;
             ca.nq = std::min(nq_max, np - p0); ca.p0 = p0;
+            if (fuse_abs) ca.wv_t = w.cross_wv_t, ca.bv = w.cross_bv, ca.out = dw.cabs, ca.tickets = clip_tickets;
             DT(4, launch_cross_absorbed(ca, stream_));
           }
-          DT(8, launch_cross_absorbed_combine(dw.abs_ws, w.cross_wv_t, w.cross_bv, dw.cabs, M, H, n_abs, d, stream_));
+          if (!fuse_abs) DT(8, launch_cross_absorbed_combine(dw.abs_ws, w.cross_wv_t, w.cross_bv, dw.cabs, M, H, n_abs, d, stream_));
           DecGemmArgs co;
           co.bf16 = bf;
           co.Wt = w.cross_wo.w; co.w_scale = w.cross_wo.scale; co.N = d; co.K = d; co.B = batch; co.M = M;
@@ -1872,14 +1879,20 @@
         lg.Wt = (bf ? tok_emb_tiled_bf_ : tok_emb_tiled).w; lg.w_scale = (bf ? tok_emb_tiled_bf_ : tok_emb_tiled).scale; lg.N = V; lg.K = d; lg.B = batch;
         lg.xin = (split ? dw.xb : x) + off; lg.xpart = split ? dw.xpart + off : nullptr; lg.ln_g = dec_ln_g; lg.ln_b = dec_ln_b;
         lg.Y = logits_host ? dw.logits : nullptr; lg.ldy = V; lg.best = dw.best;
+        if (fuse_sel) {
+          lg.sel_ticket = sel_ticket; lg.sel_ids = dw.ids; lg.sel_stride = stride; lg.sel_pos = last; lg.sel_n_ids = dw.n_ids;
+          lg.sel_finished = dw.finished; lg.sel_eot = vocab_.token_eot; lg.sel_stop = int(stop_at_eot); lg.sel_keep = forced;
+        }
         DT(9, launch_dec_gemm(lg, kProLn, kDecLogits, stream_));
         if (logits_host && steps < logits_steps_cap) {
           HIPCHK(hipMemcpy2DAsync(logits_host + size_t(steps) * V, size_t(logits_steps_cap) * V * sizeof(float),
                                   dw.logits, size_t(V) * sizeof(float), size_t(V) * sizeof(float), batch,
                                   hipMemcpyDeviceToHost, stream_));
         }
-        DT(10, launch_select_token(dw.best, (V + 31) / 32, dw.ids, stride, last, dw.n_ids, dw.finished,
-                            vocab_.token_eot, int(stop_at_eot), batch, stream_, forced));
+        if (!fuse_sel) {
+          DT(10, launch_select_token(dw.best, (V + 31) / 32, dw.ids, stride, last, dw.n_ids, dw.finished,
+                              vocab_.token_eot, int(stop_at_eot), batch, stream_, forced));
+        }
         ++steps;
       }
     }
@@ -1890,7 +1903,7 @@
     }
   };
   auto key_of = [&](int si) {
-    return std::vector<long long>{si, batch, max_pos, n_prompt, chunks, long(stop_at_eot), fc2_ksplit, bf16, absorbed ? 1 : 0, n_abs, group, stream_override, forced ? 1 : 0, pipelined ? 1 : 0, lang_mode};
+    return std::vector<long long>{si, batch, max_pos, n_prompt, chunks, long(stop_at_eot), fc2_ksplit, bf16, absorbed ? 1 : 0, n_abs, group, stream_override, forced ? 1 : 0, pipelined ? 1 : 0, lang_mode, fuse ? 1 : 0};
   };
   if (!absorbed && use_graphs && !logits_host) {
     for (Slot& s : slots_) need_cross_kv(s);
diff --git a/whisper.tflite_amd/csrc/engine.h b/whisper.tflite_amd/csrc/engine.h
--- a/whisper.tflite_amd/csrc/engine.h
+++ b/whisper.tflite_amd/csrc/engine.h
@@ -1,4 +1,5 @@
 #pragma once
+#include <cstdlib>
 #include <hip/hip_runtime.h>
 
 #include <algorithm>
@@ -85,6 +86,12 @@
   long use_graphs = 1;
   long cross_absorb = 1;
   long abs_chunks = 0;
+  long dec_fuse = dec_fuse_default();
+  static long dec_fuse_default() {
+    const char* v = getenv("WT_DEC_FUSE");
+    return v && v[0] == '1' ? 1 : 0;
+  }
+  long dec_fuse_active_ = 0;
   long dec_pair = 1;
   long dec_group = 2;
   long last_batches = 0;
@@ -333,6 +340,7 @@
     unsigned long long* best = nullptr;
     long long* ids = nullptr;
     int *n_ids = nullptr, *finished = nullptr;
+    unsigned* tickets = nullptr;
   } dws_[kDecStreams + 1];
   struct LangWorkspace {
     float *probs = nullptr, *prob = nullptr;
diff --git a/whisper.tflite_amd/csrc/k_cross_absorbed.hip b/whisper.tflite_amd/csrc/k_cross_absorbed.hip
--- a/whisper.tflite_amd/csrc/k_cross_absorbed.hip
+++ b/whisper.tflite_amd/csrc/k_cross_absorbed.hip
@@ -22,7 +22,40 @@
   float e_scale;
   float* ws;
   int B, H, T, chunks, nq, p0, tiles_per_chunk;
+  const float* wv_t;
+  const float* bv;
+  float* out;
+  unsigned* tickets;
 };
+
+__device__ __noinline__ void combine_wv_rh(const float* rec, const float* wv_t, const float* bv, float* out_row, int h,
+                                              int chunks, int DM, float* cs, float* part, int tid) {
+  float mx = -3.0e38f;
+  for (int k = 0; k < chunks; ++k) mx = fmaxf(mx, rec[k * (DM + 4) + DM]);
+  if (4 * tid < DM) {
+    f32x4 acc = {0, 0, 0, 0};
+    float l = 0.0f;
+    for (int k = 0; k < chunks; ++k) {
+      const float* r = rec + k * (long)(DM + 4);
+      const float w = __expf(r[DM] - mx);
+      acc += w * *reinterpret_cast<const f32x4*>(r + 4 * tid);
+      l += w * r[DM + 1];
+    }
+    *reinterpret_cast<f32x4*>(&cs[4 * tid]) = acc * (1.0f / l);
+  }
+  __syncthreads();
+  const int j = tid & 63, cq = tid >> 6, c4n = DM / 16;
+  const float* w = wv_t + ((long)h * (DM / 4) + cq * c4n) * 256 + j * 4;
+  float acc = 0.0f;
+  for (int c = 0; c < c4n; ++c) {
+    const f32x4 wv = *reinterpret_cast<const f32x4*>(w + (long)c * 256);
+    const f32x4 x = *reinterpret_cast<const f32x4*>(&cs[(cq * c4n + c) * 4]);
+    acc += (wv[0] * x[0] + wv[1] * x[1]) + (wv[2] * x[2] + wv[3] * x[3]);
+  }
+  part[cq * 64 + j] = acc;
+  __syncthreads();
+  if (tid < 64) out_row[h * 64 + tid] = ((part[tid] + part[64 + tid]) + (part[128 + tid] + part[192 + tid])) + bv[h * 64 + tid];
+}
 
 constexpr float kDeferA = 3.0f, kPShiftA = 12.0f;
 
@@ -79,7 +112,7 @@
   } while (0)
 #endif
 
-template <int DM, int NST, bool BF>
+template <int DM, int NST, bool BF, bool FUSE>
 __global__ __launch_bounds__(320) void cross_absorbed_attention(CrossAbsDev a) {
   using bf16x8 = __attribute__((ext_vector_type(8))) __bf16;
   constexpr int P = DM / 128;
@@ -353,6 +386,34 @@
       rec[DM + 1] = l_run * (1.0f / 4096.0f);
     }
   }
+  if constexpr (FUSE) {
+    asm volatile("s_waitcnt vmcnt(0)" ::: "memory");
+    __syncthreads();
+    float* const cs = reinterpret_cast<float*>(lds);
+    float* const part = cs + 512;
+    int* const is_last = reinterpret_cast<int*>(cs + 768);
+    if (tid == 0) {
+      __builtin_amdgcn_fence(__ATOMIC_RELEASE, "agent");
+      asm volatile("s_waitcnt vmcnt(0)" ::: "memory");
+      const unsigned t = __hip_atomic_fetch_add(a.tickets + b, 1u, __ATOMIC_RELAXED, __HIP_MEMORY_SCOPE_AGENT);
+      const int last = t + 1u == (unsigned)a.chunks;
+      if (last) {
+        __builtin_amdgcn_fence(__ATOMIC_ACQUIRE, "agent");
+        asm volatile("s_waitcnt vmcnt(0)" ::: "memory");
+      }
+      *is_last = last;
+    }
+    __syncthreads();
+    if (*is_last) {
+      for (int c = 0; c < n_qc; ++c) {
+        const int h = c % a.H;
+        const long r = (long)(a.p0 + c / a.H) * a.B + b;
+        combine_wv_rh(a.ws + (r * a.H + h) * a.chunks * (long)(DM + 4), a.wv_t, a.bv, a.out + r * (long)(a.H * 64), h, a.chunks, DM, cs,
+                      part, tid);
+      }
+      if (tid == 0) __hip_atomic_store(a.tickets + b, 0u, __ATOMIC_RELAXED, __HIP_MEMORY_SCOPE_AGENT);
+    }
+  }
 #ifdef WT_ABS_STAMPS
   ABS_STAMP(4);
   if (tid == 0 && blockIdx.x < 4096) {
@@ -369,49 +430,30 @@
                                                               const float* __restrict__ bv, float* __restrict__ out, int H,
                                                               int chunks, int DM) {
   __shared__ __attribute__((aligned(16))) float cs[512];
-  __shared__ float part[4][64];
+  __shared__ float part[4 * 64];
   const long rh = blockIdx.x;
   const int h = (int)(rh % H);
-  const float* rec = ws + rh * chunks * (long)(DM + 4);
-  const int tid = threadIdx.x;
-  float mx = -3.0e38f;
-  for (int k = 0; k < chunks; ++k) mx = fmaxf(mx, rec[k * (DM + 4) + DM]);
-  if (4 * tid < DM) {
-    f32x4 acc = {0, 0, 0, 0};
-    float l = 0.0f;
-    for (int k = 0; k < chunks; ++k) {
-      const float* r = rec + k * (long)(DM + 4);
-      const float w = __expf(r[DM] - mx);
-      acc += w * *reinterpret_cast<const f32x4*>(r + 4 * tid);
-      l += w * r[DM + 1];
-    }
-    *reinterpret_cast<f32x4*>(&cs[4 * tid]) = acc * (1.0f / l);
-  }
-  __syncthreads();
-  const int j = tid & 63, cq = tid >> 6, c4n = DM / 16;
-  const float* w = wv_t + ((long)h * (DM / 4) + cq * c4n) * 256 + j * 4;
-  float acc = 0.0f;
-  for (int c = 0; c < c4n; ++c) {
-    const f32x4 wv = *reinterpret_cast<const f32x4*>(w + (long)c * 256);
-    const f32x4 x = *reinterpret_cast<const f32x4*>(&cs[(cq * c4n + c) * 4]);
-    acc += (wv[0] * x[0] + wv[1] * x[1]) + (wv[2] * x[2] + wv[3] * x[3]);
-  }
-  part[cq][j] = acc;
-  __syncthreads();
-  if (tid < 64) out[(rh / H) * (long)(H * 64) + h * 64 + tid] = ((part[0][tid] + part[1][tid]) + (part[2][tid] + part[3][tid])) + bv[h * 64 + tid];
-}
-
-template <int DM, int NST, bool BF = false>
-void launch_abs(const CrossAbsDev& g, hipStream_t s) {
+  combine_wv_rh(ws + rh * chunks * (long)(DM + 4), wv_t, bv, out + (rh / H) * (long)(H * 64), h, chunks, DM, cs, part, threadIdx.x);
+}
+
+template <int DM, int NST, bool BF, bool FUSE>
+void launch_abs_f(const CrossAbsDev& g, hipStream_t s) {
   constexpr size_t smem = (size_t)NST * (BF ? 1 : 2) * (DM / 128) * 8192 + 8192;
   static_assert(smem <= 160 * 1024, "ring + exchange buffer fit the CU's LDS");
   static const bool raised = [] {
-    (void)hipFuncSetAttribute(reinterpret_cast<const void*>(&cross_absorbed_attention<DM, NST, BF>),
+    (void)hipFuncSetAttribute(reinterpret_cast<const void*>(&cross_absorbed_attention<DM, NST, BF, FUSE>),
                               hipFuncAttributeMaxDynamicSharedMemorySize, 160 * 1024);
     return true;
   }();
   (void)raised;
-  hipLaunchKernelGGL((cross_absorbed_attention<DM, NST, BF>), dim3(g.B * g.chunks), dim3(320), smem, s, g);
+  hipLaunchKernelGGL((cross_absorbed_attention<DM, NST, BF, FUSE>), dim3(g.B * g.chunks), dim3(320), smem, s, g);
+}
+template <int DM, int NST, bool BF = false>
+void launch_abs(const CrossAbsDev& g, hipStream_t s) {
+  if constexpr (!BF) {
+    if (g.tickets) return launch_abs_f<DM, NST, false, true>(g, s);
+  }
+  launch_abs_f<DM, NST, BF, false>(g, s);
 }
 
 }
@@ -431,13 +473,16 @@
   const int groups = (a.batch + split - 1) / split;
   const unsigned short* src[4] = {a.e, a.e2, a.e3, a.e4};
   if (groups > 4) throw Error(kErrInvalidArg, "absorbed cross-attention: at most four encoder batches per chain");
+  if (a.tickets && (a.bf16 || !a.wv_t || !a.bv || !a.out)) {
+    throw Error(kErrInvalidArg, "absorbed cross-attention: the combining tail needs wv_t, bv and out, and has no bf16 form");
+  }
   for (int i = 0; i < groups; ++i)
     if (!src[i]) throw Error(kErrInvalidArg, "absorbed cross-attention: an encoder batch of the chain has no planes");
   CrossAbsDev g{a.qp, reinterpret_cast<const _Float16*>(a.e),
                 {reinterpret_cast<const _Float16*>(a.e), reinterpret_cast<const _Float16*>(src[1] ? src[1] : a.e),
                  reinterpret_cast<const _Float16*>(src[2] ? src[2] : a.e), reinterpret_cast<const _Float16*>(src[3] ? src[3] : a.e)},
                 split, a.e_plane, a.bf16 ? 1.0f : a.e_scale, a.ws, a.batch, a.heads, a.T, a.chunks, a.nq, a.p0,
-                (tiles + a.chunks - 1) / a.chunks};
+                (tiles + a.chunks - 1) / a.chunks, a.wv_t, a.bv, a.out, a.tickets};
   switch (dm) {
     case 128: a.bf16 ? launch_abs<128, 3, true>(g, s) : launch_abs<128, 3>(g, s); break;
     case 384: a.bf16 ? launch_abs<384, 3, true>(g, s) : launch_abs<384, 3>(g, s); break;
diff --git a/whisper.tflite_amd/csrc/k_decoder.hip b/whisper.tflite_amd/csrc/k_decoder.hip
--- a/whisper.tflite_amd/csrc/k_decoder.hip
+++ b/whisper.tflite_amd/csrc/k_decoder.hip
@@ -3,6 +3,7 @@
 #include <cstdlib>
 
 #include "bf16_split.h"
+#include "dec_select.h"
 #include "kernels.h"
 
 namespace wt {
@@ -50,6 +51,13 @@
   float* part;
   const float* xpart;
   int lnp_off;
+  unsigned* sel_ticket;
+  long long* sel_ids;
+  int sel_stride, sel_pos;
+  int* sel_n_ids;
+  int* sel_finished;
+  long long sel_eot;
+  int sel_stop, sel_keep;
 };
 
 struct RowSrc {
@@ -511,6 +519,39 @@
       if (!BF) wl[s] = nwl[s];
     }
   }
+  if (g.sel_ticket) {
+    asm volatile("s_waitcnt vmcnt(0)" ::: "memory");
+    __syncthreads();
+    int* const is_last = reinterpret_cast<int*>(smem_l);
+    if (tid == 0) {
+      __builtin_amdgcn_fence(__ATOMIC_RELEASE, "agent");
+      asm volatile("s_waitcnt vmcnt(0)" ::: "memory");
+      const unsigned t = __hip_atomic_fetch_add(g.sel_ticket, 1u, __ATOMIC_RELAXED, __HIP_MEMORY_SCOPE_AGENT);
+      const int last = t + 1u == gridDim.x * gridDim.y;
+      if (last) {
+        __builtin_amdgcn_fence(__ATOMIC_ACQUIRE, "agent");
+        asm volatile("s_waitcnt vmcnt(0)" ::: "memory");
+      }
+      *is_last = last;
+    }
+    __syncthreads();
+    if (!*is_last) return;
+    for (int b = wid; b < M; b += 4) {
+      const unsigned long long* rec = g.best + (long)b * g.best_stride;
+      unsigned long long p = 0ull;
+      for (int t = lane; t < n_tiles; t += 64) {
+        const unsigned long long v = rec[t];
+        p = v > p ? v : p;
+      }
+#pragma unroll
+      for (int off = 32; off >= 1; off >>= 1) {
+        const unsigned long long o = __shfl_xor(p, off, 64);
+        p = o > p ? o : p;
+      }
+      if (lane == 0) greedy_step(p, b, g.sel_ids, g.sel_stride, g.sel_pos, g.sel_n_ids, g.sel_finished, g.sel_eot, g.sel_stop, g.sel_keep);
+    }
+    if (tid == 0) __hip_atomic_store(g.sel_ticket, 0u, __ATOMIC_RELAXED, __HIP_MEMORY_SCOPE_AGENT);
+  }
 }
 
 template <bool BF, int LNMODE>
@@ -658,7 +699,12 @@
   DecGemmDev g{a.Wt,      1.0f / a.w_scale, a.N,  a.K,       M,         a.B,     a.X,     a.ldx,   a.xin,  a.xout,
                a.ln_g,    a.ln_b,    a.ids,      a.ids_stride, a.pos,   a.tok_emb, a.pos_emb, a.n_vocab,
                a.cross_ws, a.heads,  a.chunks,   a.bias,    gelu,      a.R,     a.Y,     a.ldy,   a.best,
-               a.best_stride > 0 ? a.best_stride : (a.N + 31) / 32, ksplit, a.part,  a.xpart, 0};
+               a.best_stride > 0 ? a.best_stride : (a.N + 31) / 32, ksplit, a.part,  a.xpart, 0,
+               a.sel_ticket, a.sel_ids, a.sel_stride, a.sel_pos, a.sel_n_ids, a.sel_finished, a.sel_eot, a.sel_stop, a.sel_keep ? 1 : 0};
+  if (a.sel_ticket && !(pro == kProLn && epi == kDecLogits && a.sel_ids && a.sel_n_ids && a.sel_finished && a.sel_pos >= 0 &&
+                        a.sel_pos + 1 < a.sel_stride)) {
+    throw Error(kErrInvalidArg, "logits GEMM: the selecting tail belongs to the persistent LayerNorm form and needs ids, n_ids and finished");
+  }
   const bool resid = epi == kDecResid;
   const int waves = resid ? 8 : 4;
   const int kblock = a.K / ksplit;
diff --git a/whisper.tflite_amd/csrc/k_misc.hip b/whisper.tflite_amd/csrc/k_misc.hip
--- a/whisper.tflite_amd/csrc/k_misc.hip
+++ b/whisper.tflite_amd/csrc/k_misc.hip
@@ -3,6 +3,7 @@
 #include <algorithm>
 
 #include "bf16_split.h"
+#include "dec_select.h"
 #include "kernels.h"
 
 namespace wt {
@@ -299,12 +300,7 @@
   __syncthreads();
   if (threadIdx.x != 0) return;
   for (int w = 1; w < 4; ++w) p = wmax[w] > p ? wmax[w] : p;
-  const long long tok = (long long)(unsigned)(p & 0xffffffffull);
-  if (!keep_ids) ids[(long)b * ids_stride + pos + 1] = tok;
-  if (!finished[b]) {
-    n_ids[b] = pos + 2;
-    if (stop_at_eot && tok == eot) finished[b] = 1;
-  }
+  greedy_step(p, b, ids, ids_stride, pos, n_ids, finished, eot, stop_at_eot, keep_ids);
 }
 
 __device__ __forceinline__ float block_sum_256(float v, float* red) {
diff --git a/whisper.tflite_amd/csrc/kernels.h b/whisper.tflite_amd/csrc/kernels.h
--- a/whisper.tflite_amd/csrc/kernels.h
+++ b/whisper.tflite_amd/csrc/kernels.h
@@ -134,6 +134,14 @@
   float* part = nullptr;
   const float* xpart = nullptr;
   bool bf16 = false;
+  unsigned* sel_ticket = nullptr;
+  long long* sel_ids = nullptr;
+  int sel_stride = 0, sel_pos = 0;
+  int* sel_n_ids = nullptr;
+  int* sel_finished = nullptr;
+  long long sel_eot = 0;
+  int sel_stop = 1;
+  bool sel_keep = false;
 };
 void launch_dec_gemm(const DecGemmArgs& a, int pro, int epi, hipStream_t s);
 void launch_dec_finalize_ln(const float* xin, const float* g, const float* b, float* y, int B, int K,
@@ -197,6 +205,10 @@
   float* ws = nullptr;
   int batch = 0, heads = 0, d_model = 0, T = 0, chunks = 1, nq = 1, p0 = 0;
   bool bf16 = false;
+  const float* wv_t = nullptr;
+  const float* bv = nullptr;
+  float* out = nullptr;
+  unsigned* tickets = nullptr;
 };
 void launch_cross_absorbed(const CrossAbsorbedArgs& a, hipStream_t s);
 int cross_absorbed_max_nq(int heads);
```
